# biirving/meant

Hardware: AMD Instinct MI355X
Metric: samples/sec fwd+bwd, MEANT lag=12 d=768 (higher is better)
Workload: dtype bf16; 1 GPU; full MEANT (tweet+image) fwd+CE+bwd, lag=12, d=768, 12 heads, seq=512, 224x224 p=16, E=1, vocab 64001 (BASELINE.json configs[2]/[3]); batch_per_gpu=128, global_batch=128, parallelism=dp1, micro_batches=1, train_mode_dropout=True, activation_checkpointing=False, norm_linear_fold=False, grad_allreduce=False

## Files before the change

### include/meant_hip.h

```cpp
#ifndef MEANT_HIP_H
#define MEANT_HIP_H

#include <stddef.h>
#include <stdint.h>

#ifdef __cplusplus
extern "C" {
#endif

enum meant_dtype { MEANT_F32 = 0, MEANT_BF16 = 1 };
enum meant_raw_dtype { MEANT_RAW_F32 = 0, MEANT_RAW_BF16 = 1, MEANT_RAW_F64 = 2, MEANT_RAW_U8 = 3 };
enum meant_mask_dtype { MEANT_MASK_F32 = 0, MEANT_MASK_BF16 = 1, MEANT_MASK_I64 = 2, MEANT_MASK_U8 = 3, MEANT_MASK_I32 = 4 };

enum meant_status {
  MEANT_OK = 0,
  MEANT_ERR_ARG = -1,
  MEANT_ERR_UNSUPPORTED = -2,
  MEANT_ERR_LAUNCH = -3,
  MEANT_ERR_WORKSPACE = -4
};

enum meant_epilogue {
  MEANT_EPI_NONE = 0,
  MEANT_EPI_GELU = 1,
// ... 22 lines not shown
int meant_rmsnorm_partial_fwd(const void* x, const float* scale, const float* offset, void* y, float* rinv, int64_t rows,
                              int64_t d, int64_t d_part, float eps, int dtype, void* stream);
int meant_rmsnorm_partial_bwd(const void* dy, const void* x, const float* scale, const float* rinv, void* dx, float* dscale,
                              float* doffset, int64_t rows, int64_t d, int64_t d_part, float eps, int dtype, void* workspace,
                              size_t workspace_bytes, void* stream);

int meant_rmsnorm_pooled_ok(int64_t rows, int64_t d, int64_t group_rows);
int meant_rmsnorm_fwd_pooled(const void* x, const float* scale, void* y, float* rinv, float* pooled, int64_t rows,
                             int64_t d, int64_t group_rows, int pool_input, int gelu_input, float eps, float drop_p,
                             uint64_t seed, int dtype, void* stream);
int meant_rmsnorm_bwd_pooled(const void* dy, int dy_pooled, const void* x, const float* scale, const float* rinv,
                             void* dx, float* dscale, int64_t rows, int64_t d, int64_t group_rows, float eps,
                             float drop_p, uint64_t seed, const void* dres, int dres_pooled, const void* gelu_pre,
                             int dtype, void* workspace, size_t workspace_bytes, void* stream);

int meant_rmsnorm_stats(const void* x, float* rinv, int64_t rows, int64_t d, float eps, int dtype, void* stream);
int meant_rmsnorm_bwd_chain(const void* dy, int dy_pooled, const void* x, const float* scale, const float* rinv,
                            void* dx_scaled, float* dscale, int64_t rows, int64_t d, int64_t group_rows, float eps,
                            float drop_p, uint64_t seed, const void* gelu_pre, const float* up_rinv, const float* up_bias,
                            float up_eps, int64_t up_d, float* kcoef, float* dbias_up, int dtype, void* workspace, size_t workspace_bytes,
                            void* stream);
int meant_colscale(const float* w, const float* g, float* out, int64_t N, int64_t K, void* stream);
int meant_colscale_bwd(const float* dwp, const float* w, const float* g, float* dw, float* dg, int64_t N, int64_t K,
                       void* stream);

int meant_layernorm_fwd(const void* x, const float* gamma, const float* beta, void* y, float* stats,
                        int64_t rows, int64_t d, float eps, int dtype, void* stream);
int meant_layernorm_bwd(const void* dy, const void* x, const float* gamma, const float* stats, void* dx,
                        float* dgamma, float* dbeta, int64_t rows, int64_t d, int dtype, void* workspace,
                        size_t workspace_bytes, void* stream);

int meant_linear_fwd(const void* x, int64_t ldx, const void* w, const float* bias, const void* residual,
                     int64_t ldr, void* y, int64_t ldy, void* preact, int64_t M, int64_t N, int64_t K,
                     int epilogue, int dtype, void* stream);
int meant_qkv_proj_fwd(const void* x, int64_t ldx, const void* w, const float* bias, void* qkv, int64_t M,
                       int64_t K, int64_t S, int H, int Dh, int R, const float* qa, const float* qb,
                       const float* ka, const float* kb, int dtype, void* stream);
int meant_qkv_proj_fwd_live(const void* x, int64_t ldx, const void* w, const float* bias, void* qkv, int64_t M,
                            int64_t K, int64_t S, int H, int Dh, int R, const float* qa, const float* qb,
                            const float* ka, const float* kb, const void* kv_lists, int dtype, void* stream);
int meant_linear_fwd_rowscale(const void* x, int64_t ldx, const void* w, const float* bias, const float* row_scale,
                              const void* residual, int64_t ldr, void* y, int64_t ldy, void* preact, int64_t M, int64_t N,
                              int64_t K, int epilogue, int dtype, void* stream);
int meant_linear_bwd_dx_norm(const void* dy_scaled, int64_t lddy, const void* wT, const void* x, int64_t ldx,
                             const float* coef, const void* dres, int64_t lddres, const float* dres_pooled,
                             int64_t group_rows, void* dx, int64_t lddx, int64_t M, int64_t N, int64_t K, int dtype,
                             void* stream);
int meant_linear_bwd_dx(const void* dy, int64_t lddy, const void* wT, void* dx, int64_t lddx, int64_t M,
                        int64_t N, int64_t K, int dtype, void* stream);
size_t meant_linear_bwd_dw_ws(int64_t M, int64_t N, int64_t K, int dtype);
int meant_linear_bwd_dw(const void* dy, int64_t lddy, const void* x, int64_t ldx, float* dw, float* dbias,
                        int64_t M, int64_t N, int64_t K, int dtype, void* workspace, size_t workspace_bytes,
                        void* stream);
int meant_linear_bwd_dw_rows(const void* dy, int64_t lddy, const void* x, int64_t ldx, float* dw, float* dbias,
                             const int* rows_list, const int* rows_count, int64_t M, int64_t N, int64_t K, int dtype,
                             void* workspace, size_t workspace_bytes, void* stream);

int meant_gemm_f32_strided(const float* A, const float* B, float* C, int64_t M, int64_t N, int64_t K,
                           int64_t nb1, int64_t nb2, const int64_t* sA ,
                           const int64_t* sB , const int64_t* sC , float alpha,
                           int accumulate, void* stream);

int meant_rotary_qk(void* qkv, int64_t T, int64_t S, int H, int Dh, int R, const float* qa, const float* qb,
                    const float* ka, const float* kb, int transpose, int dtype, void* stream);

size_t meant_attn_ws(int64_t G, int64_t S, int H, int Dh, int dtype);
size_t meant_attn_fwd_ws(int64_t G, int64_t S, int H, int Dh, int dtype);
enum meant_kv_list_layout { MEANT_KV_LIST_HDR = 64 };
size_t meant_kv_live_rows_ws(int64_t G, int64_t S);
int meant_kv_live_rows(const float* key_mask, int64_t G, int64_t S, int causal, void* lists, size_t lists_bytes, void* stream);
int meant_attn_fwd(const void* qkv, void* o, float* lse, const float* key_mask, int64_t G, int64_t S, int H,
                   int Dh, float scale, int causal, int dtype, void* workspace, size_t workspace_bytes,
                   void* stream);
size_t meant_attn_drop_ws(int64_t G, int64_t S, int H, int Dh, int dtype);
int meant_attn_drop_fwd(const void* qkv, void* o, float* lse, const float* key_mask, int64_t G, int64_t S, int H, int Dh,
                        float scale, int causal, float drop_p, uint64_t seed, int dtype, void* workspace,
                        size_t workspace_bytes, void* stream);
int meant_attn_drop_bwd(const void* qkv, const void* o, const void* do_, const float* lse, const float* key_mask, void* dqkv,
                        int64_t G, int64_t S, int H, int Dh, float scale, int causal, float drop_p, uint64_t seed,
                        int dtype, void* workspace, size_t workspace_bytes, void* stream);
int meant_attn_bwd(const void* qkv, const void* o, const void* do_, const float* lse, const float* key_mask,
                   void* dqkv, int64_t G, int64_t S, int H, int Dh, float scale, int causal, const float* qa,
                   const float* qb, const float* ka, const float* kb, int R, int dtype, void* workspace,
                   size_t workspace_bytes, void* stream);

int meant_gather_rows(const void* src, const int32_t* idx, const void* fill, void* dst, int64_t n, int64_t W, int dtype,
                      void* stream);
int meant_gather_rows_rot(const void* src, const int32_t* idx, void* dst, int64_t n, int64_t S, int H, int Dh, int R,
                          const float* qa, const float* qb, const float* ka, const float* kb, int dtype, void* stream);
int meant_group_scatter(const void* ddst, const int32_t* index, void* dsrc, int64_t B, int64_t L, int64_t G, int64_t S,
                        int64_t W, int dtype, void* stream);
int meant_attn_cls_fwd(const void* qkv, void* out, int64_t ld_out, float* stats, const float* key_mask, int64_t B, int64_t L,
                       int H, int Dh, float scale, int dtype, void* stream);
int meant_attn_cls_bwd(const void* qkv, const void* out, int64_t ld_out, const void* dout, int64_t ld_dout,
                       const float* stats, const float* key_mask, void* dqkv, int64_t B, int64_t L, int H, int Dh,
                       float scale, int dtype, void* stream);
int64_t meant_attn_cls_max_len(int Dh, int backward);
size_t meant_attn_cls_split_ws(int64_t B, int64_t L, int H, int Dh, int nseg);
int meant_attn_cls_split_fwd(const void* qkv, void* out, int64_t ld_out, float* stats, const float* key_mask, int64_t B,
                             int64_t L, int H, int Dh, float scale, int nseg, int dtype, void* workspace,
                             size_t workspace_bytes, void* stream);
int meant_attn_cls_split_bwd(const void* qkv, const void* out, int64_t ld_out, const void* dout, int64_t ld_dout,
                             const float* stats, const float* key_mask, void* dqkv, int64_t B, int64_t L, int H, int Dh,
                             float scale, int nseg, int dtype, void* workspace, size_t workspace_bytes, void* stream);

int meant_token_shift(const void* x, void* y, int64_t B, int64_t frames, int64_t n, int64_t d, int transpose, int dtype,
                      void* stream);
int meant_dropout(const void* x, void* y, int64_t n, float p, uint64_t seed, int dtype, void* stream);

int meant_temporal_attn_fwd(const void* q, const void* kv, void* o, float* p, int64_t B, int L, int H, int Dh,
                            float scale, int dtype, void* stream);
int meant_temporal_attn_bwd(const void* q, const void* kv, const float* p, const void* do_, void* dq, void* dkv,
                            int64_t B, int L, int H, int Dh, float scale, int dtype, void* stream);

int meant_patchify(const void* images, int images_dtype, void* patches, int64_t G, int C, int Hh, int Ww, int p,
                   int dtype, void* stream);

int meant_patchify_raw(const void* images, int raw_dtype, float mean, float inv_std, void* patches, int64_t G, int C,
                       int Hh, int Ww, int p, int dtype, void* stream);

int meant_meanpool_fwd(const void* x, void* out, int64_t ld_out, int64_t col_off, int64_t G, int64_t S, int64_t d,
                       int dtype, int out_dtype, void* stream);
int meant_meanpool_bwd(const void* dout, int64_t ld_out, int64_t col_off, void* dx, int64_t G, int64_t S, int64_t d,
                       int dtype, int out_dtype, void* stream);

int meant_add_rowvec(const void* x, const float* v, void* y, int64_t rows, int64_t d, int64_t period, int dtype,
                     void* stream);
int meant_add_rowvec_bwd(const void* dy, float* dv, int64_t rows, int64_t d, int64_t period, int dtype, void* stream);
int meant_gelu_bwd(const void* dy, const void* pre, void* dx, int64_t n, int dtype, void* stream);
int meant_sigmoid_bwd(const void* dy, const void* y, void* dx, int64_t n, int dtype, void* stream);
int meant_geglu_fwd(const void* h, void* y, int64_t rows, int64_t w, int dtype, void* stream);
int meant_geglu_bwd(const void* h, const void* dy, void* dh, int64_t rows, int64_t w, int dtype, void* stream);
int meant_add(const void* a, const void* b, void* y, int64_t n, int dtype, void* stream);
int meant_cast(const void* src, int dtype_src, void* dst, int dtype_dst, int64_t n, void* stream);
int meant_transpose2d(const void* src, int dtype_src, void* dst, int dtype_dst, int64_t rows, int64_t cols,
                      void* stream);
int meant_pad_copy2d(const void* src, int64_t ld_src, int64_t cols_src, int dtype_src, void* dst, int64_t ld_dst,
                     int64_t cols_dst, int dtype_dst, int64_t rows, void* stream);
int meant_embedding_fwd(const float* table, const int64_t* ids, void* out, int64_t n, int64_t d, int64_t V, int dtype,
                        void* stream);
int meant_embedding_bwd(const void* dout, const int64_t* ids, float* dtable, int64_t n, int64_t d, int64_t V, int dtype,
                        void* stream);
int meant_embedding_bwd_sorted(const void* dout, const int64_t* sorted_ids, const int64_t* order, float* dtable,
                               int64_t n, int64_t d, int64_t V, int dtype, void* stream);
int meant_embedding_bwd_sorted_range(const void* dout, const int64_t* sorted_ids, const int64_t* order, float* dtable,
                                     int64_t n, int64_t d, int64_t V, int64_t id_lo, int64_t id_hi, int dtype, void* stream);
size_t meant_sort_ids_ws(int64_t n, int64_t V);
int meant_sort_ids(const int64_t* ids, int64_t n, int64_t V, int64_t* sorted_ids, int64_t* order, void* workspace,
                   size_t workspace_bytes, void* stream);
size_t meant_embedding_bwd_seg_ws(int64_t n, int64_t d);
int meant_embedding_bwd_seg(const void* dout, const int64_t* sorted_ids, const int64_t* order, float* dtable, int64_t n,
                            int64_t d, int64_t V, int64_t id_lo, int64_t id_hi, int dtype, void* workspace,
                            size_t workspace_bytes, void* stream);

int meant_ce_probs(const float* probs, const int64_t* target, float* loss_accum, float* dprobs, int64_t B, int C,
                   void* stream);
int meant_softmax_ce_fwd(const void* logits, int64_t ld, const int64_t* target, int64_t T, int64_t V, int64_t ignore_index,
                         float* row_loss, float* lse, int dtype, void* stream);
int meant_softmax_ce_bwd(const void* logits, int64_t ld, const int64_t* target, const float* lse, int64_t T, int64_t V,
                         int64_t ignore_index, const float* gscale, void* dlogits, int dtype, void* stream);
size_t meant_select_rows_ws(int64_t T);
int meant_select_rows(const int64_t* target, int64_t T, int64_t V, int64_t ignore_index, int32_t* idx, int32_t* inv,
                      int64_t* target_sel, int32_t* count, void* workspace, size_t workspace_bytes, void* stream);
int meant_metrics_update(const void* scores, int64_t ld, int dtype, const int64_t* target, int64_t B, int C, int64_t ignore_index,
                         int64_t* state, int64_t* confusion, void* stream);
int meant_metrics_update_labels(const int64_t* pred, const int64_t* target, int64_t B, int C, int64_t ignore_index,
                                int64_t* state, int64_t* confusion, void* stream);
int meant_score_capture(const void* scores, int64_t ld, int dtype, const int64_t* target, int64_t B, int C, int col0, int ncol,
                        int64_t ignore_index, uint32_t* keys, int32_t* labels, int64_t capacity, int64_t offset, int64_t* counters,
                        void* stream);
size_t meant_auroc_ws(int64_t n);
int meant_auroc_rank(const uint32_t* keys, const int32_t* labels, int64_t n, int positive, int64_t* out, void* workspace,
                     size_t workspace_bytes, void* stream);
int meant_ce_probs_soft(const float* probs, int64_t ldp, const void* target, int64_t ldt, int target_dtype,
                        float* row_loss, float* loss, float* dprobs, int64_t ldd, int64_t B, int64_t C, void* stream);
int meant_vqa_score_update(const void* scores, int64_t lds, int scores_dtype, const void* target, int64_t ldt, int target_dtype,
                           int64_t B, int64_t C, int64_t* state, void* stream);
int meant_mlm_mask(const int64_t* ids, const void* attention_mask, int mask_dtype, const int64_t* sample_ids, int64_t sample_base,
                   int64_t id_bound, const int64_t* special_ids, int n_special, int64_t B, int64_t S, uint64_t seed,
                   uint32_t threshold, uint32_t t_replace, uint32_t t_random, int64_t mask_id, int64_t V, int64_t ignore_index,
                   int64_t* ids_out, int64_t* labels, void* stream);
int meant_patchify_raw_masked(const void* images, int raw_dtype, float mean, float inv_std, void* patches, int64_t G, int C, int Hh,
                              int Ww, int p, int dtype, uint64_t seed, uint32_t threshold, const int64_t* sample_ids,
                              int64_t sample_base, int64_t id_bound, float mask_value, void* stream);
size_t meant_mim_l1_ws(int64_t N);
int meant_mim_l1_fwd(const void* out, int dtype, const void* images, int raw_dtype, float mean, float inv_std, int64_t B, int C, int Co,
                     int Hh, int Ww, uint64_t seed, uint32_t threshold, const int64_t* sample_ids, int64_t sample_base,
                     int64_t id_bound, float unmasked_label, int on_masked, float* loss, int64_t* count, void* workspace,
                     size_t workspace_bytes, void* stream);
int meant_mim_l1_bwd(const void* out, int dtype, const void* images, int raw_dtype, float mean, float inv_std, int64_t B, int C, int Co,
                     int Hh, int Ww, uint64_t seed, uint32_t threshold, const int64_t* sample_ids, int64_t sample_base,
                     int64_t id_bound, float unmasked_label, int on_masked, const float* g, const int64_t* count, void* dout,
                     void* stream);
int meant_sumsq_f32(const float* x, int64_t n, float* out_accum, void* stream);
int meant_adamw_f32(float* p, const float* g, float* m, float* v, int64_t n, float lr, float beta1, float beta2,
                    float eps, float weight_decay, int64_t step, const float* sumsq, float max_norm,
                    float grad_scale, void* stream);
enum meant_optim_kind { MEANT_OPTIM_ADAMW = 0, MEANT_OPTIM_ADAM = 1 };
enum meant_optim_state_layout { MEANT_OPTIM_STATE_BYTES = 64 };
size_t meant_grad_stats_ws(int64_t n);
int meant_grad_stats_f32(const float* g, int64_t n, void* state, int first, void* workspace, size_t workspace_bytes, void* stream);
int meant_optim_step_f32(float* p, const float* g, float* m, float* v, int64_t n, int kind, float lr, float beta1, float beta2,
                         float eps, float weight_decay, float max_norm, int clip_scaled, const void* state, void* stream);
int meant_optim_finish(void* state, float growth_factor, float backoff_factor, int growth_interval, int dynamic, void* stream);

#ifdef __cplusplus
}
#endif
#endif
```

### meant_amd/csrc/common.h

```cpp
#pragma once
#include <hip/hip_runtime.h>
#include <stdint.h>
#include <stdio.h>
#include <math.h>
#include "../../include/meant_hip.h"

typedef __bf16 bf16;
typedef __attribute__((ext_vector_type(2))) float f32x2;
typedef __attribute__((ext_vector_type(4))) float f32x4;
typedef __attribute__((ext_vector_type(16))) float f32x16;
typedef __attribute__((ext_vector_type(4))) __bf16 bf16x4;
typedef __attribute__((ext_vector_type(8))) __bf16 bf16x8;
typedef __attribute__((ext_vector_type(4))) unsigned int u32x4;
typedef __attribute__((ext_vector_type(2))) unsigned int u32x2;

#define WAVE 64

void meant_set_error(const char* fmt, ...);

#define MEANT_REQUIRE(cond, code, ...)      \
  do {                                      \
    if (!(cond)) {                          \
      meant_set_error(__VA_ARGS__);         \
      return (code);                        \
    }                                       \
  } while (0)

#define MEANT_LAUNCH_CHECK(name)                                                     \
  do {                                                                               \
    hipError_t e__ = hipGetLastError();                                              \
    if (e__ != hipSuccess) {                                                         \
      meant_set_error("%s: launch failed: %s", name, hipGetErrorString(e__));        \
      return MEANT_ERR_LAUNCH;                                                       \
    }                                                                                \
  } while (0)

#define MEANT_MAX_DEVICES 64
int meant_current_device(void);
int meant_raise_dyn_lds(const void* kernel, int bytes);
#define MEANT_RAISE_LDS(kernel, bytes)                                        \
  do {                                                                        \
    int rc__ = meant_raise_dyn_lds((const void*)(kernel), (int)(bytes));      \
    if (rc__) return rc__;                                                    \
  } while (0)

enum meant_option_id {
  MEANT_OPT_NT_STREAM = 0, MEANT_OPT_NT_DYNAMIC, MEANT_OPT_DETERMINISTIC, MEANT_OPT_NT_GRID_CAP, MEANT_OPT_ATTN_SHORT, MEANT_OPT_NT_RAGGED, MEANT_OPT_ATTN_BWD1, MEANT_OPT_TEMPORAL_LONG, MEANT_OPT_KV_SKIP, MEANT_OPT_COUNT
};
int meant_opt(int id);

enum meant_route_id {
  ROUTE_NT128 = 0, ROUTE_NT256, ROUTE_NT256S, ROUTE_NT256S_ROT, ROUTE_NT_SPLIT, ROUTE_TN128, ROUTE_TN256, ROUTE_TN256_DET, ROUTE_TN_TAIL,
  ROUTE_GEMM_F32, ROUTE_ATTN_FWD, ROUTE_ATTN_FWD_D128, ROUTE_ATTN_FWD_D96, ROUTE_ATTN_BWD,
  ROUTE_ATTN_BWD_D128, ROUTE_ATTN_BWD_D96, ROUTE_ATTN_GENERIC, ROUTE_ATTN_CLS, ROUTE_ATTN_SHORT, ROUTE_NT_OVERLAP, ROUTE_ATTN_BWD1,
  ROUTE_ATTN_FWD_D160, ROUTE_ATTN_FWD_D192, ROUTE_ATTN_FWD_D256, ROUTE_ATTN_BWD_D160, ROUTE_ATTN_BWD_D192, ROUTE_ATTN_BWD_D256, ROUTE_TEMPORAL_LONG,
  ROUTE_EMB_SEG, ROUTE_SORT_IDS, ROUTE_NT128K, ROUTE_NT256K, ROUTE_SELECT_ROWS, ROUTE_ROTARY_QK, ROUTE_ROTARY_PAIRS, ROUTE_NT_ROT,
  ROUTE_METRICS_ROWS, ROUTE_METRICS_WAVE, ROUTE_METRICS_LABELS, ROUTE_TN256_ROWS, ROUTE_ATTN_CLS_SPLIT, ROUTE_ROWS_ELEM,
  ROUTE_SCORE_CAPTURE, ROUTE_AUROC_RANK, ROUTE_CE_SOFT_WAVE, ROUTE_CE_SOFT_BLOCK, ROUTE_VQA_SCORE,
  ROUTE_GRAD_STATS, ROUTE_OPTIM_STEP,
  MEANT_ROUTE_COUNT
};
void meant_route_hit(int route);

static inline bool meant_aligned16(const void* p) { return (reinterpret_cast<uintptr_t>(p) & 15) == 0; }
static inline bool meant_aligned_elem(const void* p, int dtype) { return (reinterpret_cast<uintptr_t>(p) & (dtype == MEANT_F32 ? 3 : 1)) == 0; }
static inline int64_t ceil_div(int64_t a, int64_t b) { return (a + b - 1) / b; }

template <typename T> struct Vec8;
template <> struct Vec8<float> {
  f32x4 lo, hi;
  __device__ __forceinline__ float get(int i) const { return i < 4 ? lo[i] : hi[i - 4]; }
  __device__ __forceinline__ void set(int i, float v) { if (i < 4) lo[i] = v; else hi[i - 4] = v; }
};
template <> struct Vec8<bf16> {
  bf16x8 v;
  __device__ __forceinline__ float get(int i) const { return (float)v[i]; }
  __device__ __forceinline__ void set(int i, float x) { v[i] = (bf16)x; }
  __device__ __forceinline__ unsigned raw(int i) const {
    typedef __attribute__((ext_vector_type(4))) unsigned uvec4;
    return (__builtin_bit_cast(uvec4, v)[i >> 1] >> ((i & 1) * 16)) & 0xffffu;
  }
};

__device__ __forceinline__ void rotary_pair(float t0, float t1, float a0, float a1, float b0, float b1, float& o0, float& o1) {
  o0 = __builtin_fmaf(t0, a0, -(t1 * b0));
  o1 = __builtin_fmaf(t1, a1, t0 * b1);
}

template <typename T> __device__ __forceinline__ Vec8<T> load8(const T* p);
template <> __device__ __forceinline__ Vec8<float> load8<float>(const float* p) {
  Vec8<float> r; r.lo = *reinterpret_cast<const f32x4*>(p); r.hi = *reinterpret_cast<const f32x4*>(p + 4); return r;
}
template <> __device__ __forceinline__ Vec8<bf16> load8<bf16>(const bf16* p) {
  Vec8<bf16> r; r.v = *reinterpret_cast<const bf16x8*>(p); return r;
}
template <typename T> __device__ __forceinline__ Vec8<T> load8s(const T* p);
template <> __device__ __forceinline__ Vec8<float> load8s<float>(const float* p) {
  Vec8<float> r;
  r.lo = __builtin_nontemporal_load(reinterpret_cast<const f32x4*>(p));
  r.hi = __builtin_nontemporal_load(reinterpret_cast<const f32x4*>(p + 4));
  return r;
}
template <> __device__ __forceinline__ Vec8<bf16> load8s<bf16>(const bf16* p) {
  Vec8<bf16> r; r.v = __builtin_nontemporal_load(reinterpret_cast<const bf16x8*>(p)); return r;
}
template <typename T> __device__ __forceinline__ void store8s(T* p, const Vec8<T>& v);
template <> __device__ __forceinline__ void store8s<float>(float* p, const Vec8<float>& v) {
  __builtin_nontemporal_store(v.lo, reinterpret_cast<f32x4*>(p)); __builtin_nontemporal_store(v.hi, reinterpret_cast<f32x4*>(p + 4));
}
template <> __device__ __forceinline__ void store8s<bf16>(bf16* p, const Vec8<bf16>& v) {
  __builtin_nontemporal_store(v.v, reinterpret_cast<bf16x8*>(p));
}
template <typename T> __device__ __forceinline__ void store8(T* p, const Vec8<T>& v);
template <> __device__ __forceinline__ void store8<float>(float* p, const Vec8<float>& v) {
  *reinterpret_cast<f32x4*>(p) = v.lo; *reinterpret_cast<f32x4*>(p + 4) = v.hi;
}
template <> __device__ __forceinline__ void store8<bf16>(bf16* p, const Vec8<bf16>& v) {
  *reinterpret_cast<bf16x8*>(p) = v.v;
}

__device__ __forceinline__ float to_f(float x) { return x; }
__device__ __forceinline__ float to_f(bf16 x) { return (float)x; }
template <typename T> __device__ __forceinline__ T from_f(float x);
template <> __device__ __forceinline__ float from_f<float>(float x) { return x; }
template <> __device__ __forceinline__ bf16 from_f<bf16>(float x) { return (bf16)x; }

__device__ __forceinline__ float wave_sum(float v) {
#pragma unroll
  for (int o = 32; o > 0; o >>= 1) v += __shfl_xor(v, o, 64);
  return v;
}
__device__ __forceinline__ float wave_max(float v) {
#pragma unroll
  for (int o = 32; o > 0; o >>= 1) v = fmaxf(v, __shfl_xor(v, o, 64));
  return v;
}

#define MEANT_DPP_ADD(v, CTRL) ((v) + __builtin_bit_cast(float, __builtin_amdgcn_update_dpp(0, __builtin_bit_cast(int, (v)), (CTRL), 0xf, 0xf, true)))
__device__ __forceinline__ float wave_sum_dpp(float v) {
  v = MEANT_DPP_ADD(v, 0xB1);
  v = MEANT_DPP_ADD(v, 0x4E);
  v = MEANT_DPP_ADD(v, 0x141);
  v = MEANT_DPP_ADD(v, 0x140);
  const int b = __builtin_bit_cast(int, v);
  const float r0 = __builtin_bit_cast(float, __builtin_amdgcn_readlane(b, 0)), r1 = __builtin_bit_cast(float, __builtin_amdgcn_readlane(b, 16));
  const float r2 = __builtin_bit_cast(float, __builtin_amdgcn_readlane(b, 32)), r3 = __builtin_bit_cast(float, __builtin_amdgcn_readlane(b, 48));
  return (r0 + r1) + (r2 + r3);
}
__device__ __forceinline__ float rms_rinv(float sumsq, float inv_sqrt_d, float eps) {
  return 1.0f / (sqrtf(sumsq) * inv_sqrt_d + eps);
}

__device__ __forceinline__ float gelu_erf(float x) { return 0.5f * x * (1.0f + erff(x * 0.70710678118654752f)); }
__device__ __forceinline__ float gelu_erf_fast(float x) {
  const float z = fabsf(x) * 0.70710678118654752f;
  const float t = __builtin_amdgcn_rcpf(fmaf(0.3275911f, z, 1.0f));
  float p = fmaf(1.061405429f, t, -1.453152027f);
  p = fmaf(p, t, 1.421413741f);
  p = fmaf(p, t, -0.284496736f);
  p = fmaf(p, t, 0.254829592f);
  const float half_erfc = 0.5f * p * t * __builtin_amdgcn_exp2f(-1.4426950408889634f * z * z);
  const float phi = x < 0.f ? half_erfc : 1.0f - half_erfc;
  return x * phi;
}
__device__ __forceinline__ float gelu_phi_fast(float x) {
  const float z = fabsf(x) * 0.70710678118654752f;
  const float t = __builtin_amdgcn_rcpf(fmaf(0.3275911f, z, 1.0f));
  float p = fmaf(1.061405429f, t, -1.453152027f);
  p = fmaf(p, t, 1.421413741f);
  p = fmaf(p, t, -0.284496736f);
  p = fmaf(p, t, 0.254829592f);
  const float half_erfc = 0.5f * p * t * __builtin_amdgcn_exp2f(-1.4426950408889634f * z * z);
  return x < 0.f ? half_erfc : 1.0f - half_erfc;
}
constexpr unsigned PHI_LO = 0x3A80u, PHI_HI = 0x40FFu, PHI_N = PHI_HI - PHI_LO + 1;
__device__ __forceinline__ unsigned phi_slot(unsigned bits) {
  unsigned m = bits & 0x7FFFu;
  m = m < PHI_LO ? PHI_LO : m;
  m = m > PHI_HI ? PHI_HI : m;
  return (m - PHI_LO) + ((bits >> 15) & 1u) * PHI_N;
}
__device__ __forceinline__ float gelu_erf_grad(float x) {
  const float cdf = 0.5f * (1.0f + erff(x * 0.70710678118654752f));
  const float pdf = 0.39894228040143268f * __expf(-0.5f * x * x);
  return cdf + x * pdf;
}

__device__ __forceinline__ float gelu_erf_grad_fast(float x) {
  const float z = fabsf(x) * 0.70710678118654752f;
  const float t = __builtin_amdgcn_rcpf(fmaf(0.3275911f, z, 1.0f));
  float p = fmaf(1.061405429f, t, -1.453152027f);
  p = fmaf(p, t, 1.421413741f);
  p = fmaf(p, t, -0.284496736f);
  p = fmaf(p, t, 0.254829592f);
  const float e = __builtin_amdgcn_exp2f(-0.72134752044448170f * x * x);
  const float half_erfc = 0.5f * p * t * e;
  const float phi = x < 0.f ? half_erfc : 1.0f - half_erfc;
  return fmaf(x * 0.39894228040143268f, e, phi);
}

__device__ __forceinline__ float hash_uniform(uint64_t seed, uint64_t idx) {
  uint64_t z = seed + idx * 0x9E3779B97F4A7C15ull;
  z = (z ^ (z >> 30)) * 0xBF58476D1CE4E5B9ull;
  z = (z ^ (z >> 27)) * 0x94D049BB133111EBull;
  z = z ^ (z >> 31);
  return (float)(z >> 40) * (1.0f / 16777216.0f);
}
#ifndef DROP_HASH32
#define DROP_HASH32 1
#endif
__device__ __forceinline__ uint32_t mix32(uint32_t h) {
  h ^= h >> 16; h *= 0x85EBCA6Bu; h ^= h >> 13; h *= 0xC2B2AE35u; h ^= h >> 16;
// ... 80 lines not shown
```

### meant_amd/csrc/core.hip

```cpp
#include "common.h"
#include <stdarg.h>
#include <string.h>
#include <stdlib.h>
#include <atomic>
#include <mutex>
#include <unordered_map>

static thread_local char g_err[512] = "";

void meant_set_error(const char* fmt, ...) {
  va_list ap;
  va_start(ap, fmt);
  vsnprintf(g_err, sizeof(g_err), fmt, ap);
  va_end(ap);
}

extern "C" const char* meant_last_error(void) { return g_err; }

extern "C" int meant_version(void) { return 200;  }

namespace {
struct DeviceState {
  int cus = -1;
  std::unordered_map<const void*, int> lds_raised;
};
std::mutex g_dev_mu;
DeviceState g_dev[MEANT_MAX_DEVICES];
}

int meant_current_device(void) {
  int dev = 0;
  if (hipGetDevice(&dev) != hipSuccess || dev < 0 || dev >= MEANT_MAX_DEVICES) return -1;
  return dev;
}

extern "C" int meant_num_cus(void) {
  const int dev = meant_current_device();
  if (dev < 0) return 0;
  std::lock_guard<std::mutex> lock(g_dev_mu);
  DeviceState& st = g_dev[dev];
  if (st.cus < 0) {
    hipDeviceProp_t p;
    st.cus = hipGetDeviceProperties(&p, dev) == hipSuccess ? p.multiProcessorCount : 0;
  }
  return st.cus;
}

int meant_raise_dyn_lds(const void* kernel, int bytes) {
  const int dev = meant_current_device();
  MEANT_REQUIRE(dev >= 0, MEANT_ERR_LAUNCH, "no current HIP device (or device index >= %d)", MEANT_MAX_DEVICES);
  std::lock_guard<std::mutex> lock(g_dev_mu);
  DeviceState& st = g_dev[dev];
  const auto it = st.lds_raised.find(kernel);
  if (it != st.lds_raised.end() && it->second >= bytes) return MEANT_OK;
  const hipError_t e = hipFuncSetAttribute(kernel, hipFuncAttributeMaxDynamicSharedMemorySize, bytes);
  MEANT_REQUIRE(e == hipSuccess, MEANT_ERR_LAUNCH, "hipFuncSetAttribute(%d bytes of LDS) failed on device %d: %s", bytes, dev,
                hipGetErrorString(e));
  st.lds_raised[kernel] = bytes;
  return MEANT_OK;
}

namespace {
struct OptionDef { const char* name; const char* env; int dflt; };
const OptionDef k_options[MEANT_OPT_COUNT] = {
    {"nt_stream", "MEANT_NT_STREAM", 1},
    {"nt_dynamic", "MEANT_NT_DYNAMIC", 1},
    {"deterministic", "MEANT_DETERMINISTIC", 0},
    {"nt_grid_cap", "MEANT_NT_GRID_CAP", 0},
    {"attn_short", "MEANT_ATTN_SHORT", 1},
    {"nt_ragged", "MEANT_NT_RAGGED", 1},
    {"attn_bwd1", "MEANT_ATTN_BWD1", 1},
    {"temporal_long", "MEANT_TEMPORAL_LONG", 0},
    {"kv_skip", "MEANT_KV_SKIP", 3},
};
bool is_nt_pp(const char* name) { return name && !strcmp(name, "nt_pp"); }
std::atomic<int> g_opt[MEANT_OPT_COUNT];
std::once_flag g_opt_once;
void options_init() {
  std::call_once(g_opt_once, [] {
    for (int i = 0; i < MEANT_OPT_COUNT; ++i) {
      const char* v = getenv(k_options[i].env);
      g_opt[i].store(v && *v ? atoi(v) : k_options[i].dflt, std::memory_order_relaxed);
    }
  });
}
int option_index(const char* name) {
  if (!name) return -1;
  for (int i = 0; i < MEANT_OPT_COUNT; ++i)
    if (!strcmp(name, k_options[i].name)) return i;
  return -1;
}
}

int meant_opt(int id) {
  options_init();
  return g_opt[id].load(std::memory_order_relaxed);
}

extern "C" int meant_set_option(const char* name, int value) {
  options_init();
  if (is_nt_pp(name)) {
    MEANT_REQUIRE(value == 1, MEANT_ERR_UNSUPPORTED, "meant_set_option: nt_pp is always 1 (the lock-step kernel was removed)");
    return MEANT_OK;
  }
  const int i = option_index(name);
  MEANT_REQUIRE(i >= 0, MEANT_ERR_ARG, "meant_set_option: unknown option '%s'", name ? name : "(null)");
  g_opt[i].store(value, std::memory_order_relaxed);
  return MEANT_OK;
}

extern "C" int meant_get_option(const char* name, int* value) {
  options_init();
  if (is_nt_pp(name) && value) { *value = 1; return MEANT_OK; }
  const int i = option_index(name);
  MEANT_REQUIRE(i >= 0 && value, MEANT_ERR_ARG, "meant_get_option: unknown option '%s'", name ? name : "(null)");
  *value = g_opt[i].load(std::memory_order_relaxed);
  return MEANT_OK;
}

namespace {
const char* const k_routes[MEANT_ROUTE_COUNT] = {
    "nt128", "nt256", "nt256s", "nt256s_rot", "nt_split", "tn128", "tn256", "tn256_det", "tn_tail", "gemm_f32",
    "attn_fwd", "attn_fwd_d128", "attn_fwd_d96", "attn_bwd", "attn_bwd_d128", "attn_bwd_d96",
    "attn_generic", "attn_cls", "attn_short", "nt_overlap", "attn_bwd1",
    "attn_fwd_d160", "attn_fwd_d192", "attn_fwd_d256", "attn_bwd_d160", "attn_bwd_d192", "attn_bwd_d256",
    "temporal_long", "emb_seg", "sort_ids", "nt128k", "nt256k", "select_rows",
    "rotary_qk", "rotary_pairs",
    "nt_rot",
    "metrics_rows", "metrics_wave", "metrics_labels",
    "tn256_rows",
    "attn_cls_split",
    "rows_elem",
    "score_capture", "auroc_rank",
    "ce_soft_wave", "ce_soft_block",
    "vqa_score",
    "grad_stats", "optim_step",
};
std::atomic<long long> g_route[MEANT_ROUTE_COUNT];
}

void meant_route_hit(int route) { g_route[route].fetch_add(1, std::memory_order_relaxed); }

extern "C" int64_t meant_route_count(const char* route) {
  if (!route) return -1;
  for (int i = 0; i < MEANT_ROUTE_COUNT; ++i)
    if (!strcmp(route, k_routes[i])) return (int64_t)g_route[i].load(std::memory_order_relaxed);
  return -1;
}

extern "C" void meant_route_reset(void) {
  for (int i = 0; i < MEANT_ROUTE_COUNT; ++i) g_route[i].store(0, std::memory_order_relaxed);
}
```

### meant_amd/csrc/embedding.hip

```cpp
#include "common.h"
#include "internal.h"

#define EMB_REQ(c, ...) MEANT_REQUIRE(c, MEANT_ERR_ARG, __VA_ARGS__)

namespace {

constexpr int SORT_TILE = 2048, SORT_WAVE_SPAN = 512, SORT_ROUNDS = 8;

__device__ __forceinline__ uint32_t sort_key(int64_t id, int64_t V) {
  return (uint32_t)(id < 0 ? 0 : (id >= V ? V - 1 : id));
}

template <bool IDS>
__global__ __launch_bounds__(256) void sort_hist_kernel(const int64_t* __restrict__ ids, const uint32_t* __restrict__ keys, int64_t n, int64_t V,
                                                         int passes, uint32_t* __restrict__ ghist, uint32_t* __restrict__ tile_hist,
                                                         int64_t ntiles) {
  __shared__ uint32_t h[4][256];
  const int tid = threadIdx.x;
#pragma unroll
  for (int p = 0; p < 4; ++p) h[p][tid] = 0;
  __syncthreads();
  const int64_t base = (int64_t)blockIdx.x * SORT_TILE;
  for (int i = 0; i < SORT_TILE / 256; ++i) {
    const int64_t j = base + i * 256 + tid;
    if (j < n) {
      const uint32_t key = IDS ? sort_key(ids[j], V) : keys[j];
      for (int p = 0; p < passes; ++p) atomicAdd(&h[p][(key >> (8 * p)) & 255u], 1u);
    }
  }
  __syncthreads();
  tile_hist[(int64_t)tid * ntiles + blockIdx.x] = h[0][tid];
  for (int p = 0; p < passes; ++p)
    if (h[p][tid]) atomicAdd(&ghist[p * 256 + tid], h[p][tid]);
}

__global__ __launch_bounds__(256) void sort_count_kernel(const uint32_t* __restrict__ keys, int64_t n, int shift,
                                                          uint32_t* __restrict__ tile_hist, int64_t ntiles) {
  __shared__ uint32_t h[256];
  const int tid = threadIdx.x;
  h[tid] = 0;
  __syncthreads();
  const int64_t base = (int64_t)blockIdx.x * SORT_TILE;
  for (int i = 0; i < SORT_TILE / 256; ++i) {
    const int64_t j = base + i * 256 + tid;
    if (j < n) atomicAdd(&h[(keys[j] >> shift) & 255u], 1u);
  }
  __syncthreads();
  tile_hist[(int64_t)tid * ntiles + blockIdx.x] = h[tid];
}

__global__ __launch_bounds__(256) void sort_scan_kernel(const uint32_t* __restrict__ ghist, uint32_t* __restrict__ tile_hist, int64_t ntiles) {
  __shared__ uint32_t wsum[4];
  const int tid = threadIdx.x, digit = blockIdx.x;
  uint32_t carry;
  block_scan_incl(tid < digit ? ghist[tid] : 0u, wsum, &carry);
  uint32_t* row = tile_hist + (int64_t)digit * ntiles;
  for (int64_t t0 = 0; t0 < ntiles; t0 += 256) {
    const int64_t t = t0 + tid;
    const uint32_t x = t < ntiles ? row[t] : 0u;
    uint32_t total;
    const uint32_t incl = block_scan_incl(x, wsum, &total);
    if (t < ntiles) row[t] = carry + incl - x;
    carry += total;
  }
}

template <bool FIRST, bool LAST>
__global__ __launch_bounds__(256) void sort_scatter_kernel(const int64_t* __restrict__ ids, const uint32_t* __restrict__ kin,
                                                            const uint32_t* __restrict__ vin, int64_t n, int64_t V, int shift,
                                                            const uint32_t* __restrict__ tile_off, int64_t ntiles,
                                                            uint32_t* __restrict__ kout, uint32_t* __restrict__ vout,
                                                            int64_t* __restrict__ sorted_ids, int64_t* __restrict__ order) {
  __shared__ uint32_t cnt[4][256];
  const int tid = threadIdx.x, lane = tid & 63, wave = tid >> 6;
#pragma unroll
  for (int w = 0; w < 4; ++w) cnt[w][tid] = 0;
  __syncthreads();
  const int64_t base = (int64_t)blockIdx.x * SORT_TILE + wave * SORT_WAVE_SPAN;
  uint32_t key[SORT_ROUNDS], val[SORT_ROUNDS], rk[SORT_ROUNDS];
#pragma unroll
  for (int r = 0; r < SORT_ROUNDS; ++r) {
    const int64_t j = base + r * 64 + lane;
    const bool valid = j < n;
    key[r] = valid ? (FIRST ? sort_key(ids[j], V) : kin[j]) : 0u;
    val[r] = valid ? (FIRST ? (uint32_t)j : vin[j]) : 0u;
    const uint32_t dig = (key[r] >> shift) & 255u;
    unsigned long long m = __ballot(valid);
#pragma unroll
    for (int b = 0; b < 8; ++b) {
      const bool bit = (dig >> b) & 1u;
      const unsigned long long bal = __ballot(valid && bit);
      m &= bit ? bal : ~bal;
    }
    const unsigned long long below = m & ((1ull << lane) - 1ull);
    rk[r] = valid ? cnt[wave][dig] + (uint32_t)__popcll(below) : 0u;
    __syncthreads();
    if (valid && below == 0) cnt[wave][dig] += (uint32_t)__popcll(m);
    __syncthreads();
  }
  {
    uint32_t o = tile_off[(int64_t)tid * ntiles + blockIdx.x];
#pragma unroll
    for (int w = 0; w < 4; ++w) {
      const uint32_t c = cnt[w][tid];
      cnt[w][tid] = o;
      o += c;
    }
  }
  __syncthreads();
#pragma unroll
  for (int r = 0; r < SORT_ROUNDS; ++r) {
    const int64_t j = base + r * 64 + lane;
    if (j >= n) continue;
    const int64_t pos = (int64_t)cnt[wave][(key[r] >> shift) & 255u] + rk[r];
    if (pos >= n) continue;
    if (LAST) {
      sorted_ids[pos] = (int64_t)key[r];
      order[pos] = (int64_t)val[r];
    } else {
      kout[pos] = key[r];
      vout[pos] = val[r];
    }
  }
}

int sort_passes(int64_t V) {
  int bits = 0;
  for (uint64_t m = (uint64_t)(V - 1); m; m >>= 1) ++bits;
  const int p = (bits + 7) / 8;
  return p < 1 ? 1 : p;
}
size_t align256(size_t x) { return (x + 255) & ~(size_t)255; }
struct SortWs { size_t ghist, tile_hist, buf[2], total; int nbuf; };
SortWs sort_ws_layout(int64_t n, int passes) {
  SortWs w;
  const int64_t ntiles = ceil_div(n, SORT_TILE);
  w.nbuf = passes - 1 < 2 ? passes - 1 : 2;
  size_t off = 0;
  w.ghist = off; off += align256(4 * 256 * sizeof(uint32_t));
  w.tile_hist = off; off += align256((size_t)ntiles * 256 * sizeof(uint32_t));
  for (int i = 0; i < 2; ++i) {
    w.buf[i] = off;
    if (i < w.nbuf) off += 2 * align256((size_t)n * sizeof(uint32_t));
  }
  w.total = off;
  return w;
}

constexpr int SEG = 256;
template <typename T>
__global__ __launch_bounds__(256) void emb_seg_kernel(const T* __restrict__ dout, const int64_t* __restrict__ sorted_ids,
                                                       const int64_t* __restrict__ order, float* __restrict__ dtable,
                                                       float* __restrict__ part, int64_t n, int64_t d, int64_t V, int64_t id_lo,
                                                       int64_t id_hi, int cb_chunks) {
  const int lane = threadIdx.x & 63, wave = threadIdx.x >> 6;
  const int64_t s = (int64_t)blockIdx.x * 4 + wave;
  const int64_t j0 = s * SEG;
  if (j0 >= n) return;
  const int64_t j1 = j0 + SEG < n ? j0 + SEG : n;
  if (sorted_ids[j1 - 1] < id_lo || sorted_ids[j0] >= id_hi) return;
  const int c0 = blockIdx.y * cb_chunks;
  const int left = (int)(d >> 3) - c0;
  const int nch = left < cb_chunks ? left : cb_chunks;
  const bool has0 = lane < nch, has1 = lane + 64 < nch;
  const int64_t col0 = (int64_t)(c0 + lane) * 8, col1 = (int64_t)(c0 + lane + 64) * 8;
  float acc0[8], acc1[8];
#pragma unroll
  for (int e = 0; e < 8; ++e) acc0[e] = acc1[e] = 0.f;
  int64_t cur = sorted_ids[j0];
  bool open_left = j0 > 0 && sorted_ids[j0 - 1] == cur;

  auto flush = [&](int64_t id, int slot) {
    if (id < 0 || id >= V || id < id_lo || id >= id_hi) return;
    if (slot >= 0) {
      float* row = part + (s * 2 + slot) * d;
      Vec8<float> v;
      if (has0) {
#pragma unroll
        for (int e = 0; e < 8; ++e) v.set(e, acc0[e]);
        store8<float>(row + col0, v);
      }
      if (has1) {
#pragma unroll
        for (int e = 0; e < 8; ++e) v.set(e, acc1[e]);
        store8<float>(row + col1, v);
      }
      return;
    }
    float* row = dtable + id * d;
    if (has0) {
      Vec8<float> v = load8<float>(row + col0);
#pragma unroll
      for (int e = 0; e < 8; ++e) v.set(e, v.get(e) + acc0[e]);
      store8<float>(row + col0, v);
    }
    if (has1) {
      Vec8<float> v = load8<float>(row + col1);
#pragma unroll
      for (int e = 0; e < 8; ++e) v.set(e, v.get(e) + acc1[e]);
      store8<float>(row + col1, v);
    }
  };

  for (int64_t jb = j0; jb < j1; jb += 64) {
    const int64_t jl = jb + lane < j1 ? jb + lane : j1 - 1;
    const long long my_id = sorted_ids[jl], my_ord = order[jl];
    const int cnt = (int)(j1 - jb < 64 ? j1 - jb : 64);
    for (int t0 = 0; t0 < cnt; t0 += 4) {
      Vec8<T> r0[4], r1[4];
      long long ids4[4];
#pragma unroll
      for (int u = 0; u < 4; ++u) {
        const int t = t0 + u < cnt ? t0 + u : cnt - 1;
        ids4[u] = __shfl(my_id, t, 64);
        const long long ord = __shfl(my_ord, t, 64);
        const bool row_ok = ord >= 0 && ord < n;
        const T* src = dout + (row_ok ? ord : 0) * d;
        r0[u] = Vec8<T>{};
        r1[u] = Vec8<T>{};
        if (has0 && row_ok) r0[u] = load8s<T>(src + col0);
        if (has1 && row_ok) r1[u] = load8s<T>(src + col1);
      }
#pragma unroll
      for (int u = 0; u < 4; ++u) {
        if (t0 + u >= cnt) break;
        const int64_t id = ids4[u];
        if (id != cur) {
          flush(cur, open_left ? 0 : -1);
#pragma unroll
          for (int e = 0; e < 8; ++e) acc0[e] = acc1[e] = 0.f;
          cur = id;
          open_left = false;
        }
#pragma unroll
        for (int e = 0; e < 8; ++e) {
          if (has0) acc0[e] += r0[u].get(e);
          if (has1) acc1[e] += r1[u].get(e);
        }
      }
    }
  }
  const bool open_right = j1 < n && sorted_ids[j1] == cur;
  flush(cur, open_left ? 0 : (open_right ? 1 : -1));
}

constexpr int SEG_SHORT = 16;
__global__ __launch_bounds__(256) void emb_seg_cross_kernel(const int64_t* __restrict__ sorted_ids, const float* __restrict__ part,
                                                             int* __restrict__ longk, float* __restrict__ dtable, int64_t n, int64_t d,
                                                             int64_t V, int64_t id_lo, int64_t id_hi) {
  const int lane = threadIdx.x & 63, wave = threadIdx.x >> 6;
  const int64_t s = (int64_t)blockIdx.x * 4 + wave, j0 = s * SEG, j1 = j0 + SEG;
  if (j1 >= n) return;
  const int64_t id = sorted_ids[j1 - 1];
  const bool owner = sorted_ids[j1] == id && !(j0 > 0 && sorted_ids[j0 - 1] == id)
                     && id >= 0 && id < V && id >= id_lo && id < id_hi;
  int64_t K = 0;
  if (owner) {
    const int64_t nst = (n + SEG - 1) / SEG;
    int64_t follow = 0;
    for (int64_t t0 = s + 1;; t0 += 64) {
      const int64_t t = t0 + lane;
      const int k = __popcll(__ballot(t < nst && sorted_ids[t * SEG] == id));
      follow += k;
      if (k < 64) break;
    }
    K = follow + 1;
  }
  if (blockIdx.y == 0 && lane == 0) longk[s] = K > SEG_SHORT ? (int)K : 0;
  if (K == 0 || K > SEG_SHORT) return;
  const int64_t col = (int64_t)blockIdx.y * 256 + lane * 4;
  if (col >= d) return;
  f32x4 acc = *reinterpret_cast<const f32x4*>(part + (s * 2 + 1) * d + col);
  for (int64_t k = 1; k < K; ++k) acc += *reinterpret_cast<const f32x4*>(part + (s + k) * 2 * d + col);
  f32x4* dst = reinterpret_cast<f32x4*>(dtable + id * d + col);
  *dst = *dst + acc;
}

__global__ __launch_bounds__(256) void emb_seg_long_kernel(const int64_t* __restrict__ sorted_ids, const float* __restrict__ part,
                                                            const int* __restrict__ longk, float* __restrict__ dtable, int64_t d) {
  __shared__ f32x4 red[16][16];
  const int tid = threadIdx.x;
  const int64_t s = blockIdx.x;
  const int64_t K = longk[s];
  if (K == 0) return;
  const int64_t id = sorted_ids[s * SEG + SEG - 1];
  const int p = tid >> 4;
  const int64_t col = (int64_t)blockIdx.y * 64 + (tid & 15) * 4;
  const bool active = col < d;
  const int64_t piece = (K + 15) / 16, k0 = p * piece, k1 = k0 + piece < K ? k0 + piece : K;
  f32x4 acc = {0.f, 0.f, 0.f, 0.f};
  if (active) {
#pragma unroll 4
    for (int64_t k = k0; k < k1; ++k) {
      const float* row = k == 0 ? part + (s * 2 + 1) * d : part + (s + k) * 2 * d;
      acc += *reinterpret_cast<const f32x4*>(row + col);
    }
  }
  red[p][tid & 15] = acc;
  __syncthreads();
#pragma unroll
  for (int h = 8; h > 0; h >>= 1) {
    if (p < h) red[p][tid & 15] += red[p + h][tid & 15];
    __syncthreads();
  }
  if (p == 0 && active) {
    f32x4* dst = reinterpret_cast<f32x4*>(dtable + id * d + col);
    *dst = *dst + red[0][tid & 15];
  }
}

size_t seg_part_bytes(int64_t n, int64_t d) { return (size_t)ceil_div(n, SEG) * 2 * (size_t)d * sizeof(float); }

template <typename T>
__global__ __launch_bounds__(256) void embedding_fwd_kernel(const float* __restrict__ table, const int64_t* __restrict__ ids,
                                                             T* __restrict__ out, int64_t n, int d, int64_t V) {
  const int lane = threadIdx.x & 63, wave = threadIdx.x >> 6;
  const int nch = d >> 3;
  for (int64_t r = (int64_t)blockIdx.x * 4 + wave; r < n; r += (int64_t)gridDim.x * 4) {
    int64_t id = ids[r];
    id = id < 0 ? 0 : (id >= V ? V - 1 : id);
    const float* src = table + id * d;
    for (int ch = lane; ch < nch; ch += 64) {
      const Vec8<float> v = load8<float>(src + ch * 8);
      Vec8<T> o;
#pragma unroll
      for (int k = 0; k < 8; ++k) o.set(k, v.get(k));
      store8s<T>(out + r * d + ch * 8, o);
    }
  }
}
template <typename T>
__global__ __launch_bounds__(256) void embedding_fwd_elem_kernel(const float* __restrict__ table, const int64_t* __restrict__ ids,
                                                                  T* __restrict__ out, int64_t n, int d, int64_t V) {
  const int lane = threadIdx.x & 63, wave = threadIdx.x >> 6;
  for (int64_t r = (int64_t)blockIdx.x * 4 + wave; r < n; r += (int64_t)gridDim.x * 4) {
    int64_t id = ids[r];
    id = id < 0 ? 0 : (id >= V ? V - 1 : id);
    const float* src = table + id * d;
    for (int e = lane; e < d; e += 64) out[r * d + e] = from_f<T>(src[e]);
  }
}
template <typename T>
__global__ __launch_bounds__(256) void embedding_bwd_kernel(const T* __restrict__ dout, const int64_t* __restrict__ ids,
                                                             float* __restrict__ dtable, int64_t n, int d, int64_t V) {
  const int lane = threadIdx.x & 63, wave = threadIdx.x >> 6;
  for (int64_t r = (int64_t)blockIdx.x * 4 + wave; r < n; r += (int64_t)gridDim.x * 4) {
    int64_t id = ids[r];
    id = id < 0 ? 0 : (id >= V ? V - 1 : id);
    float* dst = dtable + id * d;
    for (int e = lane; e < d; e += 64) atomicAdd(dst + e, to_f(dout[r * d + e]));
  }
}

constexpr int EMB_SEG = 256;
template <typename T>
__global__ __launch_bounds__(256) void embedding_bwd_sorted_kernel(const T* __restrict__ dout, const int64_t* __restrict__ sorted_ids,
                                                                    const int64_t* __restrict__ order, float* __restrict__ dtable,
                                                                    int64_t n, int d, int64_t V, int det, int64_t id_lo, int64_t id_hi) {
  const int lane = threadIdx.x & 63, wave = threadIdx.x >> 6;
  int64_t j0 = ((int64_t)blockIdx.x * 4 + wave) * EMB_SEG;
  if (j0 >= n) return;
  int64_t j1 = j0 + EMB_SEG < n ? j0 + EMB_SEG : n;
  if (sorted_ids[j1 - 1] < id_lo || sorted_ids[j0] >= id_hi) return;
  if (det) {
    if (j0 > 0) {
      const int64_t prev = sorted_ids[j0 - 1];
      while (j0 < j1 && sorted_ids[j0] == prev) ++j0;
      if (j0 == j1) return;
    }
    const int64_t last = sorted_ids[j1 - 1];
    while (j1 < n && sorted_ids[j1] == last) ++j1;
  }
  const int nch = d >> 3;
  const bool has1 = lane + 64 < nch, has0 = lane < nch;
  float acc0[8], acc1[8];
#pragma unroll
  for (int e = 0; e < 8; ++e) acc0[e] = acc1[e] = 0.f;
  int64_t cur = sorted_ids[j0];
  bool shared = !det && j0 > 0 && sorted_ids[j0 - 1] == cur;

  auto flush = [&](int64_t id, bool atomic) {
    if (id < 0 || id >= V || id < id_lo || id >= id_hi) return;
    float* row = dtable + id * d;
    if (atomic) {
#pragma unroll
      for (int e = 0; e < 8; ++e) {
        if (has0) atomicAdd(row + lane * 8 + e, acc0[e]);
        if (has1) atomicAdd(row + (lane + 64) * 8 + e, acc1[e]);
      }
    } else {
      if (has0) {
        Vec8<float> v = load8<float>(row + lane * 8);
#pragma unroll
        for (int e = 0; e < 8; ++e) v.set(e, v.get(e) + acc0[e]);
        store8<float>(row + lane * 8, v);
      }
      if (has1) {
        Vec8<float> v = load8<float>(row + (lane + 64) * 8);
#pragma unroll
        for (int e = 0; e < 8; ++e) v.set(e, v.get(e) + acc1[e]);
        store8<float>(row + (lane + 64) * 8, v);
      }
    }
  };

  for (int64_t jb = j0; jb < j1; jb += 64) {
    const int64_t jl = jb + lane < j1 ? jb + lane : j1 - 1;
    const long long my_id = sorted_ids[jl], my_ord = order[jl];
    const int cnt = (int)(j1 - jb < 64 ? j1 - jb : 64);
    for (int t0 = 0; t0 < cnt; t0 += 4) {
      Vec8<T> r0[4], r1[4];
      long long ids4[4];
#pragma unroll
      for (int u = 0; u < 4; ++u) {
        const int t = t0 + u < cnt ? t0 + u : cnt - 1;
        ids4[u] = __shfl(my_id, t, 64);
        const long long ord = __shfl(my_ord, t, 64);
        const T* src = dout + ord * d;
        if (has0) r0[u] = load8s<T>(src + lane * 8);
        if (has1) r1[u] = load8s<T>(src + (lane + 64) * 8);
      }
#pragma unroll
      for (int u = 0; u < 4; ++u) {
        if (t0 + u >= cnt) break;
        const int64_t id = ids4[u];
        if (id != cur) {
          flush(cur, shared);
#pragma unroll
          for (int e = 0; e < 8; ++e) acc0[e] = acc1[e] = 0.f;
          cur = id;
          shared = false;
        }
#pragma unroll
        for (int e = 0; e < 8; ++e) {
          if (has0) acc0[e] += r0[u].get(e);
          if (has1) acc1[e] += r1[u].get(e);
        }
      }
    }
  }
  flush(cur, !det && (shared || (j1 < n && sorted_ids[j1] == cur)));
}

}

static int sort_run(const int64_t* ids, int64_t V, const uint32_t* keys, const uint32_t* vals, int64_t n, int passes, int64_t* sorted_ids,
                    int64_t* order, uint32_t* keys_out, uint32_t* vals_out, const SortWs& w, char* base, hipStream_t st, const char* what) {
  const bool from_ids = ids != nullptr;
  uint32_t* ghist = (uint32_t*)(base + w.ghist);
  uint32_t* tile_hist = (uint32_t*)(base + w.tile_hist);
  uint32_t* bk[2] = {nullptr, nullptr};
  uint32_t* bv[2] = {nullptr, nullptr};
  for (int i = 0; i < w.nbuf; ++i) {
    bk[i] = (uint32_t*)(base + w.buf[i]);
    bv[i] = (uint32_t*)(base + w.buf[i] + align256((size_t)n * sizeof(uint32_t)));
  }
  const int64_t ntiles = ceil_div(n, SORT_TILE);
  const dim3 grid((unsigned)ntiles), block(256);
  const hipError_t e = hipMemsetAsync(ghist, 0, 4 * 256 * sizeof(uint32_t), st);
  MEANT_REQUIRE(e == hipSuccess, MEANT_ERR_LAUNCH, "%s: clearing the digit counters failed: %s", what, hipGetErrorString(e));
  if (from_ids) hipLaunchKernelGGL(sort_hist_kernel<true>, grid, block, 0, st, ids, keys, n, V, passes, ghist, tile_hist, ntiles);
  else hipLaunchKernelGGL(sort_hist_kernel<false>, grid, block, 0, st, ids, keys, n, V, passes, ghist, tile_hist, ntiles);
  for (int p = 0; p < passes; ++p) {
    const bool first = p == 0, last = p == passes - 1;
    const uint32_t* kin = first ? keys : bk[(p - 1) & 1];
    const uint32_t* vin = first ? vals : bv[(p - 1) & 1];
    uint32_t* kout = last ? keys_out : bk[p & 1];
    uint32_t* vout = last ? vals_out : bv[p & 1];
    const int shift = 8 * p;
    if (!first) hipLaunchKernelGGL(sort_count_kernel, grid, block, 0, st, kin, n, shift, tile_hist, ntiles);
    hipLaunchKernelGGL(sort_scan_kernel, dim3(256), block, 0, st, (const uint32_t*)(ghist + p * 256), tile_hist, ntiles);
#define SORT_SCATTER(F, L)                                                                                                     \
  hipLaunchKernelGGL((sort_scatter_kernel<F, L>), grid, block, 0, st, ids, kin, vin, n, V, shift, (const uint32_t*)tile_hist, \
                     ntiles, kout, vout, sorted_ids, order)
    const bool F = first && from_ids, L = last && from_ids;
    if (F && L) SORT_SCATTER(true, true);
    else if (F) SORT_SCATTER(true, false);
    else if (L) SORT_SCATTER(false, true);
    else SORT_SCATTER(false, false);
#undef SORT_SCATTER
  }
  MEANT_LAUNCH_CHECK(what);
  return MEANT_OK;
}

extern "C" size_t meant_sort_ids_ws(int64_t n, int64_t V) {
  if (n <= 0 || V <= 0 || n >= (1ll << 31) || V >= (1ll << 31)) return 0;
  return sort_ws_layout(n, sort_passes(V)).total;
}

extern "C" int meant_sort_ids(const int64_t* ids, int64_t n, int64_t V, int64_t* sorted_ids, int64_t* order, void* workspace,
                              size_t workspace_bytes, void* stream) {
  EMB_REQ(ids && sorted_ids && order && n > 0 && V > 0, "sort_ids: bad argument");
  MEANT_REQUIRE(n < (1ll << 31) && V < (1ll << 31), MEANT_ERR_UNSUPPORTED, "sort_ids: n=%lld and V=%lld must be below 2^31", (long long)n,
                (long long)V);
  {
    const char *a = (const char*)ids, *o1 = (const char*)sorted_ids, *o2 = (const char*)order;
    const size_t len = (size_t)n * sizeof(int64_t);
    const auto overlap = [len](const char* x, const char* y) { return x < y + len && y < x + len; };
    EMB_REQ(!overlap(a, o1) && !overlap(a, o2) && !overlap(o1, o2), "sort_ids: ids, sorted_ids and order must not overlap");
  }
  const int passes = sort_passes(V);
  const SortWs w = sort_ws_layout(n, passes);
  MEANT_REQUIRE(workspace && workspace_bytes >= w.total, MEANT_ERR_WORKSPACE, "sort_ids: workspace of %zu bytes needed, %zu given", w.total, workspace_bytes);
  EMB_REQ((reinterpret_cast<uintptr_t>(workspace) & 3) == 0, "sort_ids: 4-byte workspace alignment");
  const int rc = sort_run(ids, V, nullptr, nullptr, n, passes, sorted_ids, order, nullptr, nullptr, w, (char*)workspace, (hipStream_t)stream, "sort_ids");
  if (rc != MEANT_OK) return rc;
  meant_route_hit(ROUTE_SORT_IDS);
  return MEANT_OK;
}

size_t sort_u32_ws(int64_t n) { return n <= 0 || n >= (1ll << 31) ? 0 : sort_ws_layout(n, 4).total; }

int sort_u32_launch(const uint32_t* keys, const uint32_t* vals, int64_t n, uint32_t* keys_out, uint32_t* vals_out, void* ws, size_t ws_bytes,
                    hipStream_t stream) {
  EMB_REQ(keys && vals && keys_out && vals_out && n > 0 && n < (1ll << 31), "sort_u32: bad argument");
  const SortWs w = sort_ws_layout(n, 4);
  MEANT_REQUIRE(ws && ws_bytes >= w.total, MEANT_ERR_WORKSPACE, "sort_u32: workspace of %zu bytes needed, %zu given", w.total, ws_bytes);
  EMB_REQ((reinterpret_cast<uintptr_t>(ws) & 3) == 0, "sort_u32: 4-byte workspace alignment");
  return sort_run(nullptr, 0, keys, vals, n, 4, nullptr, nullptr, keys_out, vals_out, w, (char*)ws, stream, "sort_u32");
}

extern "C" size_t meant_embedding_bwd_seg_ws(int64_t n, int64_t d) {
  if (n <= 0 || d <= 0) return 0;
  return seg_part_bytes(n, d) + align256((size_t)ceil_div(n, SEG) * sizeof(int));
}

extern "C" int meant_embedding_bwd_seg(const void* dout, const int64_t* sorted_ids, const int64_t* order, float* dtable, int64_t n,
                                       int64_t d, int64_t V, int64_t id_lo, int64_t id_hi, int dtype, void* workspace,
                                       size_t workspace_bytes, void* stream) {
  EMB_REQ(dout && sorted_ids && order && dtable && n > 0 && d > 0 && V > 0 && 0 <= id_lo && id_lo <= id_hi && id_hi <= V,
          "embedding_bwd_seg: bad argument");
  MEANT_REQUIRE(d % 8 == 0, MEANT_ERR_UNSUPPORTED, "embedding_bwd_seg: d=%lld must be a multiple of 8", (long long)d);
  MEANT_REQUIRE(d < (1ll << 22), MEANT_ERR_UNSUPPORTED, "embedding_bwd_seg: d=%lld is beyond the launch grid (d < 2^22)", (long long)d);
  const size_t need = meant_embedding_bwd_seg_ws(n, d);
  MEANT_REQUIRE(workspace && workspace_bytes >= need, MEANT_ERR_WORKSPACE, "embedding_bwd_seg: workspace of %zu bytes needed, %zu given", need, workspace_bytes);
  EMB_REQ(meant_aligned16(dout) && meant_aligned16(dtable) && meant_aligned16(workspace), "embedding_bwd_seg: 16-byte alignment");
  if (id_lo == id_hi) return MEANT_OK;
  const int64_t nst = ceil_div(n, SEG);
  const int chunks = (int)(d >> 3);
  const int ncb = (int)ceil_div(chunks, 128);
  const int cb_chunks = (int)ceil_div(chunks, ncb);
  hipStream_t st = (hipStream_t)stream;
  DISPATCH_DTYPE(dtype, T,
                 hipLaunchKernelGGL(emb_seg_kernel<T>, dim3((unsigned)ceil_div(nst, 4), (unsigned)ncb), dim3(256), 0, st, (const T*)dout,
                                    sorted_ids, order, dtable, (float*)workspace, n, d, V, id_lo, id_hi, cb_chunks));
  if (nst > 1) {
    int* longk = (int*)((char*)workspace + seg_part_bytes(n, d));
    hipLaunchKernelGGL(emb_seg_cross_kernel, dim3((unsigned)ceil_div(nst - 1, 4), (unsigned)ceil_div(d, 256)), dim3(256), 0, st, sorted_ids,
                       (const float*)workspace, longk, dtable, n, d, V, id_lo, id_hi);
    hipLaunchKernelGGL(emb_seg_long_kernel, dim3((unsigned)(nst - 1), (unsigned)ceil_div(d, 64)), dim3(256), 0, st, sorted_ids,
                       (const float*)workspace, (const int*)longk, dtable, d);
  }
  MEANT_LAUNCH_CHECK("embedding_bwd_seg");
  meant_route_hit(ROUTE_EMB_SEG);
  return MEANT_OK;
}

extern "C" int meant_embedding_fwd(const float* table, const int64_t* ids, void* out, int64_t n, int64_t d, int64_t V, int dtype, void* stream) {
  EMB_REQ(table && ids && out && n > 0 && d > 0 && d < (1ll << 30) && V > 0, "embedding_fwd: bad argument");
  int64_t nb = ceil_div(n, 4); if (nb > 8192) nb = 8192;
  if (d % 8 == 0) {
    DISPATCH_DTYPE(dtype, T,
                   hipLaunchKernelGGL(embedding_fwd_kernel<T>, dim3((unsigned)nb), dim3(256), 0, (hipStream_t)stream, table, ids, (T*)out, n, (int)d, V));
  } else {
    DISPATCH_DTYPE(dtype, T,
                   hipLaunchKernelGGL(embedding_fwd_elem_kernel<T>, dim3((unsigned)nb), dim3(256), 0, (hipStream_t)stream, table, ids, (T*)out, n, (int)d, V));
  }
  MEANT_LAUNCH_CHECK("embedding_fwd");
  return MEANT_OK;
}
extern "C" int meant_embedding_bwd_sorted(const void* dout, const int64_t* sorted_ids, const int64_t* order, float* dtable, int64_t n,
                                          int64_t d, int64_t V, int dtype, void* stream) {
  EMB_REQ(dout && sorted_ids && order && dtable && n > 0 && d > 0 && V > 0, "embedding_bwd_sorted: bad argument");
  MEANT_REQUIRE(d <= 1024 && d % 8 == 0, MEANT_ERR_UNSUPPORTED, "embedding_bwd_sorted: d=%lld must be a multiple of 8 and <= 1024", (long long)d);
  EMB_REQ(meant_aligned16(dout) && meant_aligned16(dtable), "embedding_bwd_sorted: 16-byte alignment");
  const int64_t nb = ceil_div(n, 4 * EMB_SEG);
  DISPATCH_DTYPE(dtype, T,
                 hipLaunchKernelGGL(embedding_bwd_sorted_kernel<T>, dim3((unsigned)nb), dim3(256), 0, (hipStream_t)stream, (const T*)dout,
                                    sorted_ids, order, dtable, n, (int)d, V, meant_opt(MEANT_OPT_DETERMINISTIC) != 0, (int64_t)0, V));
  MEANT_LAUNCH_CHECK("embedding_bwd_sorted");
  return MEANT_OK;
}

extern "C" int meant_embedding_bwd_sorted_range(const void* dout, const int64_t* sorted_ids, const int64_t* order, float* dtable, int64_t n,
                                                int64_t d, int64_t V, int64_t id_lo, int64_t id_hi, int dtype, void* stream) {
  EMB_REQ(dout && sorted_ids && order && dtable && n > 0 && d > 0 && V > 0 && 0 <= id_lo && id_lo <= id_hi && id_hi <= V,
         "embedding_bwd_sorted_range: bad argument");
  MEANT_REQUIRE(d <= 1024 && d % 8 == 0, MEANT_ERR_UNSUPPORTED, "embedding_bwd_sorted_range: d=%lld must be a multiple of 8 and <= 1024", (long long)d);
  EMB_REQ(meant_aligned16(dout) && meant_aligned16(dtable), "embedding_bwd_sorted_range: 16-byte alignment");
  if (id_lo == id_hi) return MEANT_OK;
  const int64_t nb = ceil_div(n, 4 * EMB_SEG);
  DISPATCH_DTYPE(dtype, T,
                 hipLaunchKernelGGL(embedding_bwd_sorted_kernel<T>, dim3((unsigned)nb), dim3(256), 0, (hipStream_t)stream, (const T*)dout,
                                    sorted_ids, order, dtable, n, (int)d, V, meant_opt(MEANT_OPT_DETERMINISTIC) != 0, id_lo, id_hi));
  MEANT_LAUNCH_CHECK("embedding_bwd_sorted_range");
  return MEANT_OK;
}

extern "C" int meant_embedding_bwd(const void* dout, const int64_t* ids, float* dtable, int64_t n, int64_t d, int64_t V, int dtype, void* stream) {
  EMB_REQ(dout && ids && dtable && n > 0 && d > 0 && V > 0, "embedding_bwd: bad argument");
  int64_t nb = ceil_div(n, 4); if (nb > 8192) nb = 8192;
  DISPATCH_DTYPE(dtype, T,
                 hipLaunchKernelGGL(embedding_bwd_kernel<T>, dim3((unsigned)nb), dim3(256), 0, (hipStream_t)stream, (const T*)dout, ids, dtable, n, (int)d, V));
  MEANT_LAUNCH_CHECK("embedding_bwd");
  return MEANT_OK;
}
```

### meant_amd/modules.py

```python
from __future__ import annotations

import math
from typing import Optional

import torch
from torch import nn

from . import ops
from ._lib import EPI_NONE, EPI_GELU, EPI_SIGMOID


COMPOSE_PRE_LINEAR = True

POOL_LAST_LINEAR = True

import os as _os
TWO_STREAMS = _os.environ.get("MEANT_TWO_STREAMS", "1") != "0"
_SIDE = {}


def _side_stream(device):
    key = (device.type, device.index)
    if key not in _SIDE:
        _SIDE[key] = torch.cuda.Stream(device=device)
# ... 98 lines not shown
        s = self.scale.float()[None, :] ** power[:, None]
        s = torch.cat((s, s), dim=-1)
        si = s ** -1
        return cos * s, sin * s, cos * si, sin * si

    def tables(self, seq_len: int, device, head_dim: Optional[int] = None) -> tuple:
        key = (seq_len, str(device), self.freqs._version, self.freqs.data_ptr())
        hit = self._tables.get(key)
        if hit is not None:
            if head_dim is None:
                return hit
            pkey = ("pad", head_dim) + key
            padded = self._tables.get(pkey)
            if padded is None:
                padded = self._tables[pkey] = ops.pad_rotary_tables(hit, head_dim)
            return padded
        with torch.no_grad():
            f = self.freqs.detach().float().cpu()
            pos = torch.arange(seq_len)
            ang = torch.repeat_interleave(pos.to(f.dtype)[:, None] * f[None, :], 2, dim=-1)
            cos, sin = ang.cos(), ang.sin()
            if self.use_xpos:
                power = (pos - seq_len // 2) / self.scale_base
                s = self.scale.detach().float().cpu()[None, :] ** power[:, None]
                s = torch.cat((s, s), dim=-1)
                si = s ** -1
                t = (cos * s, sin * s, cos * si, sin * si)
            else:
                t = (cos, sin, cos, sin)
            t = tuple(x.contiguous().to(device) for x in t)
            if not self.use_xpos:
                t = (t[0], t[1], t[0], t[1])
        self._tables = {k: v for k, v in self._tables.items() if k[-2:] == key[-2:]}
        self._tables[key] = t
        return t if head_dim is None else self.tables(seq_len, device, head_dim)


def _rotate_pairs(t, a, b):
    R = a.shape[1]
    tr = t[..., :R].float()
    pr = tr.reshape(*tr.shape[:-1], R // 2, 2)
    rot = torch.stack((-pr[..., 1], pr[..., 0]), dim=-1).reshape(tr.shape)
    out = tr * a[None, :, None, :] + rot * b[None, :, None, :]
    return torch.cat((out.to(t.dtype), t[..., R:]), dim=-1)


def _qkv_params(mod, pre=None):
    wqkv = torch.cat([mod.q.weight, mod.v.weight, mod.k.weight], dim=0)
    bqkv = torch.cat([mod.q.bias, mod.v.bias, mod.k.bias], dim=0)
    if pre is not None:
        wqkv, bqkv = ops.compose_linear(pre.weight, pre.bias, wqkv, bqkv)
    return wqkv, bqkv


def _rotate_learned(qkv, rot: RotaryEmbedding, G, S, H, D):
    q5 = qkv.view(G, S, 3, H, D // H)
    qa, qb, ka, kb = rot.tables_autograd(S)
    return torch.stack((_rotate_pairs(q5[:, :, 0], qa, qb), _rotate_pairs(q5[:, :, 1], ka, kb), q5[:, :, 2]), dim=2).reshape(G * S, 3 * D)


def learned_rotary_attention(x, mod, rot: RotaryEmbedding, key_mask, causal: bool, pre=None):
    G, S, d = x.shape
    H = mod.num_heads
    wqkv, bqkv = _qkv_params(mod, pre)
    D = wqkv.shape[0] // 3
    packed = _rotate_learned(ops.linear(x.reshape(G * S, d), wqkv, bqkv), rot, G, S, H, D)
    return ops.attention_core(packed, G, S, H, 1.0 / math.sqrt(D), None, causal, key_mask).view(G, S, D)


def score_dropout_attention(x, mod, rot: RotaryEmbedding, key_mask, causal: bool, p: float, seed: int, pre=None):
    G, S, d = x.shape
    H = mod.num_heads
    wqkv, bqkv = _qkv_params(mod, pre)
    D = wqkv.shape[0] // 3
    qkv = ops.linear(x.reshape(G * S, d), wqkv, bqkv)
    tables = None
    if rot is not None and getattr(rot, 'learned_freq', False):
        qkv = _rotate_learned(qkv, rot, G, S, H, D)
    elif rot is not None:
        tables = rot.tables(S, x.device)
    return ops.attention_core_score_dropout(qkv, G, S, H, 1.0 / math.sqrt(D), p, seed, tables, causal, key_mask).view(G, S, D)


class _MHA(nn.Module):

    def __init__(self, num_heads, dim, mask, droput, rot=None):
        super().__init__()
        self.num_heads, self.dim = num_heads, dim
        self.Dh = int(dim / num_heads)
        self.dropout = nn.Dropout(droput)
        if rot is not None:
            setattr(self, *rot)
        self.mask = mask
        self.softmax = nn.Softmax(dim=-1)
        self.multi_mad = Linear(self.num_heads * self.Dh, self.dim)
        self.atten_size = self.Dh * self.num_heads
        self.q = Linear(self.dim, self.atten_size)
        self.v = Linear(self.dim, self.atten_size)
        self.k = Linear(self.dim, self.atten_size)

    def _fused(self, x, rot, key_mask, pre):
        if rot is not None and getattr(rot, 'learned_freq', False):
            return learned_rotary_attention(x, self, rot, key_mask, bool(self.mask), pre)
        tables = rot.tables(x.shape[1], x.device, ops.run_head_dim(self.Dh, x.dtype)) if rot is not None else None
        prew = (pre.weight, pre.bias) if pre is not None else None
        return ops.qkv_attention(x, self.q.weight, self.q.bias, self.v.weight, self.v.bias, self.k.weight, self.k.bias,
                                 tables, key_mask, bool(self.mask), self.num_heads, pre=prew)


class attention(_MHA):

    def __init__(self, num_heads, dim, pos_emb: RotaryEmbedding, mask=False, droput=0.):
        super().__init__(num_heads, dim, mask, droput, ('pos_emb', pos_emb))

    def core(self, x, pre=None):
        return self._fused(x, self.pos_emb, None, pre)

    def forward(self, input):
        out = self.multi_mad(self.core(input))
        if self.training and self.dropout.p > 0:
            out = self.dropout(out)
        return out


class xPosAttention(_MHA):

    def __init__(self, num_heads, dim, xPos: RotaryEmbedding, mask=True, droput=0.):
        super().__init__(num_heads, dim, mask, droput, ('xPos', xPos))

    def core(self, x, attention_mask=None, pre=None):
        if self.training and self.dropout.p > 0:
            return score_dropout_attention(x, self, self.xPos, attention_mask, bool(self.mask), float(self.dropout.p), _seed(), pre)
        return self._fused(x, self.xPos, attention_mask, pre)

    def forward(self, input, attention_mask=None):
        return self.multi_mad(self.core(input, attention_mask))


class temporal(_MHA):

    def __init__(self, num_heads, dim, mask=False, droput=0.):
        super().__init__(num_heads, dim, mask, droput)

    def forward(self, input):
        o = ops.temporal_attention(input, self.q.weight, self.q.bias, self.v.weight, self.v.bias, self.k.weight, self.k.bias,
                                   self.num_heads)
        return self.multi_mad(o)


def _seed() -> int:
    return int(torch.randint(0, 2 ** 62, (1,)).item())


def _encoder_layer(e, e2, x, margs, p1, p2, pool, fold):
    n, res = ops.rmsnorm_fork(x, e[0].scale, e[0].eps, any_width=True)
    if COMPOSE_PRE_LINEAR and e[1].bias is not None:
        h = e[2].multi_mad(e[2].core(n, *margs, pre=e[1]))
    else:
        h = e[2](e[1](n), *margs)
    h = e[3](h, drop_p=p1, seed=_seed() if p1 > 0 else 0)
    x1 = e[-1](h, residual=res)
    fold = ops.norm_linear_ok(x1, e2[1].weight, fold)
    seed2 = _seed() if p2 > 0 else 0
    if pool and ops.pooled_norm_ok(x1, x1.shape[1]):
        if fold:
            return ops.norm_linear_gelu_norm_pooled(x1, e2[0].scale, e2[0].eps, e2[1].weight, e2[1].bias, e2[3].scale, e2[3].eps, p2, seed2)
        n, xm = ops.rmsnorm_fork_pooled(x1, e2[0].scale, e2[0].eps)
        return ops.linear_gelu_rmsnorm_pooled(n, e2[1].weight, e2[1].bias, e2[3].scale, e2[3].eps, p2, seed2), xm
    if fold:
        h, res = ops.norm_linear_gelu_norm(x1, e2[0].scale, e2[0].eps, e2[1].weight, e2[1].bias, e2[3].scale, e2[3].eps, p2, seed2)
    else:
        n, res = ops.rmsnorm_fork(x1, e2[0].scale, e2[0].eps, any_width=True)
        h = ops.linear_gelu_rmsnorm(n, e2[1].weight, e2[1].bias, e2[3].scale, e2[3].eps, p2, seed2, any_width=True)
    if pool:
        return h, res
    return e2[-1](h, residual=res)


class visionEncoder(nn.Module):

    def __init__(self, dim, num_heads, flash=False):
        super().__init__()
        self.dim, self.num_heads = dim, num_heads
        self.posEmbed = RotaryEmbedding(dim=math.floor(dim / num_heads / 2), freqs_for='pixel')
        atten = attention(num_heads, dim, self.posEmbed)
        self.encode = nn.ModuleList([RMSNorm(dim), Linear(dim, dim), atten, RMSNorm(dim), Linear(dim, dim)])
        self.encode2 = nn.ModuleList([RMSNorm(dim), Linear(dim, dim), nn.GELU(), RMSNorm(dim), Linear(dim, dim)])

    def forward(self, input, pool: bool = False, fold=None):
        return _encoder_layer(self.encode, self.encode2, input, (), 0.0, 0.0, pool, fold)


class languageEncoder(nn.Module):

    def __init__(self, dim, num_heads, dropout=0.0, flash=False):
        super().__init__()
        self.dim, self.num_heads = dim, num_heads
        self.xPos = RotaryEmbedding(dim=48, use_xpos=True)
        att = xPosAttention(num_heads, dim, self.xPos)
        self.encode = nn.ModuleList([RMSNorm(dim), Linear(dim, dim), att, RMSNorm(dim), nn.Dropout(dropout), Linear(dim, dim)])
        self.encode2 = nn.ModuleList([RMSNorm(dim), Linear(dim, dim), nn.GELU(), RMSNorm(dim), nn.Dropout(), Linear(dim, dim)])

    def forward(self, input, attention_mask=None, pool: bool = False, fold=None):
        e, e2 = self.encode, self.encode2
        p1, p2 = (e[4].p, e2[4].p) if self.training else (0.0, 0.0)
        return _encoder_layer(e, e2, input, (attention_mask,), p1, p2, pool, fold)


class temporalEncoder(nn.Module):

    def __init__(self, dim, num_heads, lag, norms=True):
        super().__init__()
        self.dim, self.num_heads, self.lag = dim, num_heads, lag
        self.temp_embedding = nn.Parameter(torch.randn(1, lag, dim))
        if norms:
            mods = [RMSNorm(dim), Linear(dim, dim), temporal(num_heads, dim), RMSNorm(dim), Linear(dim, dim)]
        else:
            mods = [Linear(dim, dim), temporal(num_heads, dim), Linear(dim, dim)]
        self.temp_encode = nn.ModuleList(mods)

    def forward(self, x):
        x = ops.add_rowvec(x, self.temp_embedding)
        for mod in self.temp_encode:
            x = mod(x)
        return x


class _Patchify(nn.Module):

    def __init__(self, p):
        super().__init__()
        self.p = p
        self.out_dtype = torch.float32
        self.norm_mean, self.norm_std = 0.0, 1.0

    def set_normalization(self, mean: float, std: float):
        self.norm_mean, self.norm_std = float(mean), float(std)

    def forward(self, images):
        return ops.patchify(images, self.p, self.out_dtype, self.norm_mean, self.norm_std)


class _PatchEmbed(nn.Sequential):
    def __init__(self, patch_dim, dim, p):
        super().__init__(_Patchify(p), Linear(patch_dim, dim))

    def forward(self, images, dtype=torch.float32):
        self[0].out_dtype = dtype
        return self[1](self[0](images))


def _run_encoder(enc, x, *args, checkpoint: bool = False, **kw):
    if checkpoint and torch.is_grad_enabled() and x.requires_grad:
        from torch.utils.checkpoint import checkpoint as _ckpt
        return _ckpt(enc, x, *args, use_reentrant=False, preserve_rng_state=True, **kw)
    return enc(x, *args, **kw)


def _ckpt_setting(model):
    v = getattr(model, "activation_checkpointing", False)
    return v if isinstance(v, bool) else int(v)


def _run_stack(encoders, x, *args, checkpoint=False):
    n = len(encoders)
    fold = ops.stack_fold(n, x.numel() // x.shape[-1], x.shape[-1])
    for i, enc in enumerate(encoders):
        ck = checkpoint if isinstance(checkpoint, bool) else i < checkpoint
        last = enc.encode2[-1]
        if POOL_LAST_LINEAR and i == n - 1 and isinstance(last, Linear):
            h, res = _run_encoder(enc, x, *args, checkpoint=ck, pool=True, fold=fold)
            return (h, res, last.weight, last.bias)
        x = _run_encoder(enc, x, *args, checkpoint=ck, fold=fold)
    return x


def _pool_parts(compute_dtype, *stacks):
    if all(isinstance(st, tuple) for st in stacks):
        if all(st[0].dim() == 3 for st in stacks):
            return ops.pool_linear_cat(list(stacks))
        parts = [st if st[0].dim() == 2 else (ops.meanpool_f32(st[0]), ops.meanpool_f32(st[1]), st[2], st[3]) for st in stacks]
        return ops.pooled_linear_cat(parts, compute_dtype)
    toks = []
    for st in stacks:
        if isinstance(st, tuple):
            h, res, w, b = st
            if h.dim() == 2:
                raise RuntimeError("meant_amd: one stack pooled its last layer, the other did not")
            st = ops.linear(h, w, b, residual=res)
        toks.append(st)
    return ops.meanpool_cat(*toks)


POOL_OWN_STREAM = _os.environ.get("MEANT_POOL_OWN_STREAM", "1") == "1"


def _pool_own_stream(compute_dtype, st):
    if not POOL_OWN_STREAM or not (isinstance(st, tuple) and st[0].dim() == 2):
        return st
    return ops.pooled_linear_cat([st], compute_dtype)


def _embed(mods, ids, dtype):
    x = ids
    for mod in mods:
        if isinstance(mod, nn.Embedding) and mod.max_norm is None and not mod.sparse and x.dtype in (torch.int64, torch.int32):
            x = ops.embedding(x, mod.weight, dtype)
        else:
            x = mod(x)
    if x.dtype != dtype:
        x = x.to(dtype)
    return x


HEAD_F32_MAX_CLASSES = 64


def _head(mods, x):
    x = mods[0](x)
    if x.dtype != torch.float32 and mods[1].weight.shape[0] <= HEAD_F32_MAX_CLASSES:
        x = x.float()
    if isinstance(mods[2], nn.Sigmoid):
        return mods[1](x, epilogue=EPI_SIGMOID)
    return mods[2](mods[1](x))


class meant(nn.Module):

    def __init__(self, text_dim, image_dim, price_dim, height, width, patch_res, lag, num_classes, embedding, flash=False,
                 num_heads=8, num_encoders=1, channels=4):
        super().__init__()
        self.lag, self.text_dim, self.image_dim = lag, text_dim, image_dim
        self.dim = text_dim + image_dim
        self.num_heads = num_heads
        self.channels = channels
        self.patch_dim = channels * patch_res * patch_res
        self.n = int((height * width) / (patch_res ** 2))
        self.embedding = nn.ModuleList([embedding])
        self.patchEmbed = _PatchEmbed(self.patch_dim, image_dim, patch_res)
        self.visionEncoders = nn.ModuleList([visionEncoder(image_dim, num_heads, flash=flash) for _ in range(num_encoders)])
        self.languageEncoders = nn.ModuleList([languageEncoder(text_dim, num_heads, flash=flash) for _ in range(num_encoders)])
        self.temporal_encoding = nn.ModuleList([temporalEncoder(self.dim, num_heads, lag)])
        self.mlpHead = nn.ModuleList([RMSNorm(self.dim), Linear(self.dim, num_classes), nn.Sigmoid()])
        self.compute_dtype = None

    def forward(self, tweets, images, attention_mask=None):
        dt = resolve_compute_dtype(self, images)
        B = images.shape[0]
        if images.is_cuda and TWO_STREAMS:
            ops.set_index_stream(images.device, _side_stream(images.device))
        words = _embed(self.embedding, tweets.reshape(B * self.lag, tweets.shape[2]), dt)
        if attention_mask is not None:
            attention_mask = attention_mask.reshape(B * self.lag, attention_mask.shape[2])
        ck = _ckpt_setting(self)
        side = _side_stream(images.device) if (TWO_STREAMS and images.is_cuda and not ck) else None
        if side is not None:
            main = torch.cuda.current_stream()
            side.wait_stream(main)
            with torch.cuda.stream(side):
                img = self.patchEmbed(images.reshape(B * self.lag, *images.shape[2:]), dt)
                img = _run_stack(self.visionEncoders, img, checkpoint=ck)
                img = _pool_own_stream(dt, img)
        if side is not None and LANG_PRIORITY:
            hi = _hi_stream(images.device)
            hi.wait_stream(main)
            with torch.cuda.stream(hi):
                words = _run_stack(self.languageEncoders, words, attention_mask, checkpoint=ck)
                words = _pool_own_stream(dt, words)
            main.wait_stream(hi)
            for tt in (words if isinstance(words, tuple) else (words,)):
                if tt is not None and tt.is_cuda:
                    tt.record_stream(main)
        else:
            words = _run_stack(self.languageEncoders, words, attention_mask, checkpoint=ck)
        if side is not None:
            main.wait_stream(side)
            for tt in (img if isinstance(img, tuple) else (img,)):
                if tt is not None and tt.is_cuda:
                    tt.record_stream(main)
        else:
            img = self.patchEmbed(images.reshape(B * self.lag, *images.shape[2:]), dt)
            img = _run_stack(self.visionEncoders, img, checkpoint=ck)
        done = [torch.is_tensor(st) and st.dim() == 2 for st in (words, img)]
        if any(done):
            fused = torch.cat([st if d_ else _pool_parts(dt, st) for st, d_ in zip((words, img), done)], dim=1).view(B, self.lag, self.dim)
        else:
            fused = _pool_parts(dt, words, img).view(B, self.lag, self.dim)
        for enc in self.temporal_encoding:
            fused = enc(fused)
        return _head(self.mlpHead, fused).squeeze(dim=1).float()


class meant_vision(nn.Module):

    def __init__(self, image_dim, price_dim, height, width, patch_res, lag, num_classes, flash=False, num_heads=8,
                 num_encoders=1, channels=4):
        super().__init__()
        self.dim = image_dim
        self.num_heads = num_heads
        self.channels = channels
        self.patch_dim = channels * patch_res * patch_res
        self.n = int((height * width) / (patch_res ** 2))
        self.patchEmbed = _PatchEmbed(self.patch_dim, image_dim, patch_res)
        self.visionEncoders = nn.ModuleList([visionEncoder(image_dim, num_heads, flash=flash) for _ in range(num_encoders)])
        self.temporal_encoding = nn.ModuleList([temporalEncoder(self.dim, num_heads, lag, norms=False)])
        self.mlpHead = nn.ModuleList([LayerNorm(self.dim), Linear(self.dim, num_classes), nn.Sigmoid()])
        self.compute_dtype = None

    def forward(self, images):
        dt = resolve_compute_dtype(self, images)
        B, L = images.shape[0], images.shape[1]
        img = self.patchEmbed(images.reshape(B * L, *images.shape[2:]), dt)
        img = _run_stack(self.visionEncoders, img)
        fused = _pool_parts(dt, img).view(B, L, self.dim)
        for enc in self.temporal_encoding:
            fused = enc(fused)
        return _head(self.mlpHead, fused).squeeze(dim=1).float()


class meant_tweet(nn.Module):

    def __init__(self, text_dim, price_dim, lag, num_classes, embedding, flash=False, num_heads=8, num_encoders=1, channels=4):
        super().__init__()
        self.dim = text_dim
        self.num_heads = num_heads
        self.embedding = nn.ModuleList([embedding])
        self.languageEncoders = nn.ModuleList([languageEncoder(text_dim, num_heads, flash=flash) for _ in range(num_encoders)])
        self.temporal_encoding = nn.ModuleList([temporalEncoder(self.dim, num_heads, lag, norms=False)])
        self.mlpHead = nn.ModuleList([LayerNorm(self.dim), Linear(self.dim, num_classes), nn.Sigmoid()])
        self.lag = lag
        self.compute_dtype = None

    def forward(self, tweets, attention_mask=None):
        dt = resolve_compute_dtype(self, None)
        B = tweets.shape[0]
        words = _embed(self.embedding, tweets.reshape(B * self.lag, tweets.shape[2]), dt)
        attention_mask = attention_mask.reshape(B * self.lag, attention_mask.shape[2])
        words = _run_stack(self.languageEncoders, words, attention_mask)
        fused = _pool_parts(dt, words).view(B, self.lag, self.dim)
        for enc in self.temporal_encoding:
            fused = enc(fused)
        return _head(self.mlpHead, fused).squeeze(dim=1).float()


class meant_vqa(nn.Module):

    def __init__(self, text_dim, image_dim, price_dim, height, width, patch_res, lag, num_classes, embedding, flash=False,
                 num_heads=8, num_encoders=1, channels=4):
        super().__init__()
        self.lag, self.text_dim, self.image_dim = lag, text_dim, image_dim
        self.dim = text_dim + image_dim
        self.num_heads = num_heads
        self.channels = channels
        self.patch_dim = channels * patch_res * patch_res
        self.n = int((height * width) / (patch_res ** 2))
        self.embedding = nn.ModuleList([embedding])
        self.patchEmbed = _PatchEmbed(self.patch_dim, image_dim, patch_res)
        self.visionEncoders = nn.ModuleList([visionEncoder(image_dim, num_heads, flash=flash) for _ in range(num_encoders)])
        self.languageEncoders = nn.ModuleList([languageEncoder(text_dim, num_heads, flash=flash) for _ in range(num_encoders)])
        self.multimodal_embedding = nn.Sequential(nn.Linear(1, self.dim), nn.GELU(), RMSNorm(self.dim), nn.Linear(self.dim, self.dim))
        self.multimodal_encoding = nn.ModuleList([visionEncoder(self.dim, num_heads, flash=flash)])
        self.mlpHead = nn.ModuleList([RMSNorm(self.dim), Linear(self.dim, num_classes), nn.Sigmoid()])
        self.compute_dtype = None

    def forward(self, tweets, images, attention_mask=None):
        dt = resolve_compute_dtype(self, images)
        words = _embed(self.embedding, tweets, dt)
        words = _run_stack(self.languageEncoders, words, attention_mask)
        img = self.patchEmbed(images, dt)
        img = _run_stack(self.visionEncoders, img)
        fused = _pool_parts(dt, words, img)
        return _head(self.mlpHead, fused).float()


flash_attention = attention
xPosAttention_flash = xPosAttention


MLM_LABELLED_ONLY = _os.environ.get("MEANT_MLM_LABELLED_ONLY", "1") != "0"


def _is_roberta_lm_head(h) -> bool:
    return all(hasattr(h, a) for a in ("dense", "layer_norm", "decoder")) and isinstance(getattr(h, "decoder"), nn.Linear)


class meant_language_pretrainer(nn.Module):

    def __init__(self, num_encoders, mlm_input_dim, embedding, lm_head, flash=False, lag=5, text_dim=768, num_heads=8):
        super().__init__()
        self.embedding = nn.ModuleList([embedding])
        self.languageEncoders = nn.ModuleList([languageEncoder(text_dim, num_heads, flash=flash) for _ in range(num_encoders)])
        self.mlm_head = lm_head
        self.lag = lag
        self.labelled_only = MLM_LABELLED_ONLY
        self.last_head_rows = None

    def _encode(self, words, attention_mask):
        dt = resolve_compute_dtype(self, None)
        x = _embed(self.embedding, words, dt)
        fold = ops.stack_fold(len(self.languageEncoders), x.numel() // x.shape[-1], x.shape[-1])
        for enc in self.languageEncoders:
            x = enc(x, attention_mask=attention_mask, fold=fold)
        return x

    def _head_features(self, x):
        h = self.mlm_head
        y = ops.linear(x, h.dense.weight, h.dense.bias, None, EPI_GELU)
        return ops.layernorm(y, h.layer_norm.weight, h.layer_norm.bias, h.layer_norm.eps)

    def forward(self, words, attention_mask=None):
        x = self._encode(words, attention_mask)
        h = self.mlm_head
        if _is_roberta_lm_head(h):
            return ops.vocab_linear(self._head_features(x), h.decoder.weight, h.decoder.bias)
        return h(x)

    def loss(self, words, attention_mask, labels, ignore_index: int = -100, labelled_only=None):
        h = self.mlm_head
        roberta = _is_roberta_lm_head(h)
        T = labels.numel()
        sel, m = None, T
        if roberta and (self.labelled_only if labelled_only is None else labelled_only):
            sel = ops.select_rows(labels, h.decoder.weight.shape[0], ignore_index)
            m = ops.padded_rows(sel.n)
            if m >= T:
                sel, m = None, T
        x = self._encode(words, attention_mask)
        self.last_head_rows = m
        if sel is None and not labels.is_cuda:
            labels = labels.to(x.device)
        if not roberta:
            return ops.softmax_cross_entropy(h(x), labels, ignore_index)
        if sel is not None:
            x = ops.take_rows(x.reshape(T, x.shape[-1]), sel.idx, sel.inv, m)
            labels = sel.target_sel[:m]
        return ops.vocab_linear_cross_entropy(self._head_features(x), h.decoder.weight, h.decoder.bias, labels, ignore_index)


def _is_vit_mim_decoder(dec) -> bool:
    return (isinstance(dec, nn.Sequential) and len(dec) == 2 and isinstance(dec[0], nn.Conv2d) and dec[0].kernel_size == (1, 1)
            and dec[0].stride == (1, 1) and dec[0].groups == 1 and isinstance(dec[1], nn.PixelShuffle))


class meant_vision_pretrainer(nn.Module):

    def __init__(self, num_encoders, decoder, mlm_input_dim, patch_res=16, channels=4, height=224, width=224, image_dim=768, num_heads=8):
        super().__init__()
        self.channels = channels
        self.patch_dim = channels * patch_res * patch_res
        self.n = int((height * width) / (patch_res ** 2))
        self.patchEmbed = _PatchEmbed(self.patch_dim, image_dim, patch_res)
        self.visionEncoders = nn.ModuleList([visionEncoder(image_dim, num_heads, flash=True)])
        self.decoder = decoder

    def forward(self, images):
        dt = resolve_compute_dtype(self, images)
        return self._decode(self.patchEmbed(images, dt))

    def loss(self, images, collator, sample_ids=None, sample_base: int = 0):
        dt = resolve_compute_dtype(self, images)
        pat, seed = self.patchEmbed[0], collator.epoch_seed
        rule = dict(prob=collator.p, seed=seed, sample_ids=sample_ids, sample_base=sample_base)
        patches = ops.patchify_masked(images, pat.p, dt, pat.norm_mean, pat.norm_std, mask_value=collator.mask_value, **rule)
        out = self._decode(self.patchEmbed[1](patches)).contiguous()
        return ops.mim_l1_loss(out, images, mean=pat.norm_mean, std=pat.norm_std, unmasked_label=collator.unmasked_label,
                               on_masked=collator.on_masked, **rule)

    def _decode(self, x):
        fold = ops.stack_fold(len(self.visionEncoders), x.numel() // x.shape[-1], x.shape[-1])
        for enc in self.visionEncoders:
            x = enc(x, fold=fold)
        b, n, c = x.shape
        hw = math.floor(n ** 0.5)
        dec = self.decoder
        if _is_vit_mim_decoder(dec):
            conv, r = dec[0], dec[1].upscale_factor
            y = ops.linear(x, conv.weight.view(conv.out_channels, c), conv.bias)
            co = conv.out_channels // (r * r)
            y = y.view(b, hw, hw, co, r, r).permute(0, 3, 1, 4, 2, 5).reshape(b, co, hw * r, hw * r)
            return y
        return dec(x.permute(0, 2, 1).reshape(b, c, hw, hw))


class _TSAttention(nn.Module):

    def __init__(self, dim, dim_head=64, heads=8):
        super().__init__()
        self.heads, self.dim_head, self.scale = heads, dim_head, dim_head ** -0.5
        inner = dim_head * heads
        self.to_qkv = Linear(dim, inner * 3, bias=False)
        self.to_out = nn.Sequential(Linear(inner, dim), nn.Identity())

    def forward(self, x, plan, tables, group_mask=None, cls_mask=None, residual=None, drop_p=0.0):
        H, Dh = self.heads, self.dim_head
        Dp = ops.divided_head_dim(Dh, x.dtype)
        if Dp != Dh:
            w = self.to_qkv.weight
            wp = torch.nn.functional.pad(w.view(3 * H, Dh, w.shape[1]), (0, 0, 0, Dp - Dh)).reshape(3 * H * Dp, w.shape[1])
            qkv = ops.linear(x, wp)
            out = ops.divided_attention(qkv, plan, tables, H, self.scale, group_mask, cls_mask)
            out = out.view(*out.shape[:-1], H, Dp)[..., :Dh].reshape(*out.shape[:-1], H * Dh)
        else:
            qkv = self.to_qkv(x)
            out = ops.divided_attention(qkv, plan, tables, H, self.scale, group_mask, cls_mask)
        if drop_p > 0.0:
            return ops.dropout(self.to_out[0](out), drop_p, _seed()) + residual
        return self.to_out[0](out, residual=residual)


class _TSPreNorm(nn.Module):
    def __init__(self, dim, fn):
        super().__init__()
        self.fn, self.norm = fn, LayerNorm(dim)


class _TSPreTokenShift(nn.Module):

    def __init__(self, frames, fn):
        super().__init__()
        self.frames, self.fn = frames, fn

    def forward(self, x, *args, **kw):
        return self.fn(ops.token_shift(x, self.frames, (x.shape[1] - 1) // self.frames), *args, **kw)


class _TSFeedForward(nn.Module):
    def __init__(self, dim, mult=4):
        super().__init__()
        self.net = nn.Sequential(Linear(dim, dim * mult * 2), nn.Identity(), nn.Identity(), Linear(dim * mult, dim))

    def forward(self, x, residual=None, drop_p=0.0):
        h = ops.geglu(self.net[0](x))
        if drop_p > 0.0:
            h = ops.dropout(h, drop_p, _seed())
        return self.net[3](h, residual=residual)


class TimeSformer(nn.Module):

    def __init__(self, *, dim, num_frames, num_classes, image_size=224, patch_size=16, channels=3, depth=12, heads=8, dim_head=64,
                 attn_dropout=0., ff_dropout=0., rotary_emb=True, shift_tokens=False):
        super().__init__()
        self.use_rotary_emb = bool(rotary_emb)
        self.shift_tokens, self.attn_dropout, self.ff_dropout = bool(shift_tokens), float(attn_dropout), float(ff_dropout)
        assert image_size % patch_size == 0, "Image dimensions must be divisible by the patch size."
        self.heads, self.patch_size, self.dim_head, self.num_frames = heads, patch_size, dim_head, num_frames
        self.to_patch_embedding = Linear(channels * patch_size ** 2, dim)
        self.cls_token = nn.Parameter(torch.randn(1, dim))
        if rotary_emb:
            self.frame_rot_emb = nn.Module()
            self.frame_rot_emb.register_buffer("inv_freqs", 1.0 / (10000 ** (torch.arange(0, dim_head, 2).float() / dim_head)))
            self.image_rot_emb = nn.Module()
            self.image_rot_emb.register_buffer("scales", torch.logspace(0., math.log(10 / 2) / math.log(2), dim_head // 4, base=2))
        else:
            self.pos_emb = nn.Embedding(num_frames * (image_size // patch_size) ** 2 + 1, dim)
# ... 85 lines not shown
```

### meant_amd/ops.py

```python
from __future__ import annotations

import ctypes
import math
import os
import threading
import weakref
from typing import NamedTuple, Optional

import torch

from . import _lib
from ._lib import lib, check, F32, BF16, EPI_NONE, EPI_GELU, EPI_RESIDUAL, EPI_SIGMOID


def _dt(t: torch.Tensor) -> int:
    if t.dtype == torch.float32:
        return F32
    if t.dtype == torch.bfloat16:
        return BF16
    raise TypeError(f"meant_amd: activations must be float32 or bfloat16, got {t.dtype}")


def _need_gpu(*ts):
    cur = None
# ... 677 lines not shown


def _linear_bwd_npad(dy2, x2, params, need_dx, has_bias, pad_rows, K):
    M, N = dy2.shape
    N8 = (N + 7) & ~7
    dyp = _pad_cols(dy2, N8)
    dx = None
    if need_dx:
        wT = weights.get(params, dy2.dtype, True, pad_rows, pad_cols=N8 - N)
        dx = torch.empty((M, K), device=dy2.device, dtype=dy2.dtype)
        check(lib.meant_linear_bwd_dx(_p(dyp), N8, _p(wT), _p(dx), K, M, N8, K, _dt(dy2), _stream()), "linear_bwd_dx")
    dw, db = _dw_acc(N8, x2, K, has_bias, lambda dw, db: _bwd_dw(dyp, x2, dw, db), keep=N)
    return dx, dw, db


def _linear_bwd_raw(dy2, x2, params, need_dx, has_bias, pad_rows=0, bias_param=None, site="linear", K=None):
    M, N = dy2.shape
    K8 = x2.shape[1]
    K = K8 if K is None else K
    if _n_pad_ok(N, dy2.dtype):
        return _linear_bwd_npad(dy2, x2, params, need_dx, has_bias, pad_rows, K)
    dx = None
    if need_dx:
        wT = weights.get(params, dy2.dtype, True, pad_rows)
        dx = torch.empty((M, K), device=dy2.device, dtype=dy2.dtype)
        check(lib.meant_linear_bwd_dx(_p(dy2), dy2.stride(0), _p(wT), _p(dx), K, M, N, K, _dt(dy2), _stream()), "linear_bwd_dx")
    if len(params) == 1 and pad_rows == 0 and K8 == K and grad_sinks and (bias_param is not None or not has_bias):
        ws_, bs_ = _sink_of(params[0], site), (_sink_of(bias_param, site) if has_bias else None)
        if ws_ is not None and (not has_bias or bs_ is not None) and ws_.view.shape == (N, K) and ws_.view.is_contiguous():
            _bwd_dw(dy2, x2, ws_.view, bs_.view if has_bias else None)
            ws_.report(params[0])
            if has_bias:
                bs_.report(bias_param)
            return dx, None, None
    dw, db = _dw_acc(N, x2, K, has_bias, lambda dw, db: _bwd_dw(dy2, x2, dw, db))
    return dx, dw, db


class _Linear(torch.autograd.Function):

    @staticmethod
    def forward(ctx, x, weight, bias, residual, epilogue):
        _need_gpu(x, weight)
        shp = x.shape
        x2, w_c = _k_pad(_c(x).view(-1, shp[-1]), weight)
        res2 = _c(residual).view(-1, weight.shape[0]) if residual is not None else None
        bias_f = _c(bias.detach().float()) if bias is not None else None
        epi = epilogue | (EPI_RESIDUAL if residual is not None else 0)
        y, pre = _linear_fwd_raw(x2, w_c, bias_f, res2, epi, bool(epilogue & EPI_GELU))
        ctx.epilogue = epilogue
        ctx.has_bias = bias is not None
        ctx.has_res = residual is not None
        ctx.weight, ctx.bias = weight, bias
        _claim(weight, "linear"); _claim(bias, "linear")
        ctx.save_for_backward(x2, pre if (epilogue & EPI_GELU) else (y if (epilogue & EPI_SIGMOID) else None))
        ctx.in_shape = shp
        return y.view(*shp[:-1], weight.shape[0])

    @staticmethod
    def backward(ctx, dy):
        x2, aux = ctx.saved_tensors
        N = ctx.weight.shape[0]
        dy2 = _c(dy).view(-1, N)
        dres = dy if ctx.has_res else None
        if ctx.epilogue & EPI_GELU:
            d2 = torch.empty_like(dy2)
            check(lib.meant_gelu_bwd(_p(dy2), _p(aux), _p(d2), dy2.numel(), _dt(dy2), _stream()), "gelu_bwd")
            dy2 = d2
        elif ctx.epilogue & EPI_SIGMOID:
            d2 = torch.empty_like(dy2)
            check(lib.meant_sigmoid_bwd(_p(dy2), _p(aux), _p(d2), dy2.numel(), _dt(dy2), _stream()), "sigmoid_bwd")
            dy2 = d2
        dx, dw, db = _linear_bwd_raw(dy2, x2, (ctx.weight,), ctx.needs_input_grad[0], ctx.has_bias, bias_param=ctx.bias, K=ctx.in_shape[-1])
        return (dx.view(ctx.in_shape) if dx is not None else None), dw, db, dres, None


def linear(x, weight, bias=None, residual=None, epilogue=EPI_NONE):
    return _Linear.apply(x, weight, bias, residual, epilogue)


def _gemm_f32(A, B, C, M, N, K, sA, sB, sC, alpha=1.0, accumulate=False):
    arr = ctypes.c_int64 * 4
    check(lib.meant_gemm_f32_strided(_p(A), _p(B), _p(C), M, N, K, 1, 1, arr(0, 0, *sA), arr(0, 0, *sB), arr(0, 0, *sC),
                                     float(alpha), int(accumulate), _stream()), "gemm_f32_strided")


class _ComposeLinear(torch.autograd.Function):

    @staticmethod
    def forward(ctx, w1, b1, wqkv, bqkv):
        _need_gpu(w1, wqkv)
        w1c, wqc = _c(w1.detach().float()), _c(wqkv.detach().float())
        b1c, bqc = _c(b1.detach().float()), _c(bqkv.detach().float())
        N3, dj = wqc.shape
        dk = w1c.shape[1]
        wc = torch.empty((N3, dk), device=w1.device, dtype=torch.float32)
        _gemm_f32(wqc, w1c, wc, N3, dk, dj, (dj, 1), (dk, 1), (dk, 1))
        bc = bqc.clone()
        _gemm_f32(wqc, b1c, bc, N3, 1, dj, (dj, 1), (1, 0), (1, 1), accumulate=True)
        ctx.save_for_backward(w1c, b1c, wqc)
        return wc, bc

    @staticmethod
    def backward(ctx, dwc, dbc):
        w1c, b1c, wqc = ctx.saved_tensors
        N3, dj = wqc.shape
        dk = w1c.shape[1]
        dwc, dbc = _c(dwc.float()), _c(dbc.float())
        dwq = torch.empty_like(wqc)
        _gemm_f32(dwc, w1c, dwq, N3, dj, dk, (dk, 1), (1, dk), (dj, 1))
        _gemm_f32(dbc, b1c, dwq, N3, dj, 1, (1, 0), (0, 1), (dj, 1), accumulate=True)
        dw1 = torch.empty_like(w1c)
        _gemm_f32(wqc, dwc, dw1, dj, dk, N3, (1, dj), (dk, 1), (dk, 1))
        db1 = torch.empty_like(b1c)
        _gemm_f32(wqc, dbc, db1, dj, 1, N3, (1, dj), (1, 0), (1, 1))
        return dw1, db1, dwq, dbc


def compose_linear(w1, b1, wqkv, bqkv):
    return _ComposeLinear.apply(w1, b1, wqkv, bqkv)


def _attn_fwd_raw(qkv2, km, G, S, H, Dh, scale, causal, drop=None):
    dt = _dt(qkv2)
    o = torch.empty((G * S, H * Dh), device=qkv2.device, dtype=qkv2.dtype)
    lse = torch.empty((G, H, S, 2), device=qkv2.device, dtype=torch.float32)
    wsb = (lib.meant_attn_fwd_ws if drop is None else lib.meant_attn_drop_ws)(G, S, H, Dh, dt)
    ws = _ws(wsb, qkv2.device, 16)
    if drop is None:
        check(lib.meant_attn_fwd(_p(qkv2), _p(o), _p(lse), _p(km), G, S, H, Dh, scale, causal, dt, _p(ws), wsb, _stream()), "attn_fwd")
    else:
        check(lib.meant_attn_drop_fwd(_p(qkv2), _p(o), _p(lse), _p(km), G, S, H, Dh, scale, causal, drop[0], drop[1], dt,
                                      _p(ws), wsb, _stream()), "attn_drop_fwd")
    return o, lse


def _attn_bwd_raw(qkv2, o, do2, lse, km, G, S, H, Dh, scale, causal, tables, drop=None):
    dt = _dt(do2)
    dqkv = torch.empty_like(qkv2)
    qa, qb, ka, kb, R = _rot(tables)
    wsb = (lib.meant_attn_ws if drop is None else lib.meant_attn_drop_ws)(G, S, H, Dh, dt)
    ws = _ws(wsb, do2.device, 16)
    if drop is None:
        check(lib.meant_attn_bwd(_p(qkv2), _p(o), _p(do2), _p(lse), _p(km), _p(dqkv), G, S, H, Dh, scale, causal,
                                 _p(qa), _p(qb), _p(ka), _p(kb), R, dt, _p(ws), wsb, _stream()), "attn_bwd")
    else:
        check(lib.meant_attn_drop_bwd(_p(qkv2), _p(o), _p(do2), _p(lse), _p(km), _p(dqkv), G, S, H, Dh, scale, causal, drop[0], drop[1], dt,
                                      _p(ws), wsb, _stream()), "attn_drop_bwd")
        if tables is not None:
            check(lib.meant_rotary_qk(_p(dqkv), G * S, S, H, Dh, R, _p(qa), _p(qb), _p(ka), _p(kb), 1, dt, _stream()), "rotary_qk^T")
    return dqkv


class _QKVAttention(torch.autograd.Function):

    @staticmethod
    def forward(ctx, x, wqkv, bqkv, tables, key_mask, causal, num_heads, scale=None):
        _need_gpu(x, wqkv)
        G, S, d = x.shape
        D = wqkv.shape[0] // 3
        Dh = D // num_heads
        x2 = _c(x).view(G * S, d)
        w_f = _c(wqkv.detach().float())
        if x.dtype == torch.bfloat16 and d % 8:
            d8 = (d + 7) & ~7
            x2, w_c = _pad_cols(x2, d8), _pad_cols(w_f, d8, x.dtype)
        else:
            w_c = cast(w_f, x.dtype)
        bias_f = _c(bqkv.detach().float())
        dt = _dt(x)
        qa, qb, ka, kb, R = _rot(tables)
        km = _c(key_mask.float()) if key_mask is not None else None
        skip = _kv_skip_bits(x, km, S, D, Dh)
        lists = kv_live_rows(km, causal) if skip else None
        qkv = torch.empty((G * S, 3 * D), device=x.device, dtype=x.dtype)
        if skip & KV_SKIP_FWD:
            check(lib.meant_qkv_proj_fwd_live(_p(x2), x2.stride(0), _p(w_c), _p(bias_f), _p(qkv), G * S, x2.shape[1], S, num_heads, Dh, R,
                                              _p(qa), _p(qb), _p(ka), _p(kb), _p(lists), dt, _stream()), "qkv_proj_fwd_live")
        else:
            check(lib.meant_qkv_proj_fwd(_p(x2), x2.stride(0), _p(w_c), _p(bias_f), _p(qkv), G * S, x2.shape[1], S, num_heads, Dh, R,
                                         _p(qa), _p(qb), _p(ka), _p(kb), dt, _stream()), "qkv_proj_fwd")
        scale = 1.0 / math.sqrt(Dh * num_heads) if scale is None else float(scale)
        o, lse = _attn_fwd_raw(qkv, km, G, S, num_heads, Dh, scale, int(causal))
        ctx.save_for_backward(x2, qkv, o, lse, km, w_f, lists)
        ctx.kv_skip = skip
        ctx.tables = tables
        ctx.meta = (G, S, d, D, Dh, num_heads, scale, int(causal))
        return o.view(G, S, D)

    @staticmethod
    def backward(ctx, do):
        x2, qkv, o, lse, km, w_f, lists = ctx.saved_tensors
        G, S, d, D, Dh, H, scale, causal = ctx.meta
        do2 = _c(do).view(G * S, D)
        dt = _dt(do2)
        dqkv = _attn_bwd_raw(qkv, o, do2, lse, km, G, S, H, Dh, scale, causal, ctx.tables)
        M, N, K = G * S, 3 * D, d
        dx = None
        if ctx.needs_input_grad[0]:
            wT = torch.empty((K, N), device=do2.device, dtype=do2.dtype)
            check(lib.meant_transpose2d(_p(w_f), F32, _p(wT), dt, N, K, _stream()), "transpose2d")
            dx = torch.empty((M, K), device=do2.device, dtype=do2.dtype)
            check(lib.meant_linear_bwd_dx(_p(dqkv), N, _p(wT), _p(dx), K, M, N, K, dt, _stream()), "linear_bwd_dx")
        def accumulate(dw, db):
            if ctx.kv_skip & KV_SKIP_DW:
                _bwd_dw(dqkv[:, :D], x2, dw[:D], db[:D])
                _bwd_dw_rows(dqkv[:, D:], x2, dw[D:], db[D:], lists)
            else:
                _bwd_dw(dqkv, x2, dw, db)
        dw, db = _dw_acc(N, x2, K, True, accumulate)
        return (dx.view(G, S, d) if dx is not None else None), dw, db, None, None, None, None, None


NATIVE_HEAD_DIMS = (64, 96, 128, 160, 192, 256)


def _padded_head_dim(Dh):
    if Dh in NATIVE_HEAD_DIMS or Dh > 256:
        return None
    if Dh % 8:
        return next(n for n in NATIVE_HEAD_DIMS if n > Dh)
    return 128 if Dh < 128 else next(n for n in NATIVE_HEAD_DIMS if n > Dh)


def run_head_dim(Dh: int, dtype: torch.dtype) -> int:
    return (_padded_head_dim(Dh) if dtype == torch.bfloat16 else None) or Dh


def divided_head_dim(Dh: int, dtype: torch.dtype) -> int:
    if Dh % 8 == 0:
        return Dh
    return (_padded_head_dim(Dh) if dtype == torch.bfloat16 else None) or (Dh + 7) & ~7


def pad_rotary_tables(tables, head_dim: int):
    if tables is None:
        return None
    R = tables[0].shape[1]
    R8 = (R + 7) & ~7
    if R8 == R or head_dim % 8 or R8 > head_dim:
        return tables
    done = {}
    out = []
    for i, tb in enumerate(tables):
        if id(tb) not in done:
            done[id(tb)] = torch.nn.functional.pad(tb, (0, R8 - R), value=1.0 if i % 2 == 0 else 0.0).contiguous()
        out.append(done[id(tb)])
    return tuple(out)


def qkv_attention(x, wq, bq, wk, bk, wv, bv, tables, key_mask, causal, num_heads, pre=None):
    wqkv = torch.cat([wq, wk, wv], dim=0)
    bqkv = torch.cat([bq, bk, bv], dim=0)
    if pre is not None:
        wqkv, bqkv = compose_linear(pre[0], pre[1], wqkv, bqkv)
    D = wqkv.shape[0] // 3
    Dh = D // num_heads
    Dp = _padded_head_dim(Dh) if x.dtype == torch.bfloat16 else None
    if Dp is not None:
        d = wqkv.shape[1]
        wp = torch.nn.functional.pad(wqkv.view(3 * num_heads, Dh, d), (0, 0, 0, Dp - Dh)).reshape(3 * num_heads * Dp, d)
        bp = torch.nn.functional.pad(bqkv.view(3 * num_heads, Dh), (0, Dp - Dh)).reshape(3 * num_heads * Dp)
        o = _QKVAttention.apply(x, wp, bp, tables, key_mask, causal, num_heads, 1.0 / math.sqrt(D))
        G, S = o.shape[0], o.shape[1]
        return o.view(G, S, num_heads, Dp)[..., :Dh].reshape(G, S, D)
    return _QKVAttention.apply(x, wqkv, bqkv, tables, key_mask, causal, num_heads)


class _TemporalAttention(torch.autograd.Function):

    @staticmethod
    def forward(ctx, x, wq, bq, wk, bk, wv, bv, num_heads):
        _need_gpu(x, wq)
        B, L, d = x.shape
        D = wq.shape[0]
        Dh = D // num_heads
        xc = _c(x)
        x2 = xc.view(B * L, d)
        xlast = xc[:, L - 1, :]
        wq_c = weights.get((wq,), x.dtype, False)
        wkv_c = weights.get((wk, wv), x.dtype, False)
        q, _ = _linear_fwd_raw(xlast, wq_c, _c(bq.detach().float()), None, EPI_NONE, False)
        kv, _ = _linear_fwd_raw(x2, wkv_c, torch.cat([bk.detach(), bv.detach()]).float().contiguous(), None, EPI_NONE, False)
        o = torch.empty((B, D), device=x.device, dtype=x.dtype)
        p = torch.empty((B, num_heads, L), device=x.device, dtype=torch.float32)
        scale = 1.0 / math.sqrt(Dh * num_heads)
        check(lib.meant_temporal_attn_fwd(_p(q), _p(kv), _p(o), _p(p), B, L, num_heads, Dh, scale, _dt(x), _stream()),
              "temporal_attn_fwd")
        ctx.save_for_backward(x2, q, kv, p)
        ctx.params = (wq, wk, wv)
        ctx.meta = (B, L, d, D, Dh, num_heads, scale)
        return o.view(B, 1, D)

    @staticmethod
    def backward(ctx, do):
        x2, q, kv, p = ctx.saved_tensors
        B, L, d, D, Dh, H, scale = ctx.meta
        wq, wk, wv = ctx.params
        do2 = _c(do).view(B, D)
        dq = torch.empty_like(q)
        dkv = torch.empty_like(kv)
        check(lib.meant_temporal_attn_bwd(_p(q), _p(kv), _p(p), _p(do2), _p(dq), _p(dkv), B, L, H, Dh, scale, _dt(do2), _stream()),
              "temporal_attn_bwd")
        xlast = x2.view(B, L, d)[:, L - 1, :]
        dxl, dwq, dbq = _linear_bwd_raw(dq, xlast, (wq,), True, True)
        dx2, dwkv, dbkv = _linear_bwd_raw(dkv, x2, (wk, wv), True, True)
        dx = dx2.view(B, L, d)
        last = dx[:, L - 1, :]
        tmp = torch.empty((B, d), device=dx.device, dtype=dx.dtype)
        lc = last.contiguous()
        check(lib.meant_add(_p(lc), _p(dxl), _p(tmp), B * d, _dt(dx), _stream()), "add")
        dx[:, L - 1, :] = tmp
        return dx, dwq, dbq, dwkv[:D], dbkv[:D], dwkv[D:], dbkv[D:], None


def temporal_attention(x, wq, bq, wk, bk, wv, bv, num_heads):
    return _TemporalAttention.apply(x, wq, bq, wk, bk, wv, bv, num_heads)


class _MeanPoolCat(torch.autograd.Function):

    @staticmethod
    def forward(ctx, a, b, out_dtype):
        _need_gpu(a, b)
        a = _c(a)
        G, S, da = a.shape
        db_ = 0
        if b is not None:
            b = _c(b)
            assert b.shape[0] == G and b.dtype == a.dtype
            db_ = b.shape[2]
        out = torch.empty((G, da + db_), device=a.device, dtype=out_dtype)
        dto = F32 if out_dtype == torch.float32 else BF16
        check(lib.meant_meanpool_fwd(_p(a), _p(out), da + db_, 0, G, S, da, _dt(a), dto, _stream()), "meanpool_fwd")
        if b is not None:
            check(lib.meant_meanpool_fwd(_p(b), _p(out), da + db_, da, G, b.shape[1], db_, _dt(a), dto, _stream()), "meanpool_fwd")
        ctx.meta = (a.shape, None if b is None else b.shape, a.dtype, out_dtype)
        return out

    @staticmethod
# ... 213 lines not shown
    if len(key[0]) > 16:
        raise ValueError(f"mlm_mask: at most 16 special ids, got {len(key[0])}")
    if not key[0]:
        return None, 0
    t = _special_cache.get(key)
    if t is None:
        t = _special_cache[key] = torch.tensor(key[0], dtype=torch.int64, device=device)
    return t, len(key[0])


def mlm_mask(ids, attention_mask=None, sample_ids=None, *, mask_id: int, special_ids=(), vocab_size: int, p: float = 0.15,
             replace: float = 1.0, random: float = 0.0, ignore_index: int = -100, seed: int = 0, sample_base: int = 0,
             id_bound: int = ID_BOUND, out=None):
    _need_gpu(ids, attention_mask, sample_ids, out)
    if ids.dim() != 2 or ids.dtype != torch.int64:
        raise ValueError(f"mlm_mask: ids must be int64 [B, S], got {ids.dtype} {tuple(ids.shape)}")
    if replace < 0.0 or random < 0.0 or replace + random > 1.0:
        raise ValueError(f"mlm_mask: replace = {replace} and random = {random} must be probabilities that sum to at most 1")
    ids = _c(ids)
    B, S = ids.shape
    mdt = 0
    if attention_mask is not None:
        if attention_mask.dtype not in _MASK_DTYPES or tuple(attention_mask.shape) != (B, S):
            raise ValueError(f"mlm_mask: attention_mask must be [B, S] float32 / bfloat16 / int64 / int32 / uint8 / bool, got "
                             f"{attention_mask.dtype} {tuple(attention_mask.shape)}")
        attention_mask = _c(attention_mask)
        mdt = _MASK_DTYPES[attention_mask.dtype]
    sample_ids = _sample_ids(sample_ids, B, "mlm_mask")
    spec, ns = _special_ids(special_ids, ids.device)
    if out is None:
        out = torch.empty_like(ids)
    elif out.dtype != torch.int64 or out.shape != ids.shape or not out.is_contiguous():
        raise ValueError("mlm_mask: out must be a contiguous int64 tensor of ids' shape")
    labels = torch.empty_like(ids)
    check(lib.meant_mlm_mask(_p(ids), _p(attention_mask), mdt, _p(sample_ids), int(sample_base), int(id_bound), _p(spec), ns, B, S,
                             int(seed) & (2 ** 64 - 1), draw_threshold(p), draw_threshold(replace), draw_threshold(random), int(mask_id),
                             int(vocab_size), int(ignore_index), _p(out), _p(labels), _stream()), "mlm_mask")
    return out, labels


def _raw_images(images, what: str):
    if images.dim() != 4 or images.dtype not in _RAW_DTYPES:
        raise TypeError(f"{what}: images must be [B, C, H, W] in float32 / bfloat16 / float64 / uint8 (their storage type), got "
                        f"{images.dtype} {tuple(images.shape)}")
    return _c(images)


def patchify_masked(images, p: int, dtype: torch.dtype, mean: float = 0.0, std: float = 1.0, *, prob: float = 0.15, seed: int = 0,
                    sample_ids=None, sample_base: int = 0, id_bound: int = ID_BOUND, mask_value: float = 0.0):
    _need_gpu(images, sample_ids)
    images = _raw_images(images, "patchify_masked")
    G, Cc, Hh, Ww = images.shape
    sample_ids = _sample_ids(sample_ids, G, "patchify_masked")
    out = torch.empty((G, (Hh // p) * (Ww // p), p * p * Cc), device=images.device, dtype=dtype)
    check(lib.meant_patchify_raw_masked(_p(images), _RAW_DTYPES[images.dtype], float(mean), 1.0 / float(std), _p(out), G, Cc, Hh, Ww, p,
                                        _dt(out), int(seed) & (2 ** 64 - 1), draw_threshold(prob), _p(sample_ids), int(sample_base),
                                        int(id_bound), float(mask_value), _stream()), "patchify_raw_masked")
    return out


class _MimL1(torch.autograd.Function):

    @staticmethod
    def forward(ctx, out, images, sample_ids, rule):
        B, Co, Hh, Ww = out.shape
        Cc = images.shape[1]
        dev = out.device
        loss = torch.empty(1, device=dev, dtype=torch.float32)
        count = torch.empty(1, device=dev, dtype=torch.int64)
        wsb = lib.meant_mim_l1_ws(out.numel())
        ws = _ws(wsb, dev, 16)
        head = (_RAW_DTYPES[images.dtype], rule["mean"], rule["inv_std"], B, Cc, Co, Hh, Ww, rule["seed"], rule["threshold"])
        tail = (rule["sample_base"], rule["id_bound"], rule["unmasked_label"], rule["on_masked"])
        check(lib.meant_mim_l1_fwd(_p(out), _dt(out), _p(images), *head, _p(sample_ids), *tail, _p(loss), _p(count), _p(ws), wsb, _stream()),
              "mim_l1_fwd")
        ctx.save_for_backward(out, images, sample_ids, count)
        ctx.head, ctx.tail = head, tail
        ctx.mark_non_differentiable(count)
        return loss.view(()), count

    @staticmethod
    def backward(ctx, dloss, _dcount):
        out, images, sample_ids, count = ctx.saved_tensors
        g = dloss.reshape(1)
        if g.dtype != torch.float32:
            g = g.float()
        g = _c(g)
        _need_gpu(g)
        dout = torch.empty_like(out)
        check(lib.meant_mim_l1_bwd(_p(out), _dt(out), _p(images), *ctx.head, _p(sample_ids), *ctx.tail, _p(g), _p(count), _p(dout), _stream()),
              "mim_l1_bwd")
        return dout, None, None, None


def mim_l1_loss(out, images, *, prob: float = 0.15, seed: int = 0, sample_ids=None, sample_base: int = 0, id_bound: int = ID_BOUND,
                mean: float = 0.0, std: float = 1.0, unmasked_label: float = -100.0, on_masked: bool = False, return_count: bool = False):
    _need_gpu(out, images, sample_ids)
    images = _raw_images(images, "mim_l1_loss")
    if out.dim() != 4 or out.shape[0] != images.shape[0] or out.shape[2:] != images.shape[2:] or not 0 < out.shape[1] <= images.shape[1]:
        raise ValueError(f"mim_l1_loss: out {tuple(out.shape)} does not fit images {tuple(images.shape)} ([B, Co <= C, H, W])")
    _dt(out)
    sample_ids = _sample_ids(sample_ids, out.shape[0], "mim_l1_loss")
    rule = dict(mean=float(mean), inv_std=1.0 / float(std), seed=int(seed) & (2 ** 64 - 1), threshold=draw_threshold(prob),
                sample_base=int(sample_base), id_bound=int(id_bound), unmasked_label=float(unmasked_label), on_masked=int(bool(on_masked)))
    loss, count = _MimL1.apply(_c(out), images, sample_ids, rule)
    return (loss, count) if return_count else loss


EMB_BF16_TABLE = os.environ.get("MEANT_EMB_BF16_TABLE", "1") == "1"


EMB_PRESORT = os.environ.get("MEANT_EMB_PRESORT", "1") == "1"
_aux_streams = {}
_aux_override = {}


def set_index_stream(device, stream) -> None:
    _aux_override[(device.type, device.index)] = stream


def _aux_stream(device):
    key = (device.type, device.index)
    if _aux_override.get(key) is not None:
        return _aux_override[key]
    st = _aux_streams.get(key)
    if st is None:
        st = _aux_streams[key] = torch.cuda.Stream(device=device)
    return st


def _emb_sorted_bwd_ok(n: int, d: int) -> bool:
    return d <= 1024 and d % 8 == 0 and (n >= 4096 or bool(_lib.get_option("deterministic")))


def _emb_seg_bwd_ok(n: int, d: int) -> bool:
    return d % 8 == 0 and (n >= 4096 or bool(_lib.get_option("deterministic")))


def _emb_bwd_route(n: int, d: int) -> str:
    if _emb_seg_bwd_ok(n, d) and d > 1024:
        return "seg"
    return "sorted" if _emb_sorted_bwd_ok(n, d) else "atomic"


def _sort_ids(ids_flat: torch.Tensor, V: int):
    n = ids_flat.numel()
    sorted_ids, order = torch.empty_like(ids_flat), torch.empty_like(ids_flat)
    wsb = lib.meant_sort_ids_ws(n, V)
    ws = _ws(wsb, ids_flat.device)
    check(lib.meant_sort_ids(_p(ids_flat), n, V, _p(sorted_ids), _p(order), _p(ws), wsb, _stream()), "sort_ids")
    return sorted_ids, order


class _Embedding(torch.autograd.Function):

    @staticmethod
    def forward(ctx, ids, table, dtype):
        _need_gpu(ids, table)
        ids_c = _c(ids.long())
        V, d = table.shape
        n = ids_c.numel()
        out = torch.empty((*ids.shape, d), device=table.device, dtype=dtype)
        if dtype == torch.bfloat16 and EMB_BF16_TABLE and d % 8 == 0 and V < (1 << 31):
            tb = weights.get((table,), torch.bfloat16, False)
            idx = ids_c.view(-1).clamp(0, V - 1).to(torch.int32)
            check(lib.meant_gather_rows(_p(tb), _p(idx), None, _p(out), n, d, BF16, _stream()), "gather_rows")
        else:
            tf = _c(table.detach().float())
            check(lib.meant_embedding_fwd(_p(tf), _p(ids_c), _p(out), n, d, V, F32 if dtype == torch.float32 else BF16, _stream()),
                  "embedding_fwd")
        presort = None
        route = _emb_bwd_route(n, d)
        if EMB_PRESORT and ctx.needs_input_grad[1] and route != "atomic":
            main = torch.cuda.current_stream(ids_c.device)
            side = _aux_stream(ids_c.device)
            side.wait_stream(main)
            with torch.cuda.stream(side):
                sorted_ids, order = _sort_ids(ids_c.view(-1), V)
                ev = torch.cuda.Event()
                ev.record(side)
            presort = (sorted_ids, order, ev)
        ctx.save_for_backward(ids_c)
        ctx.presort = presort
        ctx.meta = (V, d)
        ctx.table = table
        _claim(table, "embedding")
        return out

    @staticmethod
    def backward(ctx, dout):
        (ids_c,) = ctx.saved_tensors
        V, d = ctx.meta
        dout = _c(dout)
        sink = _sink_of(ctx.table, "embedding") if grad_sinks else None
        if sink is not None and (sink.view.shape != (V, d) or not sink.view.is_contiguous()):
            sink = None
        dtab = sink.view if sink is not None else torch.zeros((V, d), device=dout.device, dtype=torch.float32)
        n = ids_c.numel()
        route = _emb_bwd_route(n, d)
        if route != "atomic":
            if ctx.presort is not None:
                sorted_ids, order, ev = ctx.presort
                cur = torch.cuda.current_stream(dout.device)
                cur.wait_event(ev)
                sorted_ids.record_stream(cur)
                order.record_stream(cur)
            else:
                sorted_ids, order = _sort_ids(ids_c.view(-1), V)
            nsl = sink.row_slices(ctx.table) if sink is not None else 1
            if route == "seg":
                wsb = lib.meant_embedding_bwd_seg_ws(n, d)
                ws = _ws(wsb, dout.device)
                for c in range(nsl):
                    lo, hi = V * c // nsl, V * (c + 1) // nsl
                    check(lib.meant_embedding_bwd_seg(_p(dout), _p(sorted_ids), _p(order), _p(dtab), n, d, V, lo, hi, _dt(dout), _p(ws), wsb,
                                                      _stream()), "embedding_bwd_seg")
                    if nsl > 1:
                        sink.report_rows(ctx.table, lo, hi, c == nsl - 1)
                if nsl > 1:
                    return None, None, None
            elif nsl > 1:
                for c in range(nsl):
                    lo, hi = V * c // nsl, V * (c + 1) // nsl
                    check(lib.meant_embedding_bwd_sorted_range(_p(dout), _p(sorted_ids), _p(order), _p(dtab), n, d, V, lo, hi, _dt(dout),
                                                               _stream()), "embedding_bwd_sorted_range")
                    sink.report_rows(ctx.table, lo, hi, c == nsl - 1)
                return None, None, None
            else:
                check(lib.meant_embedding_bwd_sorted(_p(dout), _p(sorted_ids), _p(order), _p(dtab), n, d, V, _dt(dout), _stream()),
                      "embedding_bwd_sorted")
        else:
            check(lib.meant_embedding_bwd(_p(dout), _p(ids_c), _p(dtab), n, d, V, _dt(dout), _stream()), "embedding_bwd")
        if sink is not None:
            sink.report(ctx.table)
            return None, None, None
        return None, dtab, None


def embedding(ids, table, dtype):
    return _Embedding.apply(ids, table, dtype)


def cast(x: torch.Tensor, dtype: torch.dtype) -> torch.Tensor:
    _need_gpu(x)
    if x.dtype == dtype:
        return x
    x = _c(x)
    out = torch.empty_like(x, dtype=dtype)
    check(lib.meant_cast(_p(x), _dt(x), _p(out), F32 if dtype == torch.float32 else BF16, x.numel(), _stream()), "cast")
    return out


VOCAB_PAD = 256


class _SoftmaxCE(torch.autograd.Function):

    @staticmethod
    def forward(ctx, logits_pad, target, V, ignore_index):
        _need_gpu(logits_pad, target)
        logits_pad = _c(logits_pad)
        T, ld = logits_pad.shape
        assert ld % 8 == 0 and V <= ld
        tgt = _c(target.long())
        row_loss = torch.empty(T, device=logits_pad.device, dtype=torch.float32)
        lse = torch.empty(T, 2, device=logits_pad.device, dtype=torch.float32)
        check(lib.meant_softmax_ce_fwd(_p(logits_pad), ld, _p(tgt), T, V, int(ignore_index), _p(row_loss), _p(lse), _dt(logits_pad),
                                       _stream()), "softmax_ce_fwd")
        nvalid = ((tgt != ignore_index) & (tgt >= 0) & (tgt < V)).sum().clamp_(min=1).float()
        ctx.save_for_backward(logits_pad, tgt, lse, nvalid)
        ctx.V, ctx.ignore_index = int(V), int(ignore_index)
        return row_loss.sum() / nvalid

    @staticmethod
    def backward(ctx, dloss):
        logits_pad, tgt, lse, nvalid = ctx.saved_tensors
        T, ld = logits_pad.shape
        g = (dloss.float() / nvalid).reshape(1).contiguous()
        dl = torch.empty_like(logits_pad)
        check(lib.meant_softmax_ce_bwd(_p(logits_pad), ld, _p(tgt), _p(lse), T, ctx.V, ctx.ignore_index, _p(g), _p(dl), _dt(logits_pad),
                                       _stream()), "softmax_ce_bwd")
        return dl, None, None, None


class _VocabLinear(torch.autograd.Function):

    @staticmethod
    def forward(ctx, x, weight, bias):
        _need_gpu(x, weight)
        V, d = weight.shape
        Vp = (V + VOCAB_PAD - 1) // VOCAB_PAD * VOCAB_PAD
        shp = x.shape
        x2 = _c(x).view(-1, d)
        w_c = weights.get((weight,), x.dtype, False, Vp - V)
        bias_f = None
        if bias is not None:
            bias_f = _c(torch.nn.functional.pad(bias.detach().float(), (0, Vp - V)))
        y, _ = _linear_fwd_raw(x2, w_c, bias_f, None, EPI_NONE, False)
        ctx.weight, ctx.bias, ctx.has_bias, ctx.in_shape, ctx.V = weight, bias, bias is not None, shp, V
        _claim(weight, "vocab"); _claim(bias, "vocab")
        ctx.save_for_backward(x2)
        return y.view(*shp[:-1], Vp)

    @staticmethod
    def backward(ctx, dy):
        (x2,) = ctx.saved_tensors
        V = ctx.V
        Vp = dy.shape[-1]
        dy2 = _c(dy).view(-1, Vp)
        dx, dw, db = _linear_bwd_raw(dy2, x2, (ctx.weight,), ctx.needs_input_grad[0], ctx.has_bias, pad_rows=Vp - V,
                                     bias_param=ctx.bias, site="vocab")
        return ((dx.view(ctx.in_shape) if dx is not None else None), (dw[:V] if dw is not None else None),
                (db[:V] if db is not None else None))


def _vocab_logits_padded(x, weight, bias):
    return _VocabLinear.apply(x, weight, bias)


def vocab_linear(x, weight, bias=None):
    return _vocab_logits_padded(x, weight, bias)[..., :weight.shape[0]]


def vocab_linear_cross_entropy(x, weight, bias, target, ignore_index: int = -100, rows: str = "all"):
    if rows not in ("all", "labelled"):
        raise ValueError(f"vocab_linear_cross_entropy: rows must be 'all' or 'labelled', got {rows!r}")
    V = weight.shape[0]
    if rows == "labelled":
        sel = select_rows(target.reshape(-1), V, ignore_index)
        m = padded_rows(sel.n)
        if m < sel.idx.numel():
            x = take_rows(x.reshape(-1, x.shape[-1]), sel.idx, sel.inv, m)
            target = sel.target_sel[:m]
    lp = _vocab_logits_padded(x, weight, bias)
    return _SoftmaxCE.apply(lp.reshape(-1, lp.shape[-1]), target.reshape(-1), V, ignore_index)


ROW_PAD_SMALL, ROW_PAD_STREAM, ROW_STREAM_MIN = 8, 256, 1024


def padded_rows(n: int) -> int:
    g = ROW_PAD_STREAM if n >= ROW_STREAM_MIN else ROW_PAD_SMALL
    return max((int(n) + g - 1) // g * g, g)


class SelectedRows(NamedTuple):
    idx: torch.Tensor
    inv: torch.Tensor
    target_sel: torch.Tensor
    count: torch.Tensor
    n: int


def select_rows(target, V: int, ignore_index: int = -100) -> SelectedRows:
    tgt = target.reshape(-1)
    if tgt.dtype != torch.int64:
        tgt = tgt.long()
    n_host = None
    if not tgt.is_cuda:
        n_host = int(((tgt != ignore_index) & (tgt >= 0) & (tgt < V)).sum())
        tgt = tgt.to(torch.device("cuda", torch.cuda.current_device()))
    _need_gpu(tgt)
    tgt = _c(tgt)
    T = tgt.numel()
    dev = tgt.device
    idx = torch.empty(T, device=dev, dtype=torch.int32)
    inv = torch.empty(T, device=dev, dtype=torch.int32)
    tsel = torch.empty(T, device=dev, dtype=torch.int64)
    count = torch.empty(1, device=dev, dtype=torch.int32)
    wsb = lib.meant_select_rows_ws(T)
    ws = _ws(wsb, dev, 16)
    check(lib.meant_select_rows(_p(tgt), T, int(V), int(ignore_index), _p(idx), _p(inv), _p(tsel), _p(count), _p(ws), wsb, _stream()),
          "select_rows")
    if n_host is None:
        n_host = int(count.item())
    return SelectedRows(idx, inv, tsel, count, n_host)


class _TakeRows(torch.autograd.Function):

    @staticmethod
    def forward(ctx, x2d, idx, inv, m):
        ctx.save_for_backward(inv)
        return gather_rows(x2d, idx[:m])

    @staticmethod
    def backward(ctx, dy):
        (inv,) = ctx.saved_tensors
        return gather_rows(dy, inv), None, None, None


def take_rows(x2d, idx, inv, m: int):
    if x2d.dim() != 2 or x2d.shape[0] != idx.numel() or inv.numel() != idx.numel() or not 0 < m <= idx.numel():
# ... 218 lines not shown
```

Before: 3470 samples/s.

## Compute first-layer QKV and embedding backward per vocab id instead of per token

```diff
diff --git a/include/meant_hip.h b/include/meant_hip.h
--- a/include/meant_hip.h
+++ b/include/meant_hip.h
@@ -198,6 +198,13 @@
 int meant_embedding_bwd_seg(const void* dout, const int64_t* sorted_ids, const int64_t* order, float* dtable, int64_t n,
                             int64_t d, int64_t V, int64_t id_lo, int64_t id_hi, int dtype, void* workspace,
                             size_t workspace_bytes, void* stream);
+
+enum meant_by_id_stage { MEANT_BY_ID_SHARED = 1, MEANT_BY_ID_TABLE = 2 };
+size_t meant_qkv_embed_bwd_by_id_ws(int64_t n, int64_t d, int64_t N3, int64_t V);
+int meant_qkv_embed_bwd_by_id(const void* dqkv, const void* dres, const int64_t* sorted_ids, const int64_t* order,
+                              const void* table_bf16, const float* gain, float eps, const void* wT, const void* kv_lists,
+                              float* dw, float* db, float* dgain, float* dtable, int64_t n, int64_t d, int64_t N3, int64_t V,
+                              int64_t id_lo, int64_t id_hi, int stage, void* workspace, size_t workspace_bytes, void* stream);
 
 int meant_ce_probs(const float* probs, const int64_t* target, float* loss_accum, float* dprobs, int64_t B, int C,
                    void* stream);
diff --git a/meant_amd/csrc/common.h b/meant_amd/csrc/common.h
--- a/meant_amd/csrc/common.h
+++ b/meant_amd/csrc/common.h
@@ -45,7 +45,7 @@
   } while (0)
 
 enum meant_option_id {
-  MEANT_OPT_NT_STREAM = 0, MEANT_OPT_NT_DYNAMIC, MEANT_OPT_DETERMINISTIC, MEANT_OPT_NT_GRID_CAP, MEANT_OPT_ATTN_SHORT, MEANT_OPT_NT_RAGGED, MEANT_OPT_ATTN_BWD1, MEANT_OPT_TEMPORAL_LONG, MEANT_OPT_KV_SKIP, MEANT_OPT_COUNT
+  MEANT_OPT_NT_STREAM = 0, MEANT_OPT_NT_DYNAMIC, MEANT_OPT_DETERMINISTIC, MEANT_OPT_NT_GRID_CAP, MEANT_OPT_ATTN_SHORT, MEANT_OPT_NT_RAGGED, MEANT_OPT_ATTN_BWD1, MEANT_OPT_TEMPORAL_LONG, MEANT_OPT_KV_SKIP, MEANT_OPT_QKV_BY_ID, MEANT_OPT_COUNT
 };
 int meant_opt(int id);
 
@@ -57,7 +57,7 @@
   ROUTE_EMB_SEG, ROUTE_SORT_IDS, ROUTE_NT128K, ROUTE_NT256K, ROUTE_SELECT_ROWS, ROUTE_ROTARY_QK, ROUTE_ROTARY_PAIRS, ROUTE_NT_ROT,
   ROUTE_METRICS_ROWS, ROUTE_METRICS_WAVE, ROUTE_METRICS_LABELS, ROUTE_TN256_ROWS, ROUTE_ATTN_CLS_SPLIT, ROUTE_ROWS_ELEM,
   ROUTE_SCORE_CAPTURE, ROUTE_AUROC_RANK, ROUTE_CE_SOFT_WAVE, ROUTE_CE_SOFT_BLOCK, ROUTE_VQA_SCORE,
-  ROUTE_GRAD_STATS, ROUTE_OPTIM_STEP,
+  ROUTE_GRAD_STATS, ROUTE_OPTIM_STEP, ROUTE_QKV_BY_ID,
   MEANT_ROUTE_COUNT
 };
 void meant_route_hit(int route);
diff --git a/meant_amd/csrc/core.hip b/meant_amd/csrc/core.hip
--- a/meant_amd/csrc/core.hip
+++ b/meant_amd/csrc/core.hip
@@ -72,6 +72,7 @@
     {"attn_bwd1", "MEANT_ATTN_BWD1", 1},
     {"temporal_long", "MEANT_TEMPORAL_LONG", 0},
     {"kv_skip", "MEANT_KV_SKIP", 3},
+    {"qkv_by_id", "MEANT_QKV_BY_ID", 1},
 };
 bool is_nt_pp(const char* name) { return name && !strcmp(name, "nt_pp"); }
 std::atomic<int> g_opt[MEANT_OPT_COUNT];
@@ -135,6 +136,7 @@
     "ce_soft_wave", "ce_soft_block",
     "vqa_score",
     "grad_stats", "optim_step",
+    "qkv_by_id",
 };
 std::atomic<long long> g_route[MEANT_ROUTE_COUNT];
 }
diff --git a/meant_amd/csrc/embedding.hip b/meant_amd/csrc/embedding.hip
--- a/meant_amd/csrc/embedding.hip
+++ b/meant_amd/csrc/embedding.hip
@@ -147,7 +147,7 @@
   return w;
 }
 
-constexpr int SEG = 256;
+#include "seg_sum.h"
 template <typename T>
 __global__ __launch_bounds__(256) void emb_seg_kernel(const T* __restrict__ dout, const int64_t* __restrict__ sorted_ids,
                                                        const int64_t* __restrict__ order, float* __restrict__ dtable,
@@ -242,71 +242,6 @@
   }
   const bool open_right = j1 < n && sorted_ids[j1] == cur;
   flush(cur, open_left ? 0 : (open_right ? 1 : -1));
-}
-
-constexpr int SEG_SHORT = 16;
-__global__ __launch_bounds__(256) void emb_seg_cross_kernel(const int64_t* __restrict__ sorted_ids, const float* __restrict__ part,
-                                                             int* __restrict__ longk, float* __restrict__ dtable, int64_t n, int64_t d,
-                                                             int64_t V, int64_t id_lo, int64_t id_hi) {
-  const int lane = threadIdx.x & 63, wave = threadIdx.x >> 6;
-  const int64_t s = (int64_t)blockIdx.x * 4 + wave, j0 = s * SEG, j1 = j0 + SEG;
-  if (j1 >= n) return;
-  const int64_t id = sorted_ids[j1 - 1];
-  const bool owner = sorted_ids[j1] == id && !(j0 > 0 && sorted_ids[j0 - 1] == id)
-                     && id >= 0 && id < V && id >= id_lo && id < id_hi;
-  int64_t K = 0;
-  if (owner) {
-    const int64_t nst = (n + SEG - 1) / SEG;
-    int64_t follow = 0;
-    for (int64_t t0 = s + 1;; t0 += 64) {
-      const int64_t t = t0 + lane;
-      const int k = __popcll(__ballot(t < nst && sorted_ids[t * SEG] == id));
-      follow += k;
-      if (k < 64) break;
-    }
-    K = follow + 1;
-  }
-  if (blockIdx.y == 0 && lane == 0) longk[s] = K > SEG_SHORT ? (int)K : 0;
-  if (K == 0 || K > SEG_SHORT) return;
-  const int64_t col = (int64_t)blockIdx.y * 256 + lane * 4;
-  if (col >= d) return;
-  f32x4 acc = *reinterpret_cast<const f32x4*>(part + (s * 2 + 1) * d + col);
-  for (int64_t k = 1; k < K; ++k) acc += *reinterpret_cast<const f32x4*>(part + (s + k) * 2 * d + col);
-  f32x4* dst = reinterpret_cast<f32x4*>(dtable + id * d + col);
-  *dst = *dst + acc;
-}
-
-__global__ __launch_bounds__(256) void emb_seg_long_kernel(const int64_t* __restrict__ sorted_ids, const float* __restrict__ part,
-                                                            const int* __restrict__ longk, float* __restrict__ dtable, int64_t d) {
-  __shared__ f32x4 red[16][16];
-  const int tid = threadIdx.x;
-  const int64_t s = blockIdx.x;
-  const int64_t K = longk[s];
-  if (K == 0) return;
-  const int64_t id = sorted_ids[s * SEG + SEG - 1];
-  const int p = tid >> 4;
-  const int64_t col = (int64_t)blockIdx.y * 64 + (tid & 15) * 4;
-  const bool active = col < d;
-  const int64_t piece = (K + 15) / 16, k0 = p * piece, k1 = k0 + piece < K ? k0 + piece : K;
-  f32x4 acc = {0.f, 0.f, 0.f, 0.f};
-  if (active) {
-#pragma unroll 4
-    for (int64_t k = k0; k < k1; ++k) {
-      const float* row = k == 0 ? part + (s * 2 + 1) * d : part + (s + k) * 2 * d;
-      acc += *reinterpret_cast<const f32x4*>(row + col);
-    }
-  }
-  red[p][tid & 15] = acc;
-  __syncthreads();
-#pragma unroll
-  for (int h = 8; h > 0; h >>= 1) {
-    if (p < h) red[p][tid & 15] += red[p + h][tid & 15];
-    __syncthreads();
-  }
-  if (p == 0 && active) {
-    f32x4* dst = reinterpret_cast<f32x4*>(dtable + id * d + col);
-    *dst = *dst + red[0][tid & 15];
-  }
 }
 
 size_t seg_part_bytes(int64_t n, int64_t d) { return (size_t)ceil_div(n, SEG) * 2 * (size_t)d * sizeof(float); }
@@ -547,10 +482,11 @@
                                     sorted_ids, order, dtable, (float*)workspace, n, d, V, id_lo, id_hi, cb_chunks));
   if (nst > 1) {
     int* longk = (int*)((char*)workspace + seg_part_bytes(n, d));
-    hipLaunchKernelGGL(emb_seg_cross_kernel, dim3((unsigned)ceil_div(nst - 1, 4), (unsigned)ceil_div(d, 256)), dim3(256), 0, st, sorted_ids,
-                       (const float*)workspace, longk, dtable, n, d, V, id_lo, id_hi);
-    hipLaunchKernelGGL(emb_seg_long_kernel, dim3((unsigned)(nst - 1), (unsigned)ceil_div(d, 64)), dim3(256), 0, st, sorted_ids,
-                       (const float*)workspace, (const int*)longk, dtable, d);
+    const SegAddRow add{dtable, id_lo, id_hi};
+    hipLaunchKernelGGL(seg_cross_kernel<SegAddRow>, dim3((unsigned)ceil_div(nst - 1, 4), (unsigned)ceil_div(d, 256)), dim3(256), 0, st, sorted_ids,
+                       (const float*)workspace, longk, add, n, d, V);
+    hipLaunchKernelGGL(seg_long_kernel<SegAddRow>, dim3((unsigned)(nst - 1), (unsigned)ceil_div(d, 64)), dim3(256), 0, st, sorted_ids,
+                       (const float*)workspace, (const int*)longk, add, d);
   }
   MEANT_LAUNCH_CHECK("embedding_bwd_seg");
   meant_route_hit(ROUTE_EMB_SEG);
diff --git a/meant_amd/csrc/qkv_by_id.hip b/meant_amd/csrc/qkv_by_id.hip
--- /dev/null
+++ b/meant_amd/csrc/qkv_by_id.hip
@@ -0,0 +1,331 @@
+#include "common.h"
+#include "internal.h"
+
+#define BYID_REQ(c, ...) MEANT_REQUIRE(c, MEANT_ERR_ARG, __VA_ARGS__)
+
+namespace {
+
+#include "seg_sum.h"
+constexpr int VPAD = 256;
+
+size_t al256(size_t x) { return (x + 255) & ~(size_t)255; }
+
+__global__ __launch_bounds__(256) void live_flags_kernel(const int* __restrict__ lists, uint8_t* __restrict__ live, int64_t nblk) {
+  const int64_t i = (int64_t)blockIdx.x * 256 + threadIdx.x;
+  if (i >= nblk || i >= lists[0]) return;
+  const int b = lists[MEANT_KV_LIST_HDR + i];
+  if (b >= 0 && b < nblk) live[b] = 1;
+}
+
+__global__ __launch_bounds__(256) void qkv_seg_kernel(const bf16* __restrict__ dqkv, const int64_t* __restrict__ sorted_ids,
+                                                       const int64_t* __restrict__ order, const uint8_t* __restrict__ live,
+                                                       bf16* __restrict__ Dhi, bf16* __restrict__ Dlo, float* __restrict__ part,
+                                                       float* __restrict__ cpart, int64_t n, int64_t N3, int64_t Dq, int64_t V,
+                                                       int cb_chunks) {
+  const int lane = threadIdx.x & 63, wave = threadIdx.x >> 6;
+  const int64_t s = (int64_t)blockIdx.x * 4 + wave;
+  const int64_t j0 = s * SEG;
+  if (j0 >= n) return;
+  const int64_t j1 = j0 + SEG < n ? j0 + SEG : n;
+  const int c0 = blockIdx.y * cb_chunks;
+  const int left = (int)(N3 >> 3) - c0;
+  const int nch = left < cb_chunks ? left : cb_chunks;
+  const bool has0 = lane < nch, has1 = lane + 64 < nch;
+  const int64_t col0 = (int64_t)(c0 + lane) * 8, col1 = (int64_t)(c0 + lane + 64) * 8;
+  const bool kv0 = col0 >= Dq, kv1 = col1 >= Dq;
+  float acc0[8], acc1[8], cs0[8], cs1[8];
+#pragma unroll
+  for (int e = 0; e < 8; ++e) acc0[e] = acc1[e] = cs0[e] = cs1[e] = 0.f;
+  int64_t cur = sorted_ids[j0];
+  bool open_left = j0 > 0 && sorted_ids[j0 - 1] == cur;
+
+  auto flush = [&](int64_t id, int slot) {
+    if (id < 0 || id >= V) return;
+    if (slot >= 0) {
+      float* row = part + (s * 2 + slot) * N3;
+      Vec8<float> v;
+      if (has0) {
+#pragma unroll
+        for (int e = 0; e < 8; ++e) v.set(e, acc0[e]);
+        store8<float>(row + col0, v);
+      }
+      if (has1) {
+#pragma unroll
+        for (int e = 0; e < 8; ++e) v.set(e, acc1[e]);
+        store8<float>(row + col1, v);
+      }
+      return;
+    }
+    Vec8<bf16> h, l;
+    if (has0) {
+#pragma unroll
+      for (int e = 0; e < 8; ++e) {
+        h.set(e, acc0[e]);
+        l.set(e, acc0[e] - h.get(e));
+      }
+      store8<bf16>(Dhi + id * N3 + col0, h);
+      store8<bf16>(Dlo + id * N3 + col0, l);
+    }
+    if (has1) {
+#pragma unroll
+      for (int e = 0; e < 8; ++e) {
+        h.set(e, acc1[e]);
+        l.set(e, acc1[e] - h.get(e));
+      }
+      store8<bf16>(Dhi + id * N3 + col1, h);
+      store8<bf16>(Dlo + id * N3 + col1, l);
+    }
+  };
+
+  for (int64_t jb = j0; jb < j1; jb += 64) {
+    const int64_t jl = jb + lane < j1 ? jb + lane : j1 - 1;
+    const long long my_id = sorted_ids[jl], my_ord = order[jl];
+    const int cnt = (int)(j1 - jb < 64 ? j1 - jb : 64);
+    for (int t0 = 0; t0 < cnt; t0 += 4) {
+      Vec8<bf16> r0[4], r1[4];
+      long long ids4[4];
+#pragma unroll
+      for (int u = 0; u < 4; ++u) {
+        const int t = t0 + u < cnt ? t0 + u : cnt - 1;
+        ids4[u] = __shfl(my_id, t, 64);
+        const long long ord = __shfl(my_ord, t, 64);
+        const bool row_ok = ord >= 0 && ord < n;
+        const bool kv_ok = !live || (row_ok && live[ord >> 6] != 0);
+        const bf16* src = dqkv + (row_ok ? ord : 0) * N3;
+        r0[u] = Vec8<bf16>{};
+        r1[u] = Vec8<bf16>{};
+        if (has0 && row_ok && (!kv0 || kv_ok)) r0[u] = load8s<bf16>(src + col0);
+        if (has1 && row_ok && (!kv1 || kv_ok)) r1[u] = load8s<bf16>(src + col1);
+      }
+#pragma unroll
+      for (int u = 0; u < 4; ++u) {
+        if (t0 + u >= cnt) break;
+        const int64_t id = ids4[u];
+        if (id != cur) {
+          flush(cur, open_left ? 0 : -1);
+#pragma unroll
+          for (int e = 0; e < 8; ++e) acc0[e] = acc1[e] = 0.f;
+          cur = id;
+          open_left = false;
+        }
+#pragma unroll
+        for (int e = 0; e < 8; ++e) {
+          const float a = r0[u].get(e), b = r1[u].get(e);
+          acc0[e] += a; cs0[e] += a;
+          acc1[e] += b; cs1[e] += b;
+        }
+      }
+    }
+  }
+  const bool open_right = j1 < n && sorted_ids[j1] == cur;
+  flush(cur, open_left ? 0 : (open_right ? 1 : -1));
+  Vec8<float> v;
+  if (has0) {
+#pragma unroll
+    for (int e = 0; e < 8; ++e) v.set(e, cs0[e]);
+    store8<float>(cpart + s * N3 + col0, v);
+  }
+  if (has1) {
+#pragma unroll
+    for (int e = 0; e < 8; ++e) v.set(e, cs1[e]);
+    store8<float>(cpart + s * N3 + col1, v);
+  }
+}
+
+__global__ __launch_bounds__(256) void qkv_colsum_kernel(const float* __restrict__ cpart, float* __restrict__ db, int64_t nst, int64_t N3) {
+  __shared__ f32x4 red[16][16];
+  const int tid = threadIdx.x, p = tid >> 4;
+  const int64_t col = (int64_t)blockIdx.x * 64 + (tid & 15) * 4;
+  const bool active = col < N3;
+  const int64_t piece = (nst + 15) / 16, k0 = p * piece, k1 = k0 + piece < nst ? k0 + piece : nst;
+  f32x4 acc = {0.f, 0.f, 0.f, 0.f};
+  if (active)
+    for (int64_t k = k0; k < k1; ++k) acc += *reinterpret_cast<const f32x4*>(cpart + k * N3 + col);
+  red[p][tid & 15] = acc;
+  __syncthreads();
+#pragma unroll
+  for (int h = 8; h > 0; h >>= 1) {
+    if (p < h) red[p][tid & 15] += red[p + h][tid & 15];
+    __syncthreads();
+  }
+  if (p == 0 && active) {
+    f32x4* dst = reinterpret_cast<f32x4*>(db + col);
+    *dst = *dst + red[0][tid & 15];
+  }
+}
+
+__global__ __launch_bounds__(256) void widen_kernel(const bf16* __restrict__ dn_a, const bf16* __restrict__ dn_r, const bf16* __restrict__ table,
+                                                     float* __restrict__ dn, float* __restrict__ x, int64_t chunks) {
+  for (int64_t c = (int64_t)blockIdx.x * 256 + threadIdx.x; c < chunks; c += (int64_t)gridDim.x * 256) {
+    const int64_t off = c * 8;
+    const Vec8<bf16> a = load8<bf16>(dn_a + off), r = load8<bf16>(dn_r + off), t = load8<bf16>(table + off);
+    Vec8<float> v, w;
+#pragma unroll
+    for (int e = 0; e < 8; ++e) {
+      v.set(e, a.get(e) + r.get(e));
+      w.set(e, t.get(e));
+    }
+    store8<float>(dn + off, v);
+    store8<float>(x + off, w);
+  }
+}
+__global__ __launch_bounds__(256) void ones_kernel(float* __restrict__ p, int64_t n) {
+  const int64_t i = (int64_t)blockIdx.x * 256 + threadIdx.x;
+  if (i < n) p[i] = 1.f;
+}
+
+__global__ __launch_bounds__(256) void table_add_kernel(const float* __restrict__ dxtab, float* __restrict__ dtable, int64_t first, int64_t chunks) {
+  for (int64_t c = (int64_t)blockIdx.x * 256 + threadIdx.x; c < chunks; c += (int64_t)gridDim.x * 256) {
+    const int64_t off = first + c * 8;
+    const Vec8<float> g = load8<float>(dxtab + off);
+    Vec8<float> v = load8<float>(dtable + off);
+#pragma unroll
+    for (int e = 0; e < 8; ++e) v.set(e, v.get(e) + g.get(e));
+    store8<float>(dtable + off, v);
+  }
+}
+
+struct ByIdWs { size_t dxtab, dhi, dlo, ntab, rinv, dnlo, dna, dnr, ones, dn32, x32, part, cpart, longk, live, sub, sub_bytes, total; };
+ByIdWs byid_layout(int64_t n, int64_t d, int64_t N3, int64_t V) {
+  ByIdWs w;
+  const int64_t Vp = ceil_div(V, VPAD) * VPAD, nst = ceil_div(n, SEG);
+  size_t off = 0;
+  const auto take = [&off](size_t bytes) { const size_t o = off; off += al256(bytes); return o; };
+  w.dxtab = take((size_t)V * d * sizeof(float));
+  w.dhi = take((size_t)Vp * N3 * sizeof(bf16));
+  w.dlo = take((size_t)Vp * N3 * sizeof(bf16));
+  w.ntab = take((size_t)Vp * d * sizeof(bf16));
+  w.rinv = take((size_t)V * sizeof(float));
+  w.dnlo = take((size_t)Vp * d * sizeof(bf16));
+  w.dna = take((size_t)Vp * d * sizeof(bf16));
+  w.dnr = take((size_t)Vp * d * sizeof(bf16));
+  w.ones = take((size_t)Vp * sizeof(float));
+  w.dn32 = take((size_t)V * d * sizeof(float));
+  w.x32 = take((size_t)V * d * sizeof(float));
+  w.part = take((size_t)nst * 2 * N3 * sizeof(float));
+  w.cpart = take((size_t)nst * N3 * sizeof(float));
+  w.longk = take((size_t)nst * sizeof(int));
+  w.live = take((size_t)ceil_div(n, 64));
+  size_t sub = gemm_bf16_tn_ws(Vp, N3, d);
+  const size_t nb = meant_rmsnorm_bwd_ws(V, d), sb = meant_embedding_bwd_seg_ws(n, d);
+  if (nb > sub) sub = nb;
+  if (sb > sub) sub = sb;
+  w.sub_bytes = sub;
+  w.sub = take(sub);
+  w.total = off;
+  return w;
+}
+
+bool byid_shape_ok(int64_t n, int64_t d, int64_t N3, int64_t V) {
+  return n > 0 && d > 0 && N3 > 0 && V > 0 && n < (1ll << 31) && V < (1ll << 31) && d % 8 == 0 && N3 % 192 == 0 && N3 < (1ll << 22) &&
+         d < (1ll << 22);
+}
+
+}
+
+extern "C" size_t meant_qkv_embed_bwd_by_id_ws(int64_t n, int64_t d, int64_t N3, int64_t V) {
+  return byid_shape_ok(n, d, N3, V) ? byid_layout(n, d, N3, V).total : 0;
+}
+
+extern "C" int meant_qkv_embed_bwd_by_id(const void* dqkv, const void* dres, const int64_t* sorted_ids, const int64_t* order,
+                                         const void* table_bf16, const float* gain, float eps, const void* wT, const void* kv_lists,
+                                         float* dw, float* db, float* dgain, float* dtable, int64_t n, int64_t d, int64_t N3, int64_t V,
+                                         int64_t id_lo, int64_t id_hi, int stage, void* workspace, size_t workspace_bytes, void* stream) {
+  BYID_REQ(sorted_ids && order && dtable && workspace && (stage & ~(MEANT_BY_ID_SHARED | MEANT_BY_ID_TABLE)) == 0 && stage != 0,
+           "qkv_embed_bwd_by_id: bad argument");
+  MEANT_REQUIRE(byid_shape_ok(n, d, N3, V), MEANT_ERR_UNSUPPORTED,
+                "qkv_embed_bwd_by_id: n=%lld d=%lld N3=%lld V=%lld: n, V < 2^31, d %% 8 == 0, N3 = 3 H Dh with H Dh %% 64 == 0", (long long)n,
+                (long long)d, (long long)N3, (long long)V);
+  BYID_REQ(0 <= id_lo && id_lo <= id_hi && id_hi <= V, "qkv_embed_bwd_by_id: bad id range");
+  const ByIdWs w = byid_layout(n, d, N3, V);
+  MEANT_REQUIRE(workspace_bytes >= w.total, MEANT_ERR_WORKSPACE, "qkv_embed_bwd_by_id: workspace of %zu bytes needed, %zu given", w.total,
+                workspace_bytes);
+  BYID_REQ(meant_aligned16(workspace) && meant_aligned16(dtable) && (!dres || meant_aligned16(dres)), "qkv_embed_bwd_by_id: 16-byte alignment");
+  hipStream_t st = (hipStream_t)stream;
+  char* base = (char*)workspace;
+  float* dxtab = (float*)(base + w.dxtab);
+  const int64_t Vp = ceil_div(V, VPAD) * VPAD, nst = ceil_div(n, SEG);
+  int rc;
+
+  if (stage & MEANT_BY_ID_SHARED) {
+    BYID_REQ(dqkv && table_bf16 && gain && wT && dw && db && dgain, "qkv_embed_bwd_by_id: null pointer");
+    BYID_REQ(meant_aligned16(dqkv) && meant_aligned16(table_bf16) && meant_aligned16(wT) && meant_aligned16(db),
+             "qkv_embed_bwd_by_id: 16-byte alignment");
+    bf16 *Dhi = (bf16*)(base + w.dhi), *Dlo = (bf16*)(base + w.dlo), *ntab = (bf16*)(base + w.ntab);
+    bf16 *dnlo = (bf16*)(base + w.dnlo), *dna = (bf16*)(base + w.dna), *dnr = (bf16*)(base + w.dnr);
+    float *ones = (float*)(base + w.ones), *dn32 = (float*)(base + w.dn32), *x32 = (float*)(base + w.x32);
+    float *rinv = (float*)(base + w.rinv), *part = (float*)(base + w.part), *cpart = (float*)(base + w.cpart);
+    int* longk = (int*)(base + w.longk);
+    uint8_t* live = nullptr;
+    hipError_t e = hipMemsetAsync(Dhi, 0, w.ntab - w.dhi, st);
+    if (e == hipSuccess && Vp > V) e = hipMemsetAsync(ntab + V * d, 0, (size_t)(Vp - V) * d * sizeof(bf16), st);
+    if (e == hipSuccess && kv_lists) {
+      live = (uint8_t*)(base + w.live);
+      e = hipMemsetAsync(live, 0, (size_t)ceil_div(n, 64), st);
+    }
+    MEANT_REQUIRE(e == hipSuccess, MEANT_ERR_LAUNCH, "qkv_embed_bwd_by_id: clearing the workspace failed: %s", hipGetErrorString(e));
+    if (live) {
+      const int64_t nblk = n / 64;
+      BYID_REQ(n % 64 == 0, "qkv_embed_bwd_by_id: key-padding lists need n %% 64 == 0");
+      hipLaunchKernelGGL(live_flags_kernel, dim3((unsigned)ceil_div(nblk, 256)), dim3(256), 0, st, (const int*)kv_lists, live, nblk);
+    }
+    const int chunks = (int)(N3 >> 3);
+    const int ncb = (int)ceil_div(chunks, 128);
+    const int cb_chunks = (int)ceil_div(chunks, ncb);
+    hipLaunchKernelGGL(qkv_seg_kernel, dim3((unsigned)ceil_div(nst, 4), (unsigned)ncb), dim3(256), 0, st, (const bf16*)dqkv, sorted_ids, order,
+                       (const uint8_t*)live, Dhi, Dlo, part, cpart, n, N3, N3 / 3, V, cb_chunks);
+    if (nst > 1) {
+      const SegStoreHiLo images{Dhi, Dlo};
+      hipLaunchKernelGGL(seg_cross_kernel<SegStoreHiLo>, dim3((unsigned)ceil_div(nst - 1, 4), (unsigned)ceil_div(N3, 256)), dim3(256), 0, st,
+                         sorted_ids, (const float*)part, longk, images, n, N3, V);
+      hipLaunchKernelGGL(seg_long_kernel<SegStoreHiLo>, dim3((unsigned)(nst - 1), (unsigned)ceil_div(N3, 64)), dim3(256), 0, st, sorted_ids,
+                         (const float*)part, (const int*)longk, images, N3);
+    }
+    hipLaunchKernelGGL(qkv_colsum_kernel, dim3((unsigned)ceil_div(N3, 64)), dim3(256), 0, st, (const float*)cpart, db, nst, N3);
+    MEANT_LAUNCH_CHECK("qkv_embed_bwd_by_id: segmented sum");
+    rc = meant_rmsnorm_fwd(table_bf16, gain, ntab, rinv, V, d, eps, 0.f, 0, MEANT_BF16, stream);
+    if (rc) return rc;
+    void* sub = base + w.sub;
+    rc = gemm_bf16_tn_launch(Dhi, N3, ntab, d, dw, nullptr, Vp, N3, d, sub, w.sub_bytes, st);
+    if (!rc) rc = gemm_bf16_tn_launch(Dlo, N3, ntab, d, dw, nullptr, Vp, N3, d, sub, w.sub_bytes, st);
+    if (rc) return rc;
+    GemmBf16Args a{};
+    a.A = Dlo; a.lda = N3; a.B = (const bf16*)wT; a.ldb = N3; a.C = dnlo; a.ldc = d;
+    a.M = Vp; a.N = d; a.K = N3;
+    rc = gemm_bf16_nt_launch(a, st);
+    if (rc) return rc;
+    a.A = Dhi; a.C = dna; a.residual = dnlo; a.ldr = d;
+    rc = gemm_bf16_nt_launch(a, st);
+    if (rc) return rc;
+    hipLaunchKernelGGL(ones_kernel, dim3((unsigned)ceil_div(Vp, 256)), dim3(256), 0, st, ones, Vp);
+    a.C = dnr; a.sub = dna; a.ldsub = d; a.sub_coef = ones;
+    rc = gemm_bf16_nt_launch(a, st);
+    if (rc) return rc;
+    {
+      const int64_t chunks = V * d / 8;
+      int64_t nb = ceil_div(chunks, 256);
+      if (nb > 8192) nb = 8192;
+      hipLaunchKernelGGL(widen_kernel, dim3((unsigned)nb), dim3(256), 0, st, (const bf16*)dna, (const bf16*)dnr, (const bf16*)table_bf16, dn32, x32, chunks);
+      MEANT_LAUNCH_CHECK("qkv_embed_bwd_by_id: widen");
+    }
+    rc = meant_rmsnorm_bwd(dn32, x32, gain, rinv, dxtab, dgain, V, d, eps, 0.f, 0, nullptr, nullptr, MEANT_F32, sub, w.sub_bytes, stream);
+    if (rc) return rc;
+    meant_route_hit(ROUTE_QKV_BY_ID);
+  }
+
+  if ((stage & MEANT_BY_ID_TABLE) && id_lo < id_hi) {
+    if (dres) {
+      if (d <= 1024)
+        rc = meant_embedding_bwd_sorted_range(dres, sorted_ids, order, dtable, n, d, V, id_lo, id_hi, MEANT_BF16, stream);
+      else
+        rc = meant_embedding_bwd_seg(dres, sorted_ids, order, dtable, n, d, V, id_lo, id_hi, MEANT_BF16, base + w.sub, w.sub_bytes, stream);
+      if (rc) return rc;
+    }
+    const int64_t chunks = (id_hi - id_lo) * d / 8;
+    int64_t nb = ceil_div(chunks, 256);
+    if (nb > 8192) nb = 8192;
+    hipLaunchKernelGGL(table_add_kernel, dim3((unsigned)nb), dim3(256), 0, st, (const float*)dxtab, dtable, id_lo * d, chunks);
+    MEANT_LAUNCH_CHECK("qkv_embed_bwd_by_id: table rows");
+  }
+  return MEANT_OK;
+}
diff --git a/meant_amd/csrc/seg_sum.h b/meant_amd/csrc/seg_sum.h
--- /dev/null
+++ b/meant_amd/csrc/seg_sum.h
@@ -0,0 +1,88 @@
+#pragma once
+
+constexpr int SEG = 256;
+constexpr int SEG_SHORT = 16;
+
+struct SegAddRow {
+  float* dtable; int64_t id_lo, id_hi;
+  __device__ __forceinline__ bool owns(int64_t id) const { return id >= id_lo && id < id_hi; }
+  __device__ __forceinline__ void put(int64_t id, int64_t ld, int64_t col, f32x4 a) const {
+    f32x4* dst = reinterpret_cast<f32x4*>(dtable + id * ld + col);
+    *dst = *dst + a;
+  }
+};
+struct SegStoreHiLo {
+  bf16* hi; bf16* lo;
+  __device__ __forceinline__ bool owns(int64_t) const { return true; }
+  __device__ __forceinline__ void put(int64_t id, int64_t ld, int64_t col, f32x4 a) const {
+    bf16x4 h, l;
+#pragma unroll
+    for (int e = 0; e < 4; ++e) {
+      h[e] = (bf16)a[e];
+      l[e] = (bf16)(a[e] - (float)h[e]);
+    }
+    *reinterpret_cast<bf16x4*>(hi + id * ld + col) = h;
+    *reinterpret_cast<bf16x4*>(lo + id * ld + col) = l;
+  }
+};
+
+template <class Store>
+__global__ __launch_bounds__(256) void seg_cross_kernel(const int64_t* __restrict__ sorted_ids, const float* __restrict__ part,
+                                                         int* __restrict__ longk, Store st, int64_t n, int64_t d, int64_t V) {
+  const int lane = threadIdx.x & 63, wave = threadIdx.x >> 6;
+  const int64_t s = (int64_t)blockIdx.x * 4 + wave, j0 = s * SEG, j1 = j0 + SEG;
+  if (j1 >= n) return;
+  const int64_t id = sorted_ids[j1 - 1];
+  const bool owner = sorted_ids[j1] == id && !(j0 > 0 && sorted_ids[j0 - 1] == id)
+                     && id >= 0 && id < V && st.owns(id);
+  int64_t K = 0;
+  if (owner) {
+    const int64_t nst = (n + SEG - 1) / SEG;
+    int64_t follow = 0;
+    for (int64_t t0 = s + 1;; t0 += 64) {
+      const int64_t t = t0 + lane;
+      const int k = __popcll(__ballot(t < nst && sorted_ids[t * SEG] == id));
+      follow += k;
+      if (k < 64) break;
+    }
+    K = follow + 1;
+  }
+  if (blockIdx.y == 0 && lane == 0) longk[s] = K > SEG_SHORT ? (int)K : 0;
+  if (K == 0 || K > SEG_SHORT) return;
+  const int64_t col = (int64_t)blockIdx.y * 256 + lane * 4;
+  if (col >= d) return;
+  f32x4 acc = *reinterpret_cast<const f32x4*>(part + (s * 2 + 1) * d + col);
+  for (int64_t k = 1; k < K; ++k) acc += *reinterpret_cast<const f32x4*>(part + (s + k) * 2 * d + col);
+  st.put(id, d, col, acc);
+}
+
+template <class Store>
+__global__ __launch_bounds__(256) void seg_long_kernel(const int64_t* __restrict__ sorted_ids, const float* __restrict__ part,
+                                                        const int* __restrict__ longk, Store st, int64_t d) {
+  __shared__ f32x4 red[16][16];
+  const int tid = threadIdx.x;
+  const int64_t s = blockIdx.x;
+  const int64_t K = longk[s];
+  if (K == 0) return;
+  const int64_t id = sorted_ids[s * SEG + SEG - 1];
+  const int p = tid >> 4;
+  const int64_t col = (int64_t)blockIdx.y * 64 + (tid & 15) * 4;
+  const bool active = col < d;
+  const int64_t piece = (K + 15) / 16, k0 = p * piece, k1 = k0 + piece < K ? k0 + piece : K;
+  f32x4 acc = {0.f, 0.f, 0.f, 0.f};
+  if (active) {
+#pragma unroll 4
+    for (int64_t k = k0; k < k1; ++k) {
+      const float* row = k == 0 ? part + (s * 2 + 1) * d : part + (s + k) * 2 * d;
+      acc += *reinterpret_cast<const f32x4*>(row + col);
+    }
+  }
+  red[p][tid & 15] = acc;
+  __syncthreads();
+#pragma unroll
+  for (int h = 8; h > 0; h >>= 1) {
+    if (p < h) red[p][tid & 15] += red[p + h][tid & 15];
+    __syncthreads();
+  }
+  if (p == 0 && active) st.put(id, d, col, red[0][tid & 15]);
+}
diff --git a/meant_amd/modules.py b/meant_amd/modules.py
--- a/meant_amd/modules.py
+++ b/meant_amd/modules.py
@@ -274,12 +274,16 @@
     return int(torch.randint(0, 2 ** 62, (1,)).item())
 
 
-def _encoder_layer(e, e2, x, margs, p1, p2, pool, fold):
-    n, res = ops.rmsnorm_fork(x, e[0].scale, e[0].eps, any_width=True)
-    if COMPOSE_PRE_LINEAR and e[1].bias is not None:
-        h = e[2].multi_mad(e[2].core(n, *margs, pre=e[1]))
+def _encoder_layer(e, e2, x, margs, p1, p2, pool, fold, tokens=None):
+    if tokens is not None:
+        o, res = tokens.attend(e, *margs)
+        h = e[2].multi_mad(o)
     else:
-        h = e[2](e[1](n), *margs)
+        n, res = ops.rmsnorm_fork(x, e[0].scale, e[0].eps, any_width=True)
+        if COMPOSE_PRE_LINEAR and e[1].bias is not None:
+            h = e[2].multi_mad(e[2].core(n, *margs, pre=e[1]))
+        else:
+            h = e[2](e[1](n), *margs)
     h = e[3](h, drop_p=p1, seed=_seed() if p1 > 0 else 0)
     x1 = e[-1](h, residual=res)
     fold = ops.norm_linear_ok(x1, e2[1].weight, fold)
@@ -323,10 +327,10 @@
         self.encode = nn.ModuleList([RMSNorm(dim), Linear(dim, dim), att, RMSNorm(dim), nn.Dropout(dropout), Linear(dim, dim)])
         self.encode2 = nn.ModuleList([RMSNorm(dim), Linear(dim, dim), nn.GELU(), RMSNorm(dim), nn.Dropout(), Linear(dim, dim)])
 
-    def forward(self, input, attention_mask=None, pool: bool = False, fold=None):
+    def forward(self, input, attention_mask=None, pool: bool = False, fold=None, tokens=None):
         e, e2 = self.encode, self.encode2
         p1, p2 = (e[4].p, e2[4].p) if self.training else (0.0, 0.0)
-        return _encoder_layer(e, e2, input, (attention_mask,), p1, p2, pool, fold)
+        return _encoder_layer(e, e2, input, (attention_mask,), p1, p2, pool, fold, tokens)
 
 
 class temporalEncoder(nn.Module):
@@ -384,16 +388,22 @@
     return v if isinstance(v, bool) else int(v)
 
 
-def _run_stack(encoders, x, *args, checkpoint=False):
+def _run_stack(encoders, x, *args, checkpoint=False, tokens=None):
     n = len(encoders)
-    fold = ops.stack_fold(n, x.numel() // x.shape[-1], x.shape[-1])
+    rows, d = (tokens.ids.numel(), tokens.table.shape[1]) if tokens is not None else (x.numel() // x.shape[-1], x.shape[-1])
+    fold = ops.stack_fold(n, rows, d)
     for i, enc in enumerate(encoders):
         ck = checkpoint if isinstance(checkpoint, bool) else i < checkpoint
+        kw = {}
+        if i == 0 and tokens is not None:
+            if ck:
+                raise RuntimeError("meant_amd: the by-id first layer cannot run under activation recomputation")
+            kw["tokens"] = tokens
         last = enc.encode2[-1]
         if POOL_LAST_LINEAR and i == n - 1 and isinstance(last, Linear):
-            h, res = _run_encoder(enc, x, *args, checkpoint=ck, pool=True, fold=fold)
+            h, res = _run_encoder(enc, x, *args, checkpoint=ck, pool=True, fold=fold, **kw)
             return (h, res, last.weight, last.bias)
-        x = _run_encoder(enc, x, *args, checkpoint=ck, fold=fold)
+        x = _run_encoder(enc, x, *args, checkpoint=ck, fold=fold, **kw)
     return x
 
 
@@ -423,6 +433,42 @@
     return ops.pooled_linear_cat([st], compute_dtype)
 
 
+class _TokenIds:
+
+    def __init__(self, ids, table, dtype):
+        self.ids, self.table, self.dtype = ids, table, dtype
+
+    def attend(self, e, attention_mask=None):
+        att = e[2]
+        wqkv, bqkv = _qkv_params(att, e[1])
+        tables = att.xPos.tables(self.ids.shape[1], self.ids.device, ops.run_head_dim(att.Dh, self.dtype)) if att.xPos is not None else None
+        return ops.embed_qkv_attention(self.ids, self.table, e[0].scale, e[0].eps, wqkv, bqkv, tables, attention_mask, bool(att.mask),
+                                       att.num_heads)
+
+
+def _by_id_source(mods, ids, dtype, encoders, ckpt=False):
+    if len(mods) != 1 or not len(encoders) or ckpt or not torch.is_grad_enabled() or not COMPOSE_PRE_LINEAR:
+        return None
+    emb, enc = mods[0], encoders[0]
+    if not (isinstance(emb, nn.Embedding) and emb.max_norm is None and not emb.sparse and ids.dtype in (torch.int64, torch.int32)):
+        return None
+    if not (isinstance(enc, languageEncoder) and ids.is_cuda and ids.dim() == 2 and emb.weight.requires_grad and emb.weight.dtype == torch.float32):
+        return None
+    e = enc.encode
+    att, norm = e[2], e[0]
+    if not (isinstance(att, xPosAttention) and isinstance(norm, RMSNorm) and isinstance(e[1], nn.Linear) and e[1].bias is not None):
+        return None
+    rot = att.xPos
+    if (rot is not None and getattr(rot, 'learned_freq', False)) or (att.training and att.dropout.p > 0):
+        return None
+    if getattr(norm, 'p', -1.) >= 0 or getattr(norm, 'bias', False) or norm.scale.shape[0] != emb.weight.shape[1]:
+        return None
+    V, d = emb.weight.shape
+    if not ops.qkv_by_id_shape_ok(d, att.atten_size, att.Dh, V, dtype) or not ops.qkv_by_id_wanted(ids.numel(), V):
+        return None
+    return _TokenIds(ids, emb.weight, dtype)
+
+
 def _embed(mods, ids, dtype):
     x = ids
     for mod in mods:
@@ -471,10 +517,12 @@
         B = images.shape[0]
         if images.is_cuda and TWO_STREAMS:
             ops.set_index_stream(images.device, _side_stream(images.device))
-        words = _embed(self.embedding, tweets.reshape(B * self.lag, tweets.shape[2]), dt)
+        ck = _ckpt_setting(self)
+        ids2 = tweets.reshape(B * self.lag, tweets.shape[2])
+        tok = _by_id_source(self.embedding, ids2, dt, self.languageEncoders, ck if isinstance(ck, bool) else ck > 0)
+        words = _embed(self.embedding, ids2, dt) if tok is None else None
         if attention_mask is not None:
             attention_mask = attention_mask.reshape(B * self.lag, attention_mask.shape[2])
-        ck = _ckpt_setting(self)
         side = _side_stream(images.device) if (TWO_STREAMS and images.is_cuda and not ck) else None
         if side is not None:
             main = torch.cuda.current_stream()
@@ -487,14 +535,14 @@
             hi = _hi_stream(images.device)
             hi.wait_stream(main)
             with torch.cuda.stream(hi):
-                words = _run_stack(self.languageEncoders, words, attention_mask, checkpoint=ck)
+                words = _run_stack(self.languageEncoders, words, attention_mask, checkpoint=ck, tokens=tok)
                 words = _pool_own_stream(dt, words)
             main.wait_stream(hi)
             for tt in (words if isinstance(words, tuple) else (words,)):
                 if tt is not None and tt.is_cuda:
                     tt.record_stream(main)
         else:
-            words = _run_stack(self.languageEncoders, words, attention_mask, checkpoint=ck)
+            words = _run_stack(self.languageEncoders, words, attention_mask, checkpoint=ck, tokens=tok)
         if side is not None:
             main.wait_stream(side)
             for tt in (img if isinstance(img, tuple) else (img,)):
@@ -556,9 +604,11 @@
     def forward(self, tweets, attention_mask=None):
         dt = resolve_compute_dtype(self, None)
         B = tweets.shape[0]
-        words = _embed(self.embedding, tweets.reshape(B * self.lag, tweets.shape[2]), dt)
+        ids2 = tweets.reshape(B * self.lag, tweets.shape[2])
+        tok = _by_id_source(self.embedding, ids2, dt, self.languageEncoders)
+        words = _embed(self.embedding, ids2, dt) if tok is None else None
         attention_mask = attention_mask.reshape(B * self.lag, attention_mask.shape[2])
-        words = _run_stack(self.languageEncoders, words, attention_mask)
+        words = _run_stack(self.languageEncoders, words, attention_mask, tokens=tok)
         fused = _pool_parts(dt, words).view(B, self.lag, self.dim)
         for enc in self.temporal_encoding:
             fused = enc(fused)
@@ -587,8 +637,9 @@
 
     def forward(self, tweets, images, attention_mask=None):
         dt = resolve_compute_dtype(self, images)
-        words = _embed(self.embedding, tweets, dt)
-        words = _run_stack(self.languageEncoders, words, attention_mask)
+        tok = _by_id_source(self.embedding, tweets, dt, self.languageEncoders)
+        words = _embed(self.embedding, tweets, dt) if tok is None else None
+        words = _run_stack(self.languageEncoders, words, attention_mask, tokens=tok)
         img = self.patchEmbed(images, dt)
         img = _run_stack(self.visionEncoders, img)
         fused = _pool_parts(dt, words, img)
@@ -619,10 +670,12 @@
 
     def _encode(self, words, attention_mask):
         dt = resolve_compute_dtype(self, None)
-        x = _embed(self.embedding, words, dt)
-        fold = ops.stack_fold(len(self.languageEncoders), x.numel() // x.shape[-1], x.shape[-1])
-        for enc in self.languageEncoders:
-            x = enc(x, attention_mask=attention_mask, fold=fold)
+        tok = _by_id_source(self.embedding, words, dt, self.languageEncoders)
+        x = _embed(self.embedding, words, dt) if tok is None else None
+        rows, d = (words.numel(), tok.table.shape[1]) if tok is not None else (x.numel() // x.shape[-1], x.shape[-1])
+        fold = ops.stack_fold(len(self.languageEncoders), rows, d)
+        for i, enc in enumerate(self.languageEncoders):
+            x = enc(x, attention_mask=attention_mask, fold=fold, **({"tokens": tok} if tok is not None and i == 0 else {}))
         return x
 
     def _head_features(self, x):
diff --git a/meant_amd/ops.py b/meant_amd/ops.py
--- a/meant_amd/ops.py
+++ b/meant_amd/ops.py
@@ -853,40 +853,46 @@
     return dqkv
 
 
+def _qkv_attn_fwd_raw(x, wqkv, bqkv, tables, key_mask, causal, num_heads, scale=None):
+    _need_gpu(x, wqkv)
+    G, S, d = x.shape
+    D = wqkv.shape[0] // 3
+    Dh = D // num_heads
+    x2 = _c(x).view(G * S, d)
+    w_f = _c(wqkv.detach().float())
+    if x.dtype == torch.bfloat16 and d % 8:
+        d8 = (d + 7) & ~7
+        x2, w_c = _pad_cols(x2, d8), _pad_cols(w_f, d8, x.dtype)
+    else:
+        w_c = cast(w_f, x.dtype)
+    bias_f = _c(bqkv.detach().float())
+    dt = _dt(x)
+    qa, qb, ka, kb, R = _rot(tables)
+    km = _c(key_mask.float()) if key_mask is not None else None
+    skip = _kv_skip_bits(x, km, S, D, Dh)
+    lists = kv_live_rows(km, causal) if skip else None
+    qkv = torch.empty((G * S, 3 * D), device=x.device, dtype=x.dtype)
+    if skip & KV_SKIP_FWD:
+        check(lib.meant_qkv_proj_fwd_live(_p(x2), x2.stride(0), _p(w_c), _p(bias_f), _p(qkv), G * S, x2.shape[1], S, num_heads, Dh, R,
+                                          _p(qa), _p(qb), _p(ka), _p(kb), _p(lists), dt, _stream()), "qkv_proj_fwd_live")
+    else:
+        check(lib.meant_qkv_proj_fwd(_p(x2), x2.stride(0), _p(w_c), _p(bias_f), _p(qkv), G * S, x2.shape[1], S, num_heads, Dh, R,
+                                     _p(qa), _p(qb), _p(ka), _p(kb), dt, _stream()), "qkv_proj_fwd")
+    scale = 1.0 / math.sqrt(Dh * num_heads) if scale is None else float(scale)
+    o, lse = _attn_fwd_raw(qkv, km, G, S, num_heads, Dh, scale, int(causal))
+    return x2, qkv, o, lse, km, w_f, lists, skip, (G, S, d, D, Dh, num_heads, scale, int(causal))
+
+
 class _QKVAttention(torch.autograd.Function):
 
     @staticmethod
     def forward(ctx, x, wqkv, bqkv, tables, key_mask, causal, num_heads, scale=None):
-        _need_gpu(x, wqkv)
-        G, S, d = x.shape
-        D = wqkv.shape[0] // 3
-        Dh = D // num_heads
-        x2 = _c(x).view(G * S, d)
-        w_f = _c(wqkv.detach().float())
-        if x.dtype == torch.bfloat16 and d % 8:
-            d8 = (d + 7) & ~7
-            x2, w_c = _pad_cols(x2, d8), _pad_cols(w_f, d8, x.dtype)
-        else:
-            w_c = cast(w_f, x.dtype)
-        bias_f = _c(bqkv.detach().float())
-        dt = _dt(x)
-        qa, qb, ka, kb, R = _rot(tables)
-        km = _c(key_mask.float()) if key_mask is not None else None
-        skip = _kv_skip_bits(x, km, S, D, Dh)
-        lists = kv_live_rows(km, causal) if skip else None
-        qkv = torch.empty((G * S, 3 * D), device=x.device, dtype=x.dtype)
-        if skip & KV_SKIP_FWD:
-            check(lib.meant_qkv_proj_fwd_live(_p(x2), x2.stride(0), _p(w_c), _p(bias_f), _p(qkv), G * S, x2.shape[1], S, num_heads, Dh, R,
-                                              _p(qa), _p(qb), _p(ka), _p(kb), _p(lists), dt, _stream()), "qkv_proj_fwd_live")
-        else:
-            check(lib.meant_qkv_proj_fwd(_p(x2), x2.stride(0), _p(w_c), _p(bias_f), _p(qkv), G * S, x2.shape[1], S, num_heads, Dh, R,
-                                         _p(qa), _p(qb), _p(ka), _p(kb), dt, _stream()), "qkv_proj_fwd")
-        scale = 1.0 / math.sqrt(Dh * num_heads) if scale is None else float(scale)
-        o, lse = _attn_fwd_raw(qkv, km, G, S, num_heads, Dh, scale, int(causal))
+        x2, qkv, o, lse, km, w_f, lists, skip, meta = _qkv_attn_fwd_raw(x, wqkv, bqkv, tables, key_mask, causal, num_heads, scale)
         ctx.save_for_backward(x2, qkv, o, lse, km, w_f, lists)
         ctx.kv_skip = skip
         ctx.tables = tables
-        ctx.meta = (G, S, d, D, Dh, num_heads, scale, int(causal))
+        ctx.meta = meta
+        G, S, D = meta[0], meta[1], meta[3]
         return o.view(G, S, D)
 
     @staticmethod
@@ -1406,36 +1412,62 @@
     return sorted_ids, order
 
 
+def _embedding_fwd_raw(ids, table, dtype):
+    _need_gpu(ids, table)
+    ids_c = _c(ids.long())
+    V, d = table.shape
+    n = ids_c.numel()
+    out = torch.empty((*ids.shape, d), device=table.device, dtype=dtype)
+    if dtype == torch.bfloat16 and EMB_BF16_TABLE and d % 8 == 0 and V < (1 << 31):
+        tb = weights.get((table,), torch.bfloat16, False)
+        idx = ids_c.view(-1).clamp(0, V - 1).to(torch.int32)
+        check(lib.meant_gather_rows(_p(tb), _p(idx), None, _p(out), n, d, BF16, _stream()), "gather_rows")
+    else:
+        tf = _c(table.detach().float())
+        check(lib.meant_embedding_fwd(_p(tf), _p(ids_c), _p(out), n, d, V, F32 if dtype == torch.float32 else BF16, _stream()),
+              "embedding_fwd")
+    return ids_c, out
+
+
+def _presort_ids(ids_c, V, d, force=False):
+    if not EMB_PRESORT or (not force and _emb_bwd_route(ids_c.numel(), d) == "atomic"):
+        return None
+    main = torch.cuda.current_stream(ids_c.device)
+    side = _aux_stream(ids_c.device)
+    side.wait_stream(main)
+    with torch.cuda.stream(side):
+        sorted_ids, order = _sort_ids(ids_c.view(-1), V)
+        ev = torch.cuda.Event()
+        ev.record(side)
+    return sorted_ids, order, ev
+
+
+def _sorted_ids_now(presort, ids_c, V):
+    if presort is None:
+        return _sort_ids(ids_c.view(-1), V)
+    sorted_ids, order, ev = presort
+    cur = torch.cuda.current_stream(ids_c.device)
+    cur.wait_event(ev)
+    sorted_ids.record_stream(cur)
+    order.record_stream(cur)
+    return sorted_ids, order
+
+
+def _table_grad_target(table, V, d, device):
+    sink = _sink_of(table, "embedding") if grad_sinks else None
+    if sink is not None and (sink.view.shape != (V, d) or not sink.view.is_contiguous()):
+        sink = None
+    return sink, (sink.view if sink is not None else torch.zeros((V, d), device=device, dtype=torch.float32))
+
+
 class _Embedding(torch.autograd.Function):
 
     @staticmethod
     def forward(ctx, ids, table, dtype):
-        _need_gpu(ids, table)
-        ids_c = _c(ids.long())
+        ids_c, out = _embedding_fwd_raw(ids, table, dtype)
         V, d = table.shape
-        n = ids_c.numel()
-        out = torch.empty((*ids.shape, d), device=table.device, dtype=dtype)
-        if dtype == torch.bfloat16 and EMB_BF16_TABLE and d % 8 == 0 and V < (1 << 31):
-            tb = weights.get((table,), torch.bfloat16, False)
-            idx = ids_c.view(-1).clamp(0, V - 1).to(torch.int32)
-            check(lib.meant_gather_rows(_p(tb), _p(idx), None, _p(out), n, d, BF16, _stream()), "gather_rows")
-        else:
-            tf = _c(table.detach().float())
-            check(lib.meant_embedding_fwd(_p(tf), _p(ids_c), _p(out), n, d, V, F32 if dtype == torch.float32 else BF16, _stream()),
-                  "embedding_fwd")
-        presort = None
-        route = _emb_bwd_route(n, d)
-        if EMB_PRESORT and ctx.needs_input_grad[1] and route != "atomic":
-            main = torch.cuda.current_stream(ids_c.device)
-            side = _aux_stream(ids_c.device)
-            side.wait_stream(main)
-            with torch.cuda.stream(side):
-                sorted_ids, order = _sort_ids(ids_c.view(-1), V)
-                ev = torch.cuda.Event()
-                ev.record(side)
-            presort = (sorted_ids, order, ev)
         ctx.save_for_backward(ids_c)
-        ctx.presort = presort
+        ctx.presort = _presort_ids(ids_c, V, d) if ctx.needs_input_grad[1] else None
         ctx.meta = (V, d)
         ctx.table = table
         _claim(table, "embedding")
@@ -1446,21 +1478,11 @@
         (ids_c,) = ctx.saved_tensors
         V, d = ctx.meta
         dout = _c(dout)
-        sink = _sink_of(ctx.table, "embedding") if grad_sinks else None
-        if sink is not None and (sink.view.shape != (V, d) or not sink.view.is_contiguous()):
-            sink = None
-        dtab = sink.view if sink is not None else torch.zeros((V, d), device=dout.device, dtype=torch.float32)
+        sink, dtab = _table_grad_target(ctx.table, V, d, dout.device)
         n = ids_c.numel()
         route = _emb_bwd_route(n, d)
         if route != "atomic":
-            if ctx.presort is not None:
-                sorted_ids, order, ev = ctx.presort
-                cur = torch.cuda.current_stream(dout.device)
-                cur.wait_event(ev)
-                sorted_ids.record_stream(cur)
-                order.record_stream(cur)
-            else:
-                sorted_ids, order = _sort_ids(ids_c.view(-1), V)
+            sorted_ids, order = _sorted_ids_now(ctx.presort, ids_c, V)
             nsl = sink.row_slices(ctx.table) if sink is not None else 1
             if route == "seg":
                 wsb = lib.meant_embedding_bwd_seg_ws(n, d)
@@ -1493,6 +1515,78 @@
 
 def embedding(ids, table, dtype):
     return _Embedding.apply(ids, table, dtype)
+
+
+QKV_BY_ID_MIN_RATIO = 6
+QKV_BY_ID_MIN_ROWS = 4096
+
+
+def qkv_by_id_shape_ok(d: int, D: int, Dh: int, V: int, dtype: torch.dtype) -> bool:
+    return (dtype == torch.bfloat16 and EMB_BF16_TABLE and d % 8 == 0 and D % 256 == 0 and Dh in NATIVE_HEAD_DIMS and V < (1 << 31))
+
+
+def qkv_by_id_wanted(n_tokens: int, V: int) -> bool:
+    opt = _lib.get_option("qkv_by_id")
+    return opt == 2 or (opt == 1 and V >= QKV_BY_ID_MIN_ROWS and n_tokens >= QKV_BY_ID_MIN_RATIO * V)
+
+
+class _EmbedQKVAttention(torch.autograd.Function):
+
+    @staticmethod
+    def forward(ctx, ids, table, gain, eps, wqkv, bqkv, tables, key_mask, causal, num_heads):
+        ids_c, x = _embedding_fwd_raw(ids, table, torch.bfloat16)
+        V, d = table.shape
+        presort = _presort_ids(ids_c, V, d, force=True)
+        n_, sc, _rinv = _rmsnorm_fwd_raw(x, gain, eps, 0.0, 0)
+        _x2, qkv, o, lse, km, w_f, lists, skip, meta = _qkv_attn_fwd_raw(n_, wqkv, bqkv, tables, key_mask, causal, num_heads)
+        ctx.save_for_backward(ids_c, qkv, o, lse, km, w_f, lists if skip & KV_SKIP_DW else None, sc)
+        ctx.presort, ctx.tables, ctx.meta, ctx.eps, ctx.table = presort, tables, meta, eps, table
+        _claim(table, "embedding")
+        G, S, D = meta[0], meta[1], meta[3]
+        return o.view(G, S, D), x
+
+    @staticmethod
+    def backward(ctx, do, dres):
+        ids_c, qkv, o, lse, km, w_f, lists, sc = ctx.saved_tensors
+        G, S, d, D, Dh, H, scale, causal = ctx.meta
+        table = ctx.table
+        V = table.shape[0]
+        n, N3 = G * S, 3 * D
+        do2 = _c(do).view(n, D)
+        dqkv = _attn_bwd_raw(qkv, o, do2, lse, km, G, S, H, Dh, scale, causal, ctx.tables)
+        dev = do2.device
+        wT = torch.empty((d, N3), device=dev, dtype=torch.bfloat16)
+        check(lib.meant_transpose2d(_p(w_f), F32, _p(wT), BF16, N3, d, _stream()), "transpose2d")
+        dw = torch.zeros((N3, d), device=dev, dtype=torch.float32)
+        db = torch.zeros(N3, device=dev, dtype=torch.float32)
+        dgain = torch.empty(d, device=dev, dtype=torch.float32)
+        dres2 = _c(dres).view(n, d) if dres is not None else None
+        sink, dtab = _table_grad_target(table, V, d, dev)
+        sorted_ids, order = _sorted_ids_now(ctx.presort, ids_c, V)
+        tb = weights.get((table,), torch.bfloat16, False)
+        wsb = lib.meant_qkv_embed_bwd_by_id_ws(n, d, N3, V)
+        ws = _ws(wsb, dev)
+        nsl = sink.row_slices(table) if sink is not None else 1
+
+        def call(lo, hi, stage):
+            check(lib.meant_qkv_embed_bwd_by_id(_p(dqkv), _p(dres2), _p(sorted_ids), _p(order), _p(tb), _p(sc), ctx.eps, _p(wT), _p(lists),
+                                                _p(dw), _p(db), _p(dgain), _p(dtab), n, d, N3, V, lo, hi, stage, _p(ws), wsb, _stream()),
+                  "qkv_embed_bwd_by_id")
+        if nsl > 1:
+            call(0, 0, _lib.BY_ID_SHARED)
+            for c in range(nsl):
+                lo, hi = V * c // nsl, V * (c + 1) // nsl
+                call(lo, hi, _lib.BY_ID_TABLE)
+                sink.report_rows(table, lo, hi, c == nsl - 1)
+        else:
+            call(0, V, _lib.BY_ID_SHARED | _lib.BY_ID_TABLE)
+            if sink is not None:
+                sink.report(table)
+        return None, (None if sink is not None else dtab), dgain, None, dw, db, None, None, None, None
+
+
+def embed_qkv_attention(ids, table, gain, eps, wqkv, bqkv, tables, key_mask, causal, num_heads):
+    return _EmbedQKVAttention.apply(ids, table, gain, float(eps), wqkv, bqkv, tables, key_mask, bool(causal), num_heads)
 
 
 def cast(x: torch.Tensor, dtype: torch.dtype) -> torch.Tensor:
```

New measurement: 3707 samples/s (median of 6 runs). +6.8%, better.
